# arangesh/Ground-Plane-Polling

Hardware: AMD Instinct MI355X
Metric: images/sec end-to-end (resnet50, 1k planes, 1242x375) (higher is better)
Workload: dtype f16x3

## Files before the change

### ground-plane-polling_amd/csrc/conv_igemm.hip

```cpp

#include <hip/hip_runtime.h>
#include <stdint.h>
#include <stdlib.h>

#include "conv_igemm_types.h"
#include "conv_tiles.h"
#include "gpp.h"

namespace {

inline bool is_x3(int dtype) { return dtype == GPP_BF16X3 || dtype == GPP_F16X3; }
inline bool f32_storage(int dtype) { return dtype == GPP_F32 || is_x3(dtype); }
inline int elem_size(int dtype) { return f32_storage(dtype) ? 4 : 2; }

int validate(const gpp_conv_desc& d)
{
    if (!d.in || !d.weight || !d.out) return GPP_ERR_BAD_ARG;
    if (d.dtype != GPP_BF16 && d.dtype != GPP_F16 && d.dtype != GPP_F32 && !is_x3(d.dtype)) return GPP_ERR_UNSUPPORTED;
    const int esz = elem_size(d.dtype), ck = 128 / esz, va = 16 / esz;
    if (d.batch <= 0 || d.C_in <= 0 || d.C_out <= 0 || d.KH <= 0 || d.KW <= 0) return GPP_ERR_BAD_ARG;
    constexpr int kMaxDim = 1 << 20;
    if (d.batch > kMaxDim || d.C_in > kMaxDim || d.C_out > kMaxDim || d.in_pitch > kMaxDim || d.out_pitch > kMaxDim || d.res_pitch > kMaxDim ||
        d.weight_rows > kMaxDim || d.weight_rows < 0 || d.in_pitch < 0 || d.out_pitch < 0 || d.res_pitch < 0 || d.partial_bytes < 0)
        return GPP_ERR_UNSUPPORTED;
    if (d.KH > 8 || d.KW > 8) return GPP_ERR_UNSUPPORTED;
    if (d.C_in % ck != 0 || d.C_out % 4 != 0) return GPP_ERR_UNSUPPORTED;
    if (d.stride != 1 && d.stride != 2) return GPP_ERR_UNSUPPORTED;
    if (d.n_groups < 1 || d.n_groups > GPP_MAX_GROUPS) return GPP_ERR_BAD_ARG;
    if (d.split_k < 0) return GPP_ERR_BAD_ARG;
#ifndef GPP_STAMPS
    if (d.reserved != 0) return GPP_ERR_BAD_ARG;
#endif
    if (d.reserved2 != 0 || (d.x3_split & ~(GPP_X3_IN | GPP_X3_OUT | GPP_X3_RES))) return GPP_ERR_BAD_ARG;
    if (d.reserved3 != 0 || (d.gather_rows != nullptr) != (d.gather_counts != nullptr)) return GPP_ERR_BAD_ARG;
    if (((uintptr_t)d.gather_rows | (uintptr_t)d.gather_counts | (uintptr_t)d.guard) & 3) return GPP_ERR_ALIGN;
    if (d.gather_rows && (d.stride != 1 || d.residual || !d.out_f32 || d.split_k > 1)) return GPP_ERR_UNSUPPORTED;
    if (d.x3_split && !is_x3(d.dtype)) return GPP_ERR_BAD_ARG;
    if (d.out_scale && d.dtype != GPP_F16X3) return GPP_ERR_BAD_ARG;
    if ((d.x3_split & GPP_X3_OUT) && (d.out_f32 || d.C_out % 32 != 0 || d.out_pitch % 32 != 0)) return GPP_ERR_UNSUPPORTED;
    if ((d.x3_split & GPP_X3_IN) && d.in_pitch % 32 != 0) return GPP_ERR_UNSUPPORTED;
    if ((d.x3_split & GPP_X3_RES) && (!d.residual || d.res_pitch % 32 != 0)) return GPP_ERR_UNSUPPORTED;
    const int oa = (d.out_f32 || f32_storage(d.dtype)) ? 4 : 8;
    if (d.in_pitch < d.C_in || d.in_pitch % va != 0) return GPP_ERR_ALIGN;
    if (d.out_pitch < d.C_out || d.out_pitch % oa != 0) return GPP_ERR_ALIGN;
    if (d.residual && (d.res_pitch < d.C_out || d.res_pitch % va != 0)) return GPP_ERR_ALIGN;
    if (((uintptr_t)d.in | (uintptr_t)d.weight | (uintptr_t)d.out | (uintptr_t)d.zero_page | (uintptr_t)d.residual |
         (uintptr_t)d.bias | (uintptr_t)d.partial) & 15)
        return GPP_ERR_ALIGN;
    for (int g = 0; g < d.n_groups; ++g) {
        const gpp_conv_group& G = d.groups[g];
        if (G.H_in <= 0 || G.W_in <= 0 || G.H_out <= 0 || G.W_out <= 0) return GPP_ERR_BAD_ARG;
        if (G.H_in > kMaxDim || G.W_in > kMaxDim || G.H_out > kMaxDim || G.W_out > kMaxDim || G.H_res > kMaxDim || G.W_res > kMaxDim) return GPP_ERR_UNSUPPORTED;
        constexpr int64_t kMaxOff = (int64_t)1 << 40;
        if (G.in_off < 0 || G.out_off < 0 || G.res_off < 0 || G.in_bstride < 0 || G.out_bstride < 0 || G.res_bstride < 0 || G.in_off > kMaxOff ||
            G.out_off > kMaxOff || G.res_off > kMaxOff || G.in_bstride > kMaxOff || G.out_bstride > kMaxOff || G.res_bstride > kMaxOff)
            return GPP_ERR_BAD_ARG;
        if ((G.out_off | G.out_bstride) % oa != 0) return GPP_ERR_ALIGN;
        if ((G.in_off | G.in_bstride) % va != 0) return GPP_ERR_ALIGN;
        if (d.residual && ((G.res_off | G.res_bstride) % va != 0 || G.H_res <= 0 || G.W_res <= 0)) return GPP_ERR_ALIGN;
        if ((int64_t)d.batch * G.H_out * G.W_out >= (1LL << 31)) return GPP_ERR_UNSUPPORTED;
        if ((d.x3_split & GPP_X3_OUT) && ((G.out_off | G.out_bstride) % 32 != 0)) return GPP_ERR_ALIGN;
        if ((d.x3_split & GPP_X3_IN) && ((G.in_off | G.in_bstride) % 32 != 0)) return GPP_ERR_ALIGN;
        if ((d.x3_split & GPP_X3_RES) && ((G.res_off | G.res_bstride) % 32 != 0)) return GPP_ERR_ALIGN;
    }
    return GPP_OK;
}

int split_rule(const gpp_conv_desc& d)
{
    if (!d.partial) return 1;
    int64_t pix = 0;
    for (int g = 0; g < d.n_groups; ++g) pix += (int64_t)d.groups[g].H_out * d.groups[g].W_out;
    const int64_t tiles_per_image = ((pix + 127) / 128) * ((d.C_out + 127) / 128);
    const int64_t kdepth = (int64_t)d.KH * d.KW * d.C_in;
    if (tiles_per_image > 24 || kdepth < 3072) return 1;
    int split = (int)((kdepth + 768) / 1536);
    return split < 1 ? 1 : (split > 8 ? 8 : split);
}

int fill_range_counter(gpp_conv_desc& d)
{
    if (d.dtype != GPP_F16X3) return d.range_counter ? GPP_ERR_BAD_ARG : GPP_OK;
    if (!d.range_counter) d.range_counter = (uint64_t*)gpp_x3_range_counter_f16x3();
    if (!d.range_counter) return GPP_ERR_UNSUPPORTED;
    return ((uintptr_t)d.range_counter & 7) ? GPP_ERR_ALIGN : GPP_OK;
}

int dispatch_any(gpp_conv_desc& d, hipStream_t st)
{
    const int rc = fill_range_counter(d);
    if (rc != GPP_OK) return rc;
    if (d.split_k == 0) d.split_k = split_rule(d);
    if (d.gather_rows) {
        if (d.split_k > 1) return GPP_ERR_UNSUPPORTED;
        return gpp_conv_gather_dispatch(d, st);
    }
    switch (d.dtype) {
        case GPP_BF16: return gpp_conv_dispatch_bf16(d, st);
        case GPP_F16: return gpp_conv_dispatch_f16(d, st);
        case GPP_BF16X3: return gpp_conv_dispatch_bf16x3(d, st);
        case GPP_F16X3: return gpp_conv_dispatch_f16x3(d, st);
        default: return gpp_conv_dispatch_f32(d, st);
    }
}

int tail_entry(const gpp_conv_desc* conv3x3, const gpp_conv_desc* conv1x1, int tile_rows, void* stream)
{
    if (!conv3x3 || !conv1x1) return GPP_ERR_BAD_ARG;
    gpp_conv_desc d1 = *conv3x3, d2 = *conv1x1;
    int rc = validate(d1);
    if (rc == GPP_OK) rc = validate(d2);
    if (rc != GPP_OK) return rc;
    if (d1.gather_rows || d2.gather_rows || d1.guard || d2.guard) return GPP_ERR_UNSUPPORTED;
    const gpp_conv_group &G1 = d1.groups[0], &G2 = d2.groups[0];
    if (d1.dtype == GPP_F32) return GPP_ERR_UNSUPPORTED;
    if (is_x3(d1.dtype) && (!(d1.x3_split & GPP_X3_IN) || (d2.x3_split & (GPP_X3_OUT | GPP_X3_RES)) != (GPP_X3_OUT | GPP_X3_RES) || !d2.residual))
        return GPP_ERR_UNSUPPORTED;
    if (d1.dtype != d2.dtype || d1.n_groups != 1 || d2.n_groups != 1 || d1.batch != d2.batch) return GPP_ERR_UNSUPPORTED;
    if (d1.KH != 3 || d1.KW != 3 || d1.stride != 1 || d1.pad_top != 1 || d1.pad_left != 1 || d1.residual || d1.out_f32) return GPP_ERR_UNSUPPORTED;
    if (d1.C_in != d1.C_out || (d1.C_in != 64 && d1.C_in != 128) || d1.weight_rows < d1.C_out) return GPP_ERR_UNSUPPORTED;
    if (d2.KH != 1 || d2.KW != 1 || d2.stride != 1 || d2.pad_top != 0 || d2.pad_left != 0 || d2.C_in != d1.C_out) return GPP_ERR_UNSUPPORTED;
    if (d2.C_out % 128 != 0 || d2.weight_rows < d2.C_out) return GPP_ERR_UNSUPPORTED;
    if (G1.H_in != G1.H_out || G1.W_in != G1.W_out || G2.H_out != G1.H_out || G2.W_out != G1.W_out || G2.H_in != G1.H_out || G2.W_in != G1.W_out)
        return GPP_ERR_BAD_ARG;
    rc = fill_range_counter(d1);
    if (rc == GPP_OK) rc = fill_range_counter(d2);
    if (rc != GPP_OK) return rc;
    hipStream_t st = (hipStream_t)stream;
    switch (d1.dtype) {
        case GPP_BF16: return gpp_tail_dispatch_bf16(d1, d2, tile_rows, st);
        case GPP_F16: return gpp_tail_dispatch_f16(d1, d2, tile_rows, st);
        case GPP_BF16X3: return gpp_tail_dispatch_bf16x3(d1, d2, tile_rows, st);
        default: return gpp_tail_dispatch_f16x3(d1, d2, tile_rows, st);
    }
}

int block_entry(const gpp_conv_desc* conv_a, const gpp_conv_desc* conv_b, const gpp_conv_desc* conv_c, int tile, void* stream)
{
    if (!conv_a || !conv_b || !conv_c) return GPP_ERR_BAD_ARG;
    gpp_conv_desc d1 = *conv_a, d2 = *conv_b, d3 = *conv_c;
    int rc = validate(d1);
    if (rc == GPP_OK) rc = validate(d2);
    if (rc == GPP_OK) rc = validate(d3);
    if (rc != GPP_OK) return rc;
    if (d1.gather_rows || d2.gather_rows || d3.gather_rows || d1.guard || d2.guard || d3.guard) return GPP_ERR_UNSUPPORTED;
    const gpp_conv_group &G1 = d1.groups[0], &G2 = d2.groups[0], &G3 = d3.groups[0];
    if (!is_x3(d1.dtype) || d1.dtype != d2.dtype || d1.dtype != d3.dtype) return GPP_ERR_UNSUPPORTED;
    if (d1.n_groups != 1 || d2.n_groups != 1 || d3.n_groups != 1 || d1.batch != d2.batch || d1.batch != d3.batch) return GPP_ERR_UNSUPPORTED;
    if (d1.x3_split != (GPP_X3_IN | GPP_X3_OUT) || d2.x3_split != (GPP_X3_IN | GPP_X3_OUT) || d3.x3_split != (GPP_X3_IN | GPP_X3_OUT | GPP_X3_RES))
        return GPP_ERR_UNSUPPORTED;
    if (d1.KH != 1 || d1.KW != 1 || d1.pad_top != 0 || d1.pad_left != 0 || d1.residual || d1.out_f32 || d1.split_k > 1) return GPP_ERR_UNSUPPORTED;
    if (d2.KH != 3 || d2.KW != 3 || d2.stride != 1 || d2.pad_top != 1 || d2.pad_left != 1 || d2.residual || d2.out_f32 || d2.split_k > 1) return GPP_ERR_UNSUPPORTED;
    if (d3.KH != 1 || d3.KW != 1 || d3.stride != 1 || d3.pad_top != 0 || d3.pad_left != 0 || !d3.residual || d3.out_f32 || d3.split_k > 1) return GPP_ERR_UNSUPPORTED;
    const int C = d2.C_in;
    if ((C != 64 && C != 128) || d2.C_out != C || d1.C_out != C || d3.C_in != C || d3.C_out % 128 != 0) return GPP_ERR_UNSUPPORTED;
    if (d1.weight_rows < C || d2.weight_rows < C || d3.weight_rows < d3.C_out) return GPP_ERR_UNSUPPORTED;
    if (G1.H_out != (G1.H_in - 1) / d1.stride + 1 || G1.W_out != (G1.W_in - 1) / d1.stride + 1) return GPP_ERR_BAD_ARG;
    if (G2.H_in != G1.H_out || G2.W_in != G1.W_out || G2.H_out != G1.H_out || G2.W_out != G1.W_out || G3.H_in != G1.H_out || G3.W_in != G1.W_out ||
        G3.H_out != G1.H_out || G3.W_out != G1.W_out || G3.H_res != G1.H_out || G3.W_res != G1.W_out)
        return GPP_ERR_BAD_ARG;
    rc = fill_range_counter(d1);
    if (rc == GPP_OK) rc = fill_range_counter(d2);
    if (rc == GPP_OK) rc = fill_range_counter(d3);
    if (rc != GPP_OK) return rc;
    if (d1.range_counter != d3.range_counter || d2.range_counter != d3.range_counter) return GPP_ERR_BAD_ARG;
    hipStream_t st = (hipStream_t)stream;
    return d1.dtype == GPP_F16X3 ? gpp_block_dispatch_f16x3(d1, d2, d3, tile, st) : gpp_block_dispatch_bf16x3(d1, d2, d3, tile, st);
}

}

extern "C" int gpp_bottleneck_block(const gpp_conv_desc* conv1x1_a, const gpp_conv_desc* conv3x3_b, const gpp_conv_desc* conv1x1_c, int tile, void* stream)
{
    return block_entry(conv1x1_a, conv3x3_b, conv1x1_c, tile, stream);
}

extern "C" int gpp_bottleneck_tail(const gpp_conv_desc* conv3x3, const gpp_conv_desc* conv1x1, int tile_rows, void* stream)
{
    return tail_entry(conv3x3, conv1x1, tile_rows, stream);
}

extern "C" int gpp_x3_range_events(uint64_t* host_count, int reset)
{
    unsigned long long v = 0;
    const int rc = gpp_x3_range_events_f16x3(&v, reset);
    if (rc == GPP_OK && host_count) *host_count = (uint64_t)v;
    return rc;
}

extern "C" int gpp_x3_range_snapshot(uint64_t* device_count, void* stream)
{
    return gpp_x3_range_snapshot_of(nullptr, device_count, stream);
}

extern "C" int gpp_x3_range_snapshot_of(const uint64_t* counter, uint64_t* device_count, void* stream)
{
    if (!device_count) return GPP_ERR_BAD_ARG;
    if (((uintptr_t)counter | (uintptr_t)device_count) & 7) return GPP_ERR_ALIGN;
    return gpp_x3_range_snapshot_f16x3((const unsigned long long*)counter, (unsigned long long*)device_count, (hipStream_t)stream);
}

extern "C" int gpp_conv2d_flops(const gpp_conv_desc* host_desc, double* flops)
{
    if (!host_desc || !flops) return GPP_ERR_BAD_ARG;
    if (host_desc->n_groups < 1 || host_desc->n_groups > GPP_MAX_GROUPS) return GPP_ERR_BAD_ARG;
    double f = 0.0;
    for (int g = 0; g < host_desc->n_groups; ++g)
        f += 2.0 * host_desc->batch * (double)host_desc->groups[g].H_out * host_desc->groups[g].W_out *
             host_desc->KH * host_desc->KW * (double)host_desc->C_in * host_desc->C_out;
    *flops = f;
    return GPP_OK;
}

extern "C" int gpp_conv2d_split_rule(const gpp_conv_desc* host_desc, int* split_k)
{
    if (!host_desc || !split_k) return GPP_ERR_BAD_ARG;
    gpp_conv_desc d = *host_desc;
    int rc = validate(d);
    if (rc != GPP_OK) return rc;
    *split_k = d.split_k > 0 ? d.split_k : split_rule(d);
    return GPP_OK;
}

extern "C" int gpp_conv2d_workspace_bytes(const gpp_conv_desc* host_desc, size_t* bytes)
{
    if (!host_desc || !bytes) return GPP_ERR_BAD_ARG;
    gpp_conv_desc d = *host_desc;
    char probe[16] __attribute__((aligned(16)));
    if (!d.partial) { d.partial = probe; d.partial_bytes = 0; }
    int rc = validate(d);
    if (rc != GPP_OK) return rc;
    const int split = d.split_k > 0 ? d.split_k : split_rule(d);
    *bytes = 0;
    if (split <= 1) return GPP_OK;
    int64_t rows = 0;
    for (int g = 0; g < d.n_groups; ++g) rows += (int64_t)d.batch * d.groups[g].H_out * d.groups[g].W_out + 256;
    const int64_t npad = (d.C_out + 255) / 256 * 256;
    *bytes = (size_t)(split * rows * npad * 4);
    return GPP_OK;
}

extern "C" int gpp_conv2d_igemm(const gpp_conv_desc* host_desc, void* stream)
{
    if (!host_desc) return GPP_ERR_BAD_ARG;
    gpp_conv_desc d = *host_desc;
    for (int g = 0; g < GPP_MAX_GROUPS; ++g) d.groups[g].row_begin = 0;
    int rc = validate(d);
    if (rc != GPP_OK) return rc;
    return dispatch_any(d, (hipStream_t)stream);
}

static const gpp_tiles::Entry kTiles[] = {{0, gpp_tiles::PLAIN, gpp_tiles::ALL, 0, 128, 0, 0, 0}, GPP_CONV_TILES(GPP_TILE_ENTRY, GPP_TILE_NONE, GPP_TILE_NONE)};

static bool env_is_1(const char* name) { const char* e = getenv(name); return e && e[0] == '1'; }

static bool tile_is_candidate(const gpp_conv_desc* desc, const gpp_tiles::Entry& t)
{
    using namespace gpp_tiles;
    const gpp_conv_desc& d = *desc;
    if ((d.gather_rows != nullptr) != (t.form == GATHER)) return t.code == 0;
    const bool x3_in = is_x3(d.dtype) && (d.x3_split & GPP_X3_IN);
    if (!owner_has(t.owner, f32_storage(d.dtype), is_x3(d.dtype))) return false;
    if (is_x3(d.dtype) && x3_wants_split_input(t.form, t.owner) && !x3_in && t.owner != ALL_X3IN) return false;
    const int nk = d.KH * d.KW * (d.C_in / (128 / elem_size(d.dtype)));
    if (t.form == DUAL && !dual_can_run(d, nk)) return false;
    if (t.form == MIX && !mix_can_run(d, nk)) return false;
    if (t.form == WS && !ws_can_run(d, t.bm, t.bn)) return false;
    static const bool no_deep = env_is_1("GPP_NO_DEEP_TILES"), no_ws = env_is_1("GPP_NO_WS_TILES"), no_mix = env_is_1("GPP_NO_MIX_TILES");
    int64_t rows = 0;
    for (int g = 0; g < d.n_groups; ++g) rows += (int64_t)d.batch * d.groups[g].H_out * d.groups[g].W_out;
    const int bn = t.bn;
    const auto pads_less_than = [&](int other) { return (d.C_out + bn - 1) / bn * bn < (d.C_out + other - 1) / other * other; };
    switch (t.form) {
        case GATHER: return bn != 160 || pads_less_than(64);
        case DEEP: {
            int64_t tiles_m = 0;
            for (int g = 0; g < d.n_groups; ++g) tiles_m += ((int64_t)d.batch * d.groups[g].H_out * d.groups[g].W_out + t.bm - 1) / t.bm;
            const int64_t wgs = tiles_m * ((d.C_out + bn - 1) / bn) * (d.split_k > 1 ? d.split_k : 1);
            return !(bn == 64 && d.C_out > 256) && !no_deep && nk >= 12 && wgs <= 320;
        }
        case WS: return !no_ws && rows >= 256 * 16;
        case MIX: return !no_mix && nk >= 4 && rows * (d.C_out / 256) >= 256 * 256;
        default: break;
    }
    if (t.code == 0) return true;
    if (bn == 64 && d.C_out > 256 && !(d.KH == 1 && d.KW == 1 && d.C_in <= 256)) return false;
    if (bn == 256 && (d.C_out < 192 || rows < 256 * 16)) return false;
    if ((t.form == PIPE || t.form == DUAL) && nk < 4) return false;
    if ((bn == 160 || bn == 96) && !pads_less_than(128)) return false;
    return true;
}

extern "C" int gpp_conv2d_tile_candidates(const gpp_conv_desc* desc, int* tiles, int capacity, int* count)
{
    if (!desc || !count || capacity < 0 || (capacity > 0 && !tiles)) return GPP_ERR_BAD_ARG;
    {
        gpp_conv_desc d = *desc;
        for (int g = 0; g < GPP_MAX_GROUPS; ++g) d.groups[g].row_begin = 0;
        const int rc = validate(d);
        if (rc != GPP_OK) return rc;
    }
    int n = 0;
    for (const gpp_tiles::Entry& t : kTiles) {
        if (!tile_is_candidate(desc, t)) continue;
        if (n < capacity) tiles[n] = t.code;
        ++n;
    }
    *count = n;
    return GPP_OK;
}

extern "C" int gpp_conv2d_autotune(gpp_conv_desc* desc, int iters, void* stream, float* best_us)
{
    if (!desc || iters < 1) return GPP_ERR_BAD_ARG;
    {
        gpp_conv_desc d = *desc;
        for (int g = 0; g < GPP_MAX_GROUPS; ++g) d.groups[g].row_begin = 0;
        const int rc = validate(d);
        if (rc != GPP_OK) return rc;
    }
    hipStream_t st = (hipStream_t)stream;
    hipEvent_t e0, e1;
    hipError_t e = hipEventCreate(&e0);
    if (e != hipSuccess) return (int)e;
    e = hipEventCreate(&e1);
    if (e != hipSuccess) { (void)hipEventDestroy(e0); return (int)e; }
    const int tile_in = desc->tile_hint;
    float best = 1e30f;
    int best_tile = tile_in, rc = GPP_OK;
    auto time_one = [&](int tile, float* us, int reps = 2) -> int {
        desc->tile_hint = tile;
        int r = gpp_conv2d_igemm(desc, stream);
        if (r != GPP_OK) return r;
        float t_best = 1e30f;
        for (int rep = 0; rep < reps; ++rep) {
            (void)hipEventRecord(e0, st);
            for (int i = 0; i < iters; ++i) (void)gpp_conv2d_igemm(desc, stream);
            (void)hipEventRecord(e1, st);
            hipError_t s = hipEventSynchronize(e1);
            if (s != hipSuccess) return (int)s;
            float ms = 0.0f;
            (void)hipEventElapsedTime(&ms, e0, e1);
            t_best = ms < t_best ? ms : t_best;
        }
        *us = t_best * 1000.0f / iters;
        return GPP_OK;
    };
    float second = 1e30f;
    int second_tile = -1;
    for (const gpp_tiles::Entry& t : kTiles) {
        if (!tile_is_candidate(desc, t)) continue;
        const int tile = t.code;
        float us = 0.0f;
        int r = time_one(tile, &us);
        if (r != GPP_OK) { if (tile == 0) { rc = r; break; } continue; }
        if (us < best) { second = best; second_tile = best_tile; best = us; best_tile = tile; }
        else if (us < second) { second = us; second_tile = tile; }
    }
    if (rc == GPP_OK && second_tile >= 0 && second_tile != best_tile && second <= best * 1.05f) {
        float sum_a = 0.0f, sum_b = 0.0f;
        bool ok = true;
        for (int round = 0; round < 3 && ok; ++round) {
            float a = 0.0f, b = 0.0f;
            ok = time_one(best_tile, &a, 1) == GPP_OK && time_one(second_tile, &b, 1) == GPP_OK;
            sum_a += a;
            sum_b += b;
        }
        if (ok && sum_b < sum_a) { best_tile = second_tile; best = sum_b / 3.0f; }
        else if (ok) best = sum_a / 3.0f;
    }
    (void)hipEventDestroy(e0);
    (void)hipEventDestroy(e1);
    desc->tile_hint = rc == GPP_OK ? best_tile : tile_in;
    if (best_us) *best_us = best;
    return rc;
}

namespace {

#define GPP_TILE_CODE(code, ...) code,
static const int kPreactTiles[] = {0, GPP_CONV_TILES(GPP_TILE_NONE, GPP_TILE_NONE, GPP_TILE_CODE)};
#undef GPP_TILE_CODE

int preact_validate(gpp_conv_desc& d, const float* in_scale, const float* in_shift)
{
    for (int g = 0; g < GPP_MAX_GROUPS; ++g) d.groups[g].row_begin = 0;
    int rc = validate(d);
    if (rc != GPP_OK) return rc;
    if (d.dtype != GPP_F32 && !is_x3(d.dtype)) return GPP_ERR_UNSUPPORTED;
    if (!in_scale || !in_shift) return GPP_ERR_BAD_ARG;
    if (((uintptr_t)in_scale | (uintptr_t)in_shift) & 15) return GPP_ERR_ALIGN;
    if (d.KH != 1 || d.KW != 1 || d.stride != 1 || d.pad_top != 0 || d.pad_left != 0) return GPP_ERR_UNSUPPORTED;
    if (d.x3_split & GPP_X3_IN) return GPP_ERR_UNSUPPORTED;
    if (d.gather_rows || d.guard) return GPP_ERR_UNSUPPORTED;
    if (d.C_in > 4096) return GPP_ERR_UNSUPPORTED;
    return GPP_OK;
}

int preact_run(gpp_conv_desc& d, const float* in_scale, const float* in_shift, hipStream_t st)
{
    int rc = fill_range_counter(d);
    if (rc != GPP_OK) return rc;
    if (d.split_k == 0) d.split_k = split_rule(d);
    switch (d.dtype) {
        case GPP_BF16X3: return gpp_preact_dispatch_bf16x3(d, in_scale, in_shift, st);
        case GPP_F16X3: return gpp_preact_dispatch_f16x3(d, in_scale, in_shift, st);
        default: return gpp_preact_dispatch_f32(d, in_scale, in_shift, st);
    }
}

}

extern "C" int gpp_conv2d_preact(const gpp_conv_desc* host_desc, const float* in_scale, const float* in_shift, void* stream)
{
    if (!host_desc) return GPP_ERR_BAD_ARG;
    gpp_conv_desc d = *host_desc;
    const int rc = preact_validate(d, in_scale, in_shift);
    if (rc != GPP_OK) return rc;
    return preact_run(d, in_scale, in_shift, (hipStream_t)stream);
}

extern "C" int gpp_conv2d_preact_tile_candidates(const gpp_conv_desc* desc, int* tiles, int capacity, int* count)
{
    if (!desc || !count || capacity < 0 || (capacity > 0 && !tiles)) return GPP_ERR_BAD_ARG;
    gpp_conv_desc d = *desc;
    static const float probe[4] __attribute__((aligned(16))) = {0.f, 0.f, 0.f, 0.f};
    const int rc = preact_validate(d, probe, probe);
    if (rc != GPP_OK) return rc;
    int n = 0;
    for (int tile : kPreactTiles) {
        if (n < capacity) tiles[n] = tile;
        ++n;
    }
    *count = n;
    return GPP_OK;
}

extern "C" int gpp_conv2d_preact_autotune(gpp_conv_desc* desc, const float* in_scale, const float* in_shift, int iters, void* stream,
                                          float* best_us)
{
    if (!desc || iters < 1) return GPP_ERR_BAD_ARG;
    {
        gpp_conv_desc d = *desc;
        const int rc = preact_validate(d, in_scale, in_shift);
        if (rc != GPP_OK) return rc;
    }
    hipStream_t st = (hipStream_t)stream;
    hipEvent_t e0, e1;
    hipError_t e = hipEventCreate(&e0);
    if (e != hipSuccess) return (int)e;
    e = hipEventCreate(&e1);
    if (e != hipSuccess) { (void)hipEventDestroy(e0); return (int)e; }
    const int tile_in = desc->tile_hint;
    float best = 1e30f;
    int best_tile = tile_in, rc = GPP_OK;
    for (int tile : kPreactTiles) {
        desc->tile_hint = tile;
        int r = gpp_conv2d_preact(desc, in_scale, in_shift, stream);
        if (r != GPP_OK) { if (tile == 0) { rc = r; break; } continue; }
        float t_best = 1e30f;
        for (int rep = 0; rep < 2 && r == GPP_OK; ++rep) {
            (void)hipEventRecord(e0, st);
            for (int i = 0; i < iters; ++i) (void)gpp_conv2d_preact(desc, in_scale, in_shift, stream);
            (void)hipEventRecord(e1, st);
            const hipError_t s = hipEventSynchronize(e1);
            if (s != hipSuccess) { r = (int)s; break; }
            float ms = 0.0f;
            (void)hipEventElapsedTime(&ms, e0, e1);
            t_best = ms < t_best ? ms : t_best;
        }
        if (r != GPP_OK) { rc = r; break; }
        const float us = t_best * 1000.0f / iters;
        if (us < best) { best = us; best_tile = tile; }
    }
    (void)hipEventDestroy(e0);
    (void)hipEventDestroy(e1);
    desc->tile_hint = rc == GPP_OK ? best_tile : tile_in;
// ... 4 lines not shown
```

### ground-plane-polling_amd/csrc/conv_igemm_impl.h

```cpp
#ifndef GPP_CONV_IGEMM_IMPL_H_
#define GPP_CONV_IGEMM_IMPL_H_

#include <hip/hip_runtime.h>
#include <stdint.h>

#include <atomic>
#include <type_traits>

#include "conv_tiles.h"
#include "gpp.h"

namespace {

typedef __attribute__((ext_vector_type(8))) __bf16 bf16x8;
typedef __attribute__((ext_vector_type(8))) _Float16 f16x8;
typedef __attribute__((ext_vector_type(4))) float f32x4;

struct f32x8 {
    f32x4 lo, hi;
    __device__ __forceinline__ float operator[](int e) const { return e < 4 ? lo[e] : hi[e - 4]; }
};

template <int DT> struct Elem;
template <> struct Elem<GPP_BF16> {
// ... 269 lines not shown
        *(vec8*)dst = Elem<DT>::pack(v);
    }
}

struct RowAddr { int64_t obase; int64_t rbase; };
__device__ __forceinline__ RowAddr row_addr(const gpp_conv_desc& d, int m, int HoWo, int W_out, int H_out, int H_res, int W_res,
                                            int64_t out_off, int64_t out_bs, int64_t res_off, int64_t res_bs)
{
    const int b = m / HoWo, p = m - b * HoWo;
    int64_t rp = p;
    if (d.residual && (H_res != H_out || W_res != W_out)) {
        const float sy = (float)H_res / (float)H_out, sx = (float)W_res / (float)W_out;
        const int oy = p / W_out, ox = p - oy * W_out;
        const int ry = min((int)floorf((float)oy * sy), H_res - 1);
        const int rx = min((int)floorf((float)ox * sx), W_res - 1);
        rp = (int64_t)ry * W_res + rx;
    }
    RowAddr a;
    a.obase = out_off + (int64_t)b * out_bs + (int64_t)p * d.out_pitch;
    a.rbase = res_off + (int64_t)b * res_bs + rp * d.res_pitch;
    return a;
}

struct PixWalk {
    int b, oy, ox;
    __device__ __forceinline__ void init(int m, int HoWo, int W_out)
    {
        b = m / HoWo;
        const int p = m - b * HoWo;
        oy = p / W_out;
        ox = p - oy * W_out;
    }
    __device__ __forceinline__ void advance(int n, int H_out, int W_out)
    {
        ox += n;
        while (ox >= W_out) { ox -= W_out; ++oy; }
        while (oy >= H_out) { oy -= H_out; ++b; }
    }
};

__device__ __forceinline__ RowAddr row_addr_at(const gpp_conv_desc& d, const PixWalk& w, int W_out, int H_out, int H_res, int W_res,
                                               int64_t out_off, int64_t out_bs, int64_t res_off, int64_t res_bs)
{
    const int p = w.oy * W_out + w.ox;
    int64_t rp = p;
    if (d.residual && (H_res != H_out || W_res != W_out)) {
        const float sy = (float)H_res / (float)H_out, sx = (float)W_res / (float)W_out;
        const int ry = min((int)floorf((float)w.oy * sy), H_res - 1);
        const int rx = min((int)floorf((float)w.ox * sx), W_res - 1);
        rp = (int64_t)ry * W_res + rx;
    }
    RowAddr a;
    a.obase = out_off + (int64_t)w.b * out_bs + (int64_t)p * d.out_pitch;
    a.rbase = res_off + (int64_t)w.b * res_bs + rp * d.res_pitch;
    return a;
}

template <int DT> struct ElemX3 {
    using scalar = float;
    using vec8 = f32x8;
    using frag = f32x4;
    static constexpr int ESZ = 4;
    static __device__ __forceinline__ vec8 pack(const float (&v)[8]) { return Elem<GPP_F32>::pack(v); }
    static __device__ __forceinline__ f32x4 mfma(frag, frag, f32x4 c) { return c; }
    static __device__ __forceinline__ void split(const f32x4 x0, const f32x4 x1, typename X3Half<DT>::vec& hi, typename X3Half<DT>::vec& lo)
    {
        using half = typename X3Half<DT>::half;
#pragma unroll
        for (int e = 0; e < 8; ++e) {
            const float x = X3Half<DT>::clamp(e < 4 ? x0[e] : x1[e - 4]);
            const half h = (half)x;
            hi[e] = h;
            lo[e] = (half)(x - (float)h);
        }
    }
};
template <> struct Elem<GPP_BF16X3> : ElemX3<GPP_BF16X3> {};
template <> struct Elem<GPP_F16X3> : ElemX3<GPP_F16X3> {};

template <int DT> constexpr bool kF32Storage = (DT == GPP_F32 || DT == GPP_BF16X3 || DT == GPP_F16X3);

constexpr int stage_rows(int BM, int NW) { return (BM + 8 * NW - 1) / (8 * NW) * (8 * NW); }

template <int DT, int BM, int BN, int WM, int WN, int STAGES, bool PIPE, bool XIN = false, bool PRE = false, bool GATHER = false>
__device__ __forceinline__ void conv_igemm_body(const gpp_conv_desc& d, const int block_x, const int grid_x, const float* pre_s = nullptr,
                                                const float* pre_t = nullptr)
{
    static_assert(!XIN || kX3<DT>, "pre-split input maps: GPP_BF16X3 / GPP_F16X3");
    static_assert(!PRE || (!PIPE && !XIN && kF32Storage<DT>), "pre-activation: float32-sized input maps, plain loop");
    static_assert(!GATHER || (!PIPE && !PRE), "gathered rows: plain loop");
    if (d.guard != nullptr && *(const volatile int32_t*)d.guard != d.guard_value) return;
    using E = Elem<DT>;
    using vec8 = typename E::vec8;
    using frag = typename E::frag;
    using scalar = typename E::scalar;
    using xh8 = typename X3Half<DT>::vec;
    constexpr int ESZ = E::ESZ, CK = kRowBytes / ESZ;
    constexpr int NW = WM * WN;
    constexpr int MF = BM / WM / 16, NF = BN / WN / 16;
    constexpr int BMS = stage_rows(BM, NW);
    constexpr int A_BYTES = BMS * kRowBytes, B_BYTES = BN * kRowBytes, STAGE = A_BYTES + B_BYTES;
    constexpr int A_IT = BMS / 8 / NW, B_IT = BN / 8 / NW;
    constexpr int PER_STAGE = A_IT + B_IT;
    constexpr int PF = STAGES - 1;
    static_assert(MF >= 1 && NF >= 1 && A_IT >= 1 && B_IT >= 1 && BMS % (8 * NW) == 0 && BN % (8 * NW) == 0 && BM % (16 * WM) == 0, "tile / wave shape");

    extern __shared__ __attribute__((aligned(16))) unsigned char smem[];

    const int tid = threadIdx.x, lane = tid & 63;
    const int wave = __builtin_amdgcn_readfirstlane(tid >> 6);
    const int wm = wave / WN, wn = wave % WN;
    GPP_STAMP(0);

    const int bid = GATHER ? block_x : xcd_remap(block_x, grid_x);
    const int n_tiles = (d.C_out + BN - 1) / BN;
    const int nt = bid % n_tiles, mt = bid / n_tiles;
    int tile_start = 0, row_begin = 0, H_in = 0, W_in = 0, H_out = 0, W_out = 0, H_res = 0, W_res = 0;
    int64_t in_off = 0, in_bs = 0, out_off = 0, out_bs = 0, res_off = 0, res_bs = 0;
    int list_begin = 0, list_next = 0, group = 0;
#pragma unroll
    for (int q = 0; q < GPP_MAX_GROUPS; ++q) {
        if constexpr (GATHER) {
            if (q < d.n_groups && mt >= d.groups[q].tile_start) { list_begin = list_next; group = q; }
            if (q < d.n_groups) list_next += d.batch * d.groups[q].H_out * d.groups[q].W_out;
        }
        if (q < d.n_groups && mt >= d.groups[q].tile_start) {
            tile_start = d.groups[q].tile_start;
            row_begin = d.groups[q].row_begin;
            H_in = d.groups[q].H_in; W_in = d.groups[q].W_in;
            H_out = d.groups[q].H_out; W_out = d.groups[q].W_out;
            H_res = d.groups[q].H_res; W_res = d.groups[q].W_res;
            in_off = d.groups[q].in_off; in_bs = d.groups[q].in_bstride;
            out_off = d.groups[q].out_off; out_bs = d.groups[q].out_bstride;
            res_off = d.groups[q].res_off; res_bs = d.groups[q].res_bstride;
        }
    }
    const int HoWo = H_out * W_out;
    const int Mpix = d.batch * HoWo;
    const int32_t* const glist = GATHER ? d.gather_rows + list_begin : nullptr;
    const int Mg = GATHER ? min(max(d.gather_counts[group], 0), Mpix) : Mpix;
    const int m0 = row_begin + (mt - tile_start) * BM, n0 = nt * BN;
    if constexpr (GATHER) {
        if (m0 >= Mg) return;
    }
    auto pixel_of = [&](int m) { return min(max(glist[m], 0), Mpix - 1); };
    const int Ktot = d.KH * d.KW * d.C_in;
    const int cpt = d.C_in / CK;
    const int nk_total = d.KH * d.KW * cpt;
    const int nsplit = gridDim.y, split = blockIdx.y;
    int ks0 = 0, nk = nk_total;
    if (nsplit > 1) {
        ks0 = (int)((unsigned)(nk_total * split) / (unsigned)nsplit);
        nk = (int)((unsigned)(nk_total * (split + 1)) / (unsigned)nsplit) - ks0;
    }

    const int srow = lane >> 3;
    const int gchunk = (lane & 7) ^ srow;
    const __amdgpu_buffer_rsrc_t in_rsrc = __builtin_amdgcn_make_buffer_rsrc((void*)d.in, 0, d.in_bytes, 0x00020000);
    const __amdgpu_buffer_rsrc_t w_rsrc = __builtin_amdgcn_make_buffer_rsrc((void*)d.weight, 0, d.weight_bytes, 0x00020000);
    constexpr bool VOFF_INLINE = PIPE && A_IT >= 8;
    int a_base[A_IT], a_mask[A_IT], a_voff[VOFF_INLINE ? 1 : A_IT];
    int tap_delta = 0, tap_need = 0;
    const int pitch2 = d.in_pitch * ESZ;
    {
        PixWalk pw;
        if constexpr (!GATHER) pw.init(m0 + wave * A_IT * 8 + srow, HoWo, W_out);
#pragma unroll
        for (int i = 0; i < A_IT; ++i) {
            const int m = m0 + (wave * A_IT + i) * 8 + srow;
            a_mask[i] = 0;
            a_base[i] = 0;
            if (m < Mg) {
                if constexpr (GATHER) pw.init(pixel_of(m), HoWo, W_out);
                const int iy0 = pw.oy * d.stride - d.pad_top, ix0 = pw.ox * d.stride - d.pad_left;
                const int rlo = max(0, -iy0), rhi = min(d.KH, max(0, H_in - iy0));
                const int clo = max(0, -ix0), chi = min(d.KW, max(0, W_in - ix0));
                const int rmask = rhi > rlo ? ((1 << rhi) - 1) & ~((1 << rlo) - 1) : 0;
                const int cmask = chi > clo ? ((1 << chi) - 1) & ~((1 << clo) - 1) : 0;
                a_mask[i] = rmask | (cmask << 8);
                a_base[i] = (int)((in_off + (int64_t)pw.b * in_bs) * ESZ) + gchunk * 16 + (iy0 * W_in + ix0) * pitch2;
            }
            if (!GATHER && i + 1 < A_IT) pw.advance(8, H_out, W_out);
        }
    }
    int w_voff[B_IT];
#pragma unroll
    for (int i = 0; i < B_IT; ++i) w_voff[i] = (n0 + (wave * B_IT + i) * 8 + srow) * Ktot * ESZ + gchunk * 16;

    auto set_tap = [&](int kh, int kw) {
        const int delta = (kh * W_in + kw) * pitch2;
        const int need = (1 << kh) | (1 << (8 + kw));
        if constexpr (VOFF_INLINE) {
            tap_delta = delta; tap_need = need;
        } else {
#pragma unroll
            for (int i = 0; i < A_IT; ++i) a_voff[i] = ((a_mask[i] & need) == need) ? a_base[i] + delta : kOutOfRange;
        }
    };
    auto voff_of = [&](int i) {
        if constexpr (VOFF_INLINE) return ((a_mask[i] & tap_need) == tap_need) ? a_base[i] + tap_delta : kOutOfRange;
        else return a_voff[i];
    };
    auto stage = [&](int buf, int cc, int ks) {
        unsigned char* sa = smem + buf * STAGE + wave * A_IT * 8 * kRowBytes;
        unsigned char* sb = smem + buf * STAGE + A_BYTES + wave * B_IT * 8 * kRowBytes;
#pragma unroll
        for (int i = 0; i < A_IT; ++i) glds16(in_rsrc, voff_of(i), cc * kRowBytes, sa + i * 8 * kRowBytes);
#pragma unroll
        for (int i = 0; i < B_IT; ++i) glds16(w_rsrc, w_voff[i], ks * kRowBytes, sb + i * 8 * kRowBytes);
    };
// ... 456 lines not shown
        }
        if (use_pre) {
#pragma unroll
            for (int i = 0; i < MF; ++i) {
                const int m = m0 + wm * (BM / WM) + i * 16 + frow;
                if (m >= Mg) continue;
#pragma unroll
                for (int jj = 0; jj < NF / 2; ++jj) {
                    const int n = n0 + wn * COLS + jj * 32 + fq * 8;
                    if (n >= d.C_out) continue;
                    float v[8];
#pragma unroll
                    for (int e = 0; e < 4; ++e) {
                        v[e] = comb(acc[i][2 * jj][e], jj, e);
                        v[4 + e] = comb(acc[i][2 * jj + 1][e], jj, 4 + e);
                    }
                    finish8_pre<DT>(d, v, n, ra_pre[i].obase, true, rpre[i][jj]);
                }
            }
            GPP_STAMP_END();
            return;
        }
    }
    if (interior && !res) {
        const int mfirst = m0 + wm * (BM / WM) + frow;
        int b = mfirst / HoWo, p = mfirst - b * HoWo;
#pragma unroll
        for (int i = 0; i < MF; ++i) {
            const int64_t obase = out_off + (int64_t)b * out_bs + (int64_t)p * d.out_pitch;
#pragma unroll
            for (int jj = 0; jj < NF / 2; ++jj) {
                float v[8];
#pragma unroll
                for (int e = 0; e < 4; ++e) {
                    v[e] = comb(acc[i][2 * jj][e], jj, e);
                    v[4 + e] = comb(acc[i][2 * jj + 1][e], jj, 4 + e);
                }
                finish8_pre<DT>(d, v, n0 + wn * COLS + jj * 32 + fq * 8, obase, false, typename E::vec8());
            }
            p += 16;
            while (p >= HoWo) { p -= HoWo; ++b; }
        }
        GPP_STAMP_END();
        return;
    }
    PixWalk pwe;
    if constexpr (!GATHER) pwe.init(m0 + wm * (BM / WM) + frow, HoWo, W_out);
#pragma unroll
    for (int i = 0; i < MF; ++i) {
        const int m = m0 + wm * (BM / WM) + i * 16 + frow;
        if (m >= Mg) break;
        if constexpr (GATHER) pwe.init(pixel_of(m), HoWo, W_out);
        const RowAddr ra = row_addr_at(d, pwe, W_out, H_out, H_res, W_res, out_off, out_bs, res_off, res_bs);
        if constexpr (!GATHER) pwe.advance(16, H_out, W_out);
        const scalar* rrow = res ? res + ra.rbase : nullptr;
#pragma unroll
        for (int jj = 0; jj < NF / 2; ++jj) {
            const int n = n0 + wn * COLS + jj * 32 + fq * 8;
            if (n >= d.C_out) continue;
            float v[8];
#pragma unroll
            for (int e = 0; e < 4; ++e) {
                v[e] = comb(acc[i][2 * jj][e], jj, e);
                v[4 + e] = comb(acc[i][2 * jj + 1][e], jj, 4 + e);
            }
            finish8<DT>(d, v, n, ra.obase, rrow);
        }
    }
    GPP_STAMP_END();
}

template <int DT, int BM, int BN, int WM, int WN, int STAGES, bool PIPE, bool XIN = false>
__global__ __launch_bounds__(64 * WM * WN, 2) void conv_igemm_kernel(const gpp_conv_desc d)
{
    conv_igemm_body<DT, BM, BN, WM, WN, STAGES, PIPE, XIN>(d, blockIdx.x, gridDim.x);
}

template <int DT, int BM, int BN, int WM, int WN, int STAGES, bool XIN>
__global__ __launch_bounds__(64 * WM * WN, 2) void conv_gather_kernel(const gpp_conv_desc d)
{
    conv_igemm_body<DT, BM, BN, WM, WN, STAGES, false, XIN, false, true>(d, blockIdx.x, gridDim.x);
}

template <int DT, int BM, int BN, int WM, int WN>
__global__ __launch_bounds__(64 * WM * WN, 2) void conv_preact_kernel(const gpp_conv_desc d, const float* in_scale, const float* in_shift)
{
    conv_igemm_body<DT, BM, BN, WM, WN, 2, false, false, true>(d, blockIdx.x, gridDim.x, in_scale, in_shift);
}

template <int DT, bool XIN = false>
__global__ __launch_bounds__(512, 2) void conv_igemm_dual_kernel(const gpp_conv_desc d0, const gpp_conv_desc d1, const int n0,
                                                                 const int split0, const int n1)
{
    if ((int)blockIdx.x < split0) {
        if ((int)blockIdx.x < n0) conv_igemm_body<DT, 256, 256, 2, 4, 2, true, XIN>(d0, blockIdx.x, n0);
    } else {
        conv_igemm_body<DT, 512, 128, 4, 2, 2, true, XIN>(d1, (int)blockIdx.x - split0, n1);
    }
}

template <int DT, int BMA, int BMB, int BN, bool XIN>
__global__ __launch_bounds__(512, 2) void conv_igemm_mix_kernel(const gpp_conv_desc da, const gpp_conv_desc db, const int na,
                                                                const int splita, const int nb)
{
    if ((int)blockIdx.x < splita) {
        if ((int)blockIdx.x < na) conv_igemm_body<DT, BMA, BN, 2, 4, 2, true, XIN>(da, blockIdx.x, na);
    } else {
        conv_igemm_body<DT, BMB, BN, 2, 4, 2, true, XIN>(db, (int)blockIdx.x - splita, nb);
    }
}

template <int DT>
__global__ __launch_bounds__(256) void splitk_reduce_kernel(const gpp_conv_desc d, int BM, int npad, int nsplit)
{
    if (d.guard != nullptr && *(const volatile int32_t*)d.guard != d.guard_value) return;
    using scalar = typename Elem<DT>::scalar;
    const int n8 = (d.C_out + 7) / 8;
    const int64_t total = (int64_t)d.partial_rows * n8;
    const int64_t e = (int64_t)blockIdx.x * 256 + threadIdx.x;
    if (e >= total) return;
    const int r = (int)(e / n8), n = (int)(e - (int64_t)r * n8) * 8;
    const int mt = r / BM;
    int tile_start = 0, H_out = 0, W_out = 0, H_res = 0, W_res = 0;
    int64_t out_off = 0, out_bs = 0, res_off = 0, res_bs = 0;
#pragma unroll
    for (int q = 0; q < GPP_MAX_GROUPS; ++q) {
        if (q < d.n_groups && mt >= d.groups[q].tile_start) {
            tile_start = d.groups[q].tile_start;
            H_out = d.groups[q].H_out; W_out = d.groups[q].W_out;
            H_res = d.groups[q].H_res; W_res = d.groups[q].W_res;
            out_off = d.groups[q].out_off; out_bs = d.groups[q].out_bstride;
            res_off = d.groups[q].res_off; res_bs = d.groups[q].res_bstride;
        }
    }
    const int HoWo = H_out * W_out;
    const int m = r - tile_start * BM;
    if (m >= d.batch * HoWo) return;
    float v[8];
#pragma unroll
    for (int k = 0; k < 8; ++k) v[k] = 0.0f;
    const float* src = (const float*)d.partial + (int64_t)r * npad + n;
    for (int s = 0; s < nsplit; ++s) {
        const f32x4 a = *(const f32x4*)(src + (int64_t)s * d.partial_rows * npad);
        const f32x4 b = *(const f32x4*)(src + (int64_t)s * d.partial_rows * npad + 4);
#pragma unroll
        for (int k = 0; k < 4; ++k) { v[k] += a[k]; v[4 + k] += b[k]; }
    }
    if constexpr (DT == GPP_F16X3) {
        if (d.out_scale) {
#pragma unroll
            for (int k = 0; k < 8; ++k) if (n + k < d.C_out) v[k] *= d.out_scale[n + k];
        }
    }
    if (d.bias) {
#pragma unroll
        for (int k = 0; k < 8; ++k) if (n + k < d.C_out) v[k] += d.bias[n + k];
    }
    const RowAddr ra = row_addr(d, m, HoWo, W_out, H_out, H_res, W_res, out_off, out_bs, res_off, res_bs);
    finish8<DT>(d, v, n, ra.obase, d.residual ? (const scalar*)d.residual + ra.rbase : nullptr);
}

template <int DT, int BM, int CMID>
__global__ __launch_bounds__(256, 2) void bottleneck_tail_kernel(const gpp_conv_desc d1, const gpp_conv_desc d2)
{
    using E = Elem<DT>;
    using vec8 = typename E::vec8;
// ... 911 lines not shown

template <int DT, int BMA, int BMB>
int launch_mix(const gpp_conv_desc& d, hipStream_t st)
{
    constexpr int BN = 256, CUS = 256;
    constexpr int ESZ = Elem<DT>::ESZ, CK = kRowBytes / ESZ;
    static_assert(kX3<DT>, "mixed grids exist for the x3 types");
    if (!gpp_tiles::mix_can_run(d, d.KH * d.KW * (d.C_in / CK))) return GPP_ERR_UNSUPPORTED;
    const int n_tiles = d.C_out / BN;
    const int64_t rows0 = (int64_t)d.batch * d.groups[0].H_out * d.groups[0].W_out;
    auto tiles_b = [&](int64_t begin, int bm) {
        int64_t t = (rows0 - begin + bm - 1) / bm;
        for (int g = 1; g < d.n_groups; ++g) t += ((int64_t)d.batch * d.groups[g].H_out * d.groups[g].W_out + bm - 1) / bm;
        return t * n_tiles;
    };
    int64_t best_cost = (tiles_b(0, BMA) + CUS - 1) / CUS * BMA;
    int best_ra = 0;
    for (int ra = 1; ra <= 64; ++ra) {
        if ((ra * CUS) % n_tiles != 0) continue;
        const int64_t ma = (int64_t)ra * CUS / n_tiles;
        if (ma * BMA > rows0) break;
        const int64_t cost = (int64_t)ra * BMA + (tiles_b(ma * BMA, BMB) + CUS - 1) / CUS * BMB;
        if (cost < best_cost) { best_cost = cost; best_ra = ra; }
    }
    if (best_ra == 0) return GPP_ERR_UNSUPPORTED;
    constexpr int lds = 2 * (stage_rows(BMA > BMB ? BMA : BMB, 8) + BN) * kRowBytes;
    constexpr auto kernel = conv_igemm_mix_kernel<DT, BMA, BMB, BN, true>;
    const int rc = allow_lds<kernel>(lds);
    if (rc != GPP_OK) return rc;
    const int ma = best_ra * CUS / n_tiles;
    gpp_conv_desc da = d, db = d;
    da.n_groups = 1;
    const int ta = prepare<BMA, BN>(da);
    if (ta < 0) return ta;
    db.groups[0].row_begin = ma * BMA;
    const int tb = prepare<BMB, BN>(db);
    if (tb < 0) return tb;
    da.in_bytes = db.in_bytes;
    const int na = ma * n_tiles, nb = tb * n_tiles;
    const int splita = (na + 7) / 8 * 8;
    kernel<<<dim3((unsigned)(splita + nb)), dim3(512), lds, st>>>(da, db, na, splita, nb);
    return last_launch_rc();
}

template <int DT, int BM, int BN>
int launch_ws(gpp_conv_desc& d, hipStream_t st)
{
    constexpr int R = 4;
    static_assert(kX3<DT>, "weight-stationary 1 x 1: x3 types");
    if (!gpp_tiles::ws_can_run(d, BM, BN)) return GPP_ERR_UNSUPPORTED;
    const gpp_conv_group& G = d.groups[0];
    const int lds = (d.C_in / 32) * BN * kRowBytes + R * BM * kRowBytes;
    const int tiles = prepare<BM, BN>(d);
    if (tiles < 0) return tiles;
    const int n_mtiles = (int)(((int64_t)d.batch * G.H_out * G.W_out + BM - 1) / BM);
    const auto go = [&](auto has_res) {
        constexpr auto kernel = conv1x1_ws_kernel<DT, BM, BN, decltype(has_res)::value>;
        const int rc = allow_lds<kernel>(160 * 1024);
        if (rc != GPP_OK) return rc;
        kernel<<<dim3(256), dim3(512), lds, st>>>(d, n_mtiles);
        return last_launch_rc();
    };
    return d.residual ? go(std::true_type()) : go(std::false_type());
}

template <int DT, int BM, int BN, int WM, int WN, int STAGES, bool XIN = false>
int launch_gather(gpp_conv_desc& d, hipStream_t st)
{
    if constexpr (kX3<DT> && !XIN) {
        if (d.x3_split & GPP_X3_IN) return launch_gather<DT, BM, BN, WM, WN, STAGES, true>(d, st);
    }
    constexpr int BMS = stage_rows(BM, WM * WN);
    constexpr int lds = STAGES * (BMS + BN) * kRowBytes;
    constexpr auto kernel = conv_gather_kernel<DT, BM, BN, WM, WN, STAGES, XIN>;
    const int rc = allow_lds<kernel>(lds);
    if (rc != GPP_OK) return rc;
    const int tiles = prepare<BM, BN>(d);
    if (tiles < 0) return tiles;
    const int n_tiles = (d.C_out + BN - 1) / BN;
    kernel<<<dim3((unsigned)(tiles * n_tiles)), dim3(64 * WM * WN), lds, st>>>(d);
    return last_launch_rc();
}

template <int DT, int FORM, int OWNER, int BM, int BN, int WM, int WN, int STAGES>
int run_tile(gpp_conv_desc& d, hipStream_t st)
{
    if constexpr (FORM == gpp_tiles::GATHER) {
        return GPP_ERR_BAD_ARG;
    } else if constexpr (!gpp_tiles::owner_has(OWNER, kF32Storage<DT>, kX3<DT>)) {
        return kF32Storage<DT> ? GPP_ERR_UNSUPPORTED : GPP_ERR_BAD_ARG;
    } else {
        constexpr bool XIN = kX3<DT> && gpp_tiles::x3_wants_split_input(FORM, OWNER);
        if (XIN && !(d.x3_split & GPP_X3_IN)) return GPP_ERR_UNSUPPORTED;
        if constexpr (FORM == gpp_tiles::DUAL) return launch_dual<DT>(d, st);
        else if constexpr (FORM == gpp_tiles::MIX) return launch_mix<DT, BM, BN>(d, st);
        else if constexpr (FORM == gpp_tiles::WS) return d.guard ? GPP_ERR_UNSUPPORTED : launch_ws<DT, BM, BN>(d, st);
        else return launch<DT, BM, BN, WM, WN, STAGES, gpp_tiles::tile_pipelined(FORM, BM, BN, kF32Storage<DT>), XIN>(d, st);
    }
}

#define GPP_RUN_TILE(code, form, owner, bm, bn, wm, wn, stages) \
    case code: return run_tile<DT, gpp_tiles::form, gpp_tiles::owner, bm, bn, wm, wn, stages>(d, st);
#define GPP_RUN_GATHER(code, form, owner, bm, bn, wm, wn, stages) \
    case code: if constexpr (gpp_tiles::form == gpp_tiles::GATHER) return launch_gather<DT, bm, bn, wm, wn, stages>(d, st); else break;
#define GPP_RUN_PREACT(code, form, owner, bm, bn, wm, wn, stages) \
    case code: return launch_preact<DT, bm, bn, wm, wn>(d, in_scale, in_shift, st);

template <int DT>
int dispatch_preact(gpp_conv_desc& d, const float* in_scale, const float* in_shift, hipStream_t st)
{
    switch (d.tile_hint) {
        case 0: return d.C_out <= 64 ? launch_preact<DT, 128, 64, 2, 2>(d, in_scale, in_shift, st)
                                     : launch_preact<DT, 128, 128, 2, 2>(d, in_scale, in_shift, st);
        GPP_CONV_TILES(GPP_TILE_NONE, GPP_TILE_NONE, GPP_RUN_PREACT)
        default: return GPP_ERR_BAD_ARG;
    }
}

template <int DT>
int dispatch_gather(gpp_conv_desc& d, hipStream_t st)
{
    switch (d.tile_hint) {
        case 0: return launch_gather<DT, 64, 64, 2, 2, 2>(d, st);
        GPP_CONV_TILES(GPP_RUN_GATHER, GPP_RUN_GATHER, GPP_TILE_NONE)
        default: break;
    }
    return GPP_ERR_BAD_ARG;
}

template <int DT>
int dispatch(gpp_conv_desc& d, hipStream_t st)
{
#ifdef GPP_STAMPS
    if constexpr (!kF32Storage<DT>) {
        if ((d.reserved & 4) && (d.tile_hint == 128 || d.tile_hint == 128128)) return launch<DT, 128, 128, 2, 2, 2, true>(d, st);
        if ((d.reserved & 8) && (d.tile_hint == 512 || d.tile_hint == 256256)) return launch<DT, 256, 256, 2, 4, 2, false>(d, st);
    }
#endif
    switch (d.tile_hint) {
        GPP_CONV_TILES(GPP_RUN_TILE, GPP_RUN_TILE, GPP_TILE_NONE)
        case 0: break;
        default: return GPP_ERR_BAD_ARG;
    }
    if (d.C_out <= 64 || (d.C_out % 128 != 0 && d.C_out % 128 <= 64)) return launch<DT, 128, 64, 2, 2, 2, false>(d, st);
    if constexpr (!kF32Storage<DT>) {
        int64_t rows = 0;
        for (int g = 0; g < d.n_groups; ++g) rows += (int64_t)d.batch * d.groups[g].H_out * d.groups[g].W_out;
        const int nk = d.KH * d.KW * (d.C_in / 64);
        const int n256 = (d.C_out + 255) / 256;
        const int64_t big_blocks = ((rows + 255) / 256) * n256;
        const bool n_fits = d.C_out >= 256 && n256 * 256 * 7 <= d.C_out * 8;
        if (n_fits && big_blocks >= 512 && nk >= 8 && d.split_k <= 1) return launch<DT, 256, 256, 2, 4, 2, true>(d, st);
    }
    return launch<DT, 128, 128, 2, 2, 2, false>(d, st);
}

template <auto KERNEL, int BM, int CMID, int ESZ, int LDS>
int launch_tail_as(gpp_conv_desc& d1, gpp_conv_desc& d2, hipStream_t st)
{
    int rc = allow_lds<KERNEL>(LDS);
    if (rc == GPP_OK) rc = set_input_extent(d1, ESZ);
    if (rc == GPP_OK) rc = set_weight_extent(d1, 9 * CMID, ESZ);
    if (rc == GPP_OK) rc = set_weight_extent(d2, CMID, ESZ);
    if (rc != GPP_OK) return rc;
    const gpp_conv_group& G = d1.groups[0];
    const int64_t rows = (int64_t)d1.batch * G.H_out * G.W_out;
    KERNEL<<<dim3((unsigned)((rows + BM - 1) / BM)), dim3(256), LDS, st>>>(d1, d2);
    return last_launch_rc();
}

template <int DT, int BM, int CMID>
int launch_tail(gpp_conv_desc& d1, gpp_conv_desc& d2, hipStream_t st)
{
    return launch_tail_as<bottleneck_tail_kernel<DT, BM, CMID>, BM, CMID, 2, 2 * (BM + CMID) * kRowBytes>(d1, d2, st);
}

template <int DT, int BM, int CMID>
int launch_tail_x3(gpp_conv_desc& d1, gpp_conv_desc& d2, hipStream_t st)
{
    constexpr int KC = CMID / 32;
    constexpr int ring = 2 * (BM + CMID) * kRowBytes, phase2 = KC * BM * kRowBytes + KC * 128 * kRowBytes;
    return launch_tail_as<bottleneck_tail_x3_kernel<DT, BM, CMID>, BM, CMID, 4, (ring > phase2 ? ring : phase2)>(d1, d2, st);
}

template <int DT>
int dispatch_tail_x3(gpp_conv_desc& d1, gpp_conv_desc& d2, int tile_rows, hipStream_t st)
{
    if (d1.C_in != 64) return GPP_ERR_UNSUPPORTED;
    switch (tile_rows) {
        case 64: return launch_tail_x3<DT, 64, 64>(d1, d2, st);
        case 96: return launch_tail_x3<DT, 96, 64>(d1, d2, st);
        case 0:
        case 128: return launch_tail_x3<DT, 128, 64>(d1, d2, st);
        case 160: return launch_tail_x3<DT, 160, 64>(d1, d2, st);
        default: return GPP_ERR_BAD_ARG;
    }
}

template <int DT>
int dispatch_tail(gpp_conv_desc& d1, gpp_conv_desc& d2, int tile_rows, hipStream_t st)
{
    const bool c64 = d1.C_in == 64;
    switch (tile_rows) {
        case 96: return c64 ? launch_tail<DT, 96, 64>(d1, d2, st) : launch_tail<DT, 96, 128>(d1, d2, st);
        case 0:
        case 128: return c64 ? launch_tail<DT, 128, 64>(d1, d2, st) : launch_tail<DT, 128, 128>(d1, d2, st);
// ... 9 lines not shown
```

### ground-plane-polling_amd/csrc/conv_tiles.h

```cpp
#ifndef GPP_CONV_TILES_H_
#define GPP_CONV_TILES_H_

#include <stdint.h>

#include "gpp.h"

namespace gpp_tiles {

enum Form {
    PLAIN,
    PIPE,
    DUAL,
    MIX,
    WS,
    DEEP,
    GATHER,
    PREACT,
};

enum Owner {
    ALL,
    ALL_X3IN,
    B16,
    NOT_F32,
    X3,
    X3IN,
};

struct Entry {
    int code, form, owner;
    int bm, bn;
    int wm, wn, stages;
};

#define GPP_CONV_TILES(T, X, P)                                                                                                          \
    T(64064, PLAIN, ALL, 64, 64, 2, 2, 2)                                                                                                \
    T(96064, PLAIN, ALL, 96, 64, 2, 2, 2)                                                                                                \
    T(128064, PLAIN, ALL, 128, 64, 2, 2, 2)                                                                                              \
    T(160064, PLAIN, ALL, 160, 64, 2, 2, 2)                                                                                              \
    T(192064, PLAIN, ALL, 192, 64, 2, 2, 2)                                                                                              \
    T(64128, PLAIN, ALL, 64, 128, 2, 2, 2)                                                                                               \
    T(96128, PLAIN, ALL, 96, 128, 2, 2, 2)                                                                                               \
    T(128128, PLAIN, ALL, 128, 128, 2, 2, 2)                                                                                             \
    T(160128, PLAIN, ALL, 160, 128, 2, 2, 2)                                                                                             \
    T(192128, PLAIN, ALL, 192, 128, 2, 2, 2)                                                                                             \
    T(224128, PLAIN, ALL, 224, 128, 2, 2, 2)                                                                                             \
    T(1128128, PIPE, NOT_F32, 128, 128, 2, 2, 2)                                                                                         \
    T(1192128, PIPE, NOT_F32, 192, 128, 2, 2, 2)                                                                                         \
    T(1128256, PIPE, NOT_F32, 128, 256, 2, 4, 2)                                                                                         \
    T(1160256, PIPE, X3IN, 160, 256, 2, 4, 2)                                 \
    T(1192256, PIPE, NOT_F32, 192, 256, 2, 4, 2)                                                                                         \
    T(1224256, PIPE, X3IN, 224, 256, 2, 4, 2)                                                                                            \
                                \
    T(256256, PLAIN, NOT_F32, 256, 256, 2, 4, 2)                                                                                         \
    T(1256256, PIPE, X3IN, 256, 256, 2, 4, 2)                                                                                            \
                     \
    T(128160, PLAIN, ALL, 128, 160, 4, 1, 2)                                                                                             \
    T(192160, PLAIN, ALL_X3IN, 192, 160, 4, 1, 2)                  \
    T(1192160, PIPE, B16, 192, 160, 4, 1, 2)                                                                                             \
    T(1128160, PIPE, NOT_F32, 128, 160, 4, 1, 2)                                                                                         \
    T(2256256, DUAL, NOT_F32, 256, 256, 2, 4, 2)                                                                                         \
    T(1192096, PIPE, NOT_F32, 192, 96, 4, 1, 2)                                                                                          \
    T(3256224, MIX, X3IN, 256, 224, 2, 4, 2)                                                                                             \
    T(3192160, MIX, X3IN, 192, 160, 2, 4, 2)                                                                                             \
    T(4128064, WS, X3IN, 128, 64, 2, 4, 4)                                                                                               \
    T(4064064, WS, X3IN, 64, 64, 2, 4, 4)                                                                                                \
    T(4128128, WS, X3IN, 128, 128, 2, 4, 4)                                                                                              \
    T(4064128, WS, X3IN, 64, 128, 2, 4, 4)                                                                                               \
              \
    T(5064064, DEEP, X3IN, 64, 64, 2, 2, 4)                                                                                              \
    T(5096064, DEEP, X3IN, 96, 64, 2, 2, 4)                                                                                              \
    T(5064128, DEEP, X3IN, 64, 128, 2, 2, 4)                                                                                             \
    T(5096128, DEEP, X3IN, 96, 128, 2, 2, 4)                                                                                             \
    T(5128128, DEEP, X3IN, 128, 128, 2, 2, 4)                                                                                            \
                                                 \
    T(128256, PLAIN, X3, 128, 256, 2, 4, 2)                                                                                              \
    T(192256, PLAIN, X3, 192, 256, 2, 4, 2)                                                                                              \
           \
    T(6064064, GATHER, ALL, 64, 64, 2, 2, 2)                                                                                             \
    T(6032064, GATHER, ALL, 32, 64, 2, 2, 2)                                                                                             \
    T(6064160, GATHER, ALL, 64, 160, 4, 1, 2)                                                                                            \
    T(7064064, GATHER, ALL, 64, 64, 2, 2, 4)                                                                                             \
    T(7032064, GATHER, ALL, 32, 64, 2, 2, 4)                                                                                             \
    T(7064160, GATHER, ALL, 64, 160, 4, 1, 4)                                                                                            \
    X(64, PLAIN, ALL, 128, 64, 2, 2, 2)                                                                                                  \
    X(128, PLAIN, ALL, 128, 128, 2, 2, 2)                                                                                                \
    X(256, PLAIN, B16, 256, 128, 4, 2, 3)                                                             \
    X(512, PLAIN, B16, 256, 256, 2, 4, 2)                                                                                                \
    P(64064, PREACT, ALL, 64, 64, 2, 2, 2)                                                                                               \
    P(128064, PREACT, ALL, 128, 64, 2, 2, 2)                                                                                             \
    P(64128, PREACT, ALL, 64, 128, 2, 2, 2)                                                                                              \
    P(128128, PREACT, ALL, 128, 128, 2, 2, 2)                                                                                            \
    P(192128, PREACT, ALL, 192, 128, 2, 2, 2)

#define GPP_TILE_ENTRY(code, form, owner, bm, bn, wm, wn, stages) {code, gpp_tiles::form, gpp_tiles::owner, bm, bn, wm, wn, stages},
#define GPP_TILE_NONE(...)

constexpr bool owner_has(int owner, bool f32_storage, bool x3)
{
    return owner == ALL || owner == ALL_X3IN || (owner == B16 && !f32_storage) || (owner == NOT_F32 && (!f32_storage || x3)) ||
           ((owner == X3 || owner == X3IN) && x3);
}

constexpr bool x3_wants_split_input(int form, int owner)
{
    return owner == X3IN || owner == ALL_X3IN || (form != PLAIN && form != GATHER && form != PREACT);
}

constexpr bool tile_pipelined(int form, int bm, int bn, bool f32_storage) { return form == PIPE || (!f32_storage && form == PLAIN && bm == 256 && bn == 256); }


inline bool dual_can_run(const gpp_conv_desc& d, int nk) { return d.C_out >= 384 && d.C_out % 256 == 128 && nk >= 2 && d.split_k <= 1; }

inline bool mix_can_run(const gpp_conv_desc& d, int nk) { return d.C_out % 256 == 0 && nk >= 2 && d.split_k <= 1; }

inline bool ws_can_run(const gpp_conv_desc& d, int bm, int bn)
{
    const gpp_conv_group& G = d.groups[0];
    return (d.x3_split & GPP_X3_IN) && d.KH == 1 && d.KW == 1 && d.stride == 1 && d.pad_top == 0 && d.pad_left == 0 && d.n_groups == 1 && d.split_k <= 1 &&
           d.C_out % bn == 0 && 32 % (d.C_out / bn) == 0 && d.C_in % 32 == 0 && G.H_in == G.H_out && G.W_in == G.W_out &&
           (!d.residual || ((d.x3_split & GPP_X3_RES) && G.H_res == G.H_out && G.W_res == G.W_out)) &&
           (d.C_in / 32) * bn * 128 + 4 * bm * 128 <= 160 * 1024;
}

}

#endif
```

### ground-plane-polling_amd/csrc/decode.hip

```cpp

#include <hip/hip_runtime.h>
#include <stdint.h>
#include <limits.h>

#include <atomic>

#include "gpp.h"

namespace {

constexpr int kCounterStride = 4096;
constexpr int kHeaderBytes = 64 * kCounterStride;
constexpr int kKeptCountWord = 1;
constexpr int kKeptKeysOffset = 1024;

__device__ __forceinline__ float cephes_expf(float x)
{
    x = fminf(fmaxf(x, -88.3762626647949f), 88.3762626647949f);
    float fx = floorf(x * 1.44269504088896341f + 0.5f);
    x = (x - fx * 0.693359375f) - fx * -2.12194440e-4f;
    const float z = x * x;
    float y = 1.9875691500e-4f;
    y = y * x + 1.3981999507e-3f;
    y = y * x + 8.3334519073e-3f;
// ... 567 lines not shown
    if (stages & GPP_DETECT_CANDIDATES) {
        clear_counters_kernel<<<1, 64, 0, st>>>(cnt, lists);
        const dim3 grid((unsigned)((n_anchors + 255) / 256), (unsigned)B);
        if (osf) candidates_osf_kernel<<<grid, 256, 0, st>>>(cls_logits, n_anchors, kstride, score_thr, keys, cnt);
        else candidates_kernel<<<grid, 256, 0, st>>>(cls_logits, n_anchors, kstride, score_thr, keys, cnt);
    }
    if (stages & GPP_DETECT_SELECT) {
        static std::atomic<uint64_t> configured{0};
        int dev = 0;
        e = hipGetDevice(&dev);
        if (e != hipSuccess) return (int)e;
        if (!(configured.load(std::memory_order_acquire) & (1ull << (dev & 63)))) {
            e = hipFuncSetAttribute((const void*)nms_kernel, hipFuncAttributeMaxDynamicSharedMemorySize, kLdsKeys * 16 + kHistBins * 4);
            if (e != hipSuccess) return (int)e;
            configured.fetch_or(1ull << (dev & 63), std::memory_order_release);
        }
        nms_kernel<<<dim3((unsigned)lists), kNmsThreads, kLdsKeys * 16 + kHistBins * 4, st>>>(
            keys, cnt, kstride, cls_logits, regression, regression_dim, (const float4*)anchors, n_anchors, L, iou_thr, max_det,
            counts, wboxes, alive, ws, lists_per_image);
    }
    if (stages & GPP_DETECT_EMIT) {
        if (osf)
            emit_osf_kernel<<<dim3((unsigned)B), 512, 0, st>>>(ws, cls_logits, regression, regression_dim, (const float4*)anchors,
                                                               n_anchors, L, max_det, boxes, dims, scores, labels, orientations,
                                                               anchor_index, counts);
        else
            emit_kernel<<<dim3((unsigned)B), 128, 0, st>>>(ws, cls_logits, regression, regression_dim, (const float4*)anchors,
                                                           n_anchors, L, max_det, boxes, dims, scores, labels, orientations, anchor_index);
    }
    e = hipGetLastError();
    return e == hipSuccess ? GPP_OK : (int)e;
}

}

namespace {

__global__ __launch_bounds__(256) void pack_kernel(const float* __restrict__ boxes, const float* __restrict__ dims,
                                                   const float* __restrict__ scores, const int32_t* __restrict__ labels,
                                                   const int32_t* __restrict__ orient, const float* __restrict__ keypoints,
                                                   const float* __restrict__ keyplanes, const float* __restrict__ residuals,
                                                   float* __restrict__ out, int64_t rows)
{
    const int64_t e = (int64_t)blockIdx.x * 256 + threadIdx.x;
    if (e >= rows * 35) return;
    const int64_t r = e / 35;
    const int c = (int)(e - r * 35);
    float v;
    if (c < 12) v = boxes[r * 12 + c];
    else if (c < 15) v = dims[r * 3 + (c - 12)];
    else if (c == 15) v = scores[r];
    else if (c == 16) v = (float)labels[r];
    else if (c == 17) v = (float)orient[r];
    else if (c < 30) v = keypoints[r * 12 + (c - 18)];
    else if (c < 34) v = keyplanes[r * 4 + (c - 30)];
    else v = residuals[r];
    out[e] = v;
}

}

extern "C" int gpp_pack_detections(const float* boxes, const float* dims, const float* scores, const int32_t* labels,
                                   const int32_t* orientations, const float* keypoints, const float* keyplanes,
                                   const float* residuals, int B, int D, float* packed, void* stream)
{
    if (B < 0 || D < 0) return GPP_ERR_BAD_ARG;
    if (B == 0 || D == 0) return GPP_OK;
    if (!boxes || !dims || !scores || !labels || !orientations || !keypoints || !keyplanes || !residuals || !packed) return GPP_ERR_BAD_ARG;
    const int64_t rows = (int64_t)B * D;
    pack_kernel<<<dim3((unsigned)((rows * 35 + 255) / 256)), 256, 0, (hipStream_t)stream>>>(
        boxes, dims, scores, labels, orientations, keypoints, keyplanes, residuals, packed, rows);
    hipError_t e = hipGetLastError();
    return e == hipSuccess ? GPP_OK : (int)e;
}

namespace {

struct LevelTable {
    int n_levels;
    int pix[GPP_MAX_GROUPS];
    int pix_begin[GPP_MAX_GROUPS];
    int word_begin[GPP_MAX_GROUPS];
    int list_begin[GPP_MAX_GROUPS];
};

__global__ __launch_bounds__(256) void mark_pixels_kernel(const unsigned long long* __restrict__ keys, const int32_t* __restrict__ cnt,
                                                          int64_t key_stride, int64_t n_anchors, int nba, int lists_per_image,
                                                          const LevelTable T, uint32_t* __restrict__ bitmap)
{
    const int list = blockIdx.y, b = list / lists_per_image;
    const int64_t n = min((int64_t)max(cnt[list * (kCounterStride / 4)], 0), n_anchors);
    for (int64_t i = (int64_t)blockIdx.x * 256 + threadIdx.x; i < n; i += (int64_t)gridDim.x * 256) {
        const uint32_t a = 0xFFFFFFFFu - (uint32_t)keys[(int64_t)list * key_stride + i];
        if ((int64_t)a >= n_anchors) continue;
        const int pixel = (int)(a / (uint32_t)nba);
        int l = 0;
        for (int q = 1; q < T.n_levels; ++q) l = pixel >= T.pix_begin[q] ? q : l;
        const int bit = b * T.pix[l] + (pixel - T.pix_begin[l]);
        atomicOr(&bitmap[T.word_begin[l] + (bit >> 5)], 1u << (bit & 31));
    }
}

constexpr int kCompactThreads = 1024;
__global__ __launch_bounds__(kCompactThreads) void compact_pixels_kernel(uint32_t* __restrict__ bitmap, const LevelTable T, int B, int max_rows,
                                                                         int32_t* __restrict__ rows, int32_t* __restrict__ counts,
                                                                         int32_t* __restrict__ flag)
{
    __shared__ int wave_sum[kCompactThreads / 64];
    const int tid = threadIdx.x, lane = tid & 63, wave = tid >> 6;
    int total = 0;
    for (int l = 0; l < GPP_MAX_GROUPS; ++l) {
        int running = 0;
        if (l < T.n_levels) {
            const int n_words = (B * T.pix[l] + 31) >> 5;
            for (int w0 = 0; w0 < n_words; w0 += kCompactThreads) {
                const int w = w0 + tid;
                uint32_t word = 0;
                if (w < n_words) {
                    word = bitmap[T.word_begin[l] + w];
                    if (word) bitmap[T.word_begin[l] + w] = 0;
                }
                const int c = __popc(word);
                int incl = c;
#pragma unroll
                for (int s = 1; s < 64; s <<= 1) {
                    const int up = __shfl_up(incl, s, 64);
                    if (lane >= s) incl += up;
                }
                if (lane == 63) wave_sum[wave] = incl;
                __syncthreads();
                int before = 0, all = 0;
#pragma unroll
                for (int q = 0; q < kCompactThreads / 64; ++q) {
                    const int v = wave_sum[q];
                    before += q < wave ? v : 0;
                    all += v;
                }
                __syncthreads();
                int pos = running + before + incl - c;
                while (word) {
                    const int bit = __ffs((int)word) - 1;
                    word &= word - 1;
                    rows[T.list_begin[l] + pos++] = w * 32 + bit;
                }
                running += all;
            }
        }
        if (tid == 0) counts[l] = running;
        total += running;
    }
    if (tid == 0) {
        counts[GPP_MAX_GROUPS] = total;
        flag[0] = total > max_rows ? 1 : 0;
    }
}

}

extern "C" int gpp_detect_pixel_lists(const gpp_pixel_list_desc* host_desc, void* stream)
{
    if (!host_desc) return GPP_ERR_BAD_ARG;
    const gpp_pixel_list_desc& d = *host_desc;
    if (d.B < 0 || d.B > kMaxBatch || d.n_anchors <= 0 || d.n_anchors > kMaxAnchors || d.num_base_anchors <= 0 || d.max_rows < 0 ||
        d.n_levels < 1 || d.n_levels > GPP_MAX_GROUPS || (d.lists_per_image != 1 && d.lists_per_image != 4) || d.reserved != 0 || d.reserved2 != 0)
        return GPP_ERR_BAD_ARG;
    if (d.B == 0) return GPP_OK;
    if (!d.workspace || !d.bitmap || !d.rows || !d.counts || !d.flag) return GPP_ERR_BAD_ARG;
    if (((uintptr_t)d.workspace & 15) || (((uintptr_t)d.bitmap | (uintptr_t)d.rows | (uintptr_t)d.counts | (uintptr_t)d.flag) & 3)) return GPP_ERR_ALIGN;
    const int lists = d.B * d.lists_per_image;
    if (lists > 64) return GPP_ERR_UNSUPPORTED;
    LevelTable T;
    T.n_levels = d.n_levels;
    int64_t pixels = 0, words = 0;
    for (int l = 0; l < GPP_MAX_GROUPS; ++l) {
        const int pix = l < d.n_levels ? d.level_pixels[l] : 0;
        if (l < d.n_levels && pix <= 0) return GPP_ERR_BAD_ARG;
        if ((int64_t)d.B * (pixels + pix) >= (1LL << 31)) return GPP_ERR_UNSUPPORTED;
        T.pix[l] = pix;
        T.pix_begin[l] = (int)pixels;
        T.word_begin[l] = (int)words;
        T.list_begin[l] = (int)((int64_t)d.B * pixels);
        pixels += pix;
        words += ((int64_t)d.B * pix + 31) / 32;
    }
    if (pixels * d.num_base_anchors != d.n_anchors) return GPP_ERR_BAD_ARG;
    hipStream_t st = (hipStream_t)stream;
    const unsigned char* ws = (const unsigned char*)d.workspace;
    const int32_t* cnt = (const int32_t*)ws;
    const unsigned long long* keys = (const unsigned long long*)(ws + kHeaderBytes);
    mark_pixels_kernel<<<dim3(16, (unsigned)lists), 256, 0, st>>>(keys, cnt, pow2_ceil(d.n_anchors), d.n_anchors, d.num_base_anchors,
                                                                   d.lists_per_image, T, d.bitmap);
    compact_pixels_kernel<<<1, kCompactThreads, 0, st>>>(d.bitmap, T, d.B, d.max_rows, d.rows, d.counts, d.flag);
    const hipError_t e = hipGetLastError();
    return e == hipSuccess ? GPP_OK : (int)e;
}

extern "C" int gpp_detect_workspace_bytes(int B, int64_t n_anchors, size_t* bytes)
{
    if (!bytes || B < 0 || B > kMaxBatch || n_anchors <= 0 || n_anchors > kMaxAnchors) return GPP_ERR_BAD_ARG;
    *bytes = detect_bytes(B, n_anchors, 1);
    return GPP_OK;
}

extern "C" int gpp_detect_osf_workspace_bytes(int B, int64_t n_anchors, size_t* bytes)
{
    if (!bytes || B < 0 || B > kMaxBatch || n_anchors <= 0 || n_anchors > kMaxAnchors) return GPP_ERR_BAD_ARG;
    *bytes = detect_bytes(B, n_anchors, 4);
    return GPP_OK;
}

extern "C" int gpp_detect_stages_f32(int stages, const float* cls_logits, const float* regression,
                                     const float* regression_dim, const float* anchors, int B, int64_t n_anchors,
                                     int num_base_anchors, int fused_layout, float score_thr, float iou_thr, int max_det,
                                     float* boxes, float* dims, float* scores, int32_t* labels, int32_t* orientations,
                                     int32_t* anchor_index, int32_t* counts,
                                     void* workspace, size_t workspace_bytes, void* stream)
{
    return detect_impl(stages, 1, cls_logits, regression, regression_dim, anchors, B, n_anchors, num_base_anchors, fused_layout, score_thr,
                       iou_thr, max_det, boxes, dims, scores, labels, orientations, anchor_index, counts, workspace, workspace_bytes, stream);
}

extern "C" int gpp_detect_osf_f32(const float* cls_logits, const float* regression, const float* regression_dim,
                                  const float* anchors, int B, int64_t n_anchors, int num_base_anchors, int fused_layout,
                                  float score_thr, float iou_thr, int max_det,
                                  float* boxes, float* dims, float* scores, int32_t* labels, int32_t* orientations,
                                  int32_t* anchor_index, int32_t* counts,
                                  void* workspace, size_t workspace_bytes, void* stream)
{
    return detect_impl(GPP_DETECT_CANDIDATES | GPP_DETECT_SELECT | GPP_DETECT_EMIT, 4, cls_logits, regression, regression_dim, anchors, B,
                       n_anchors, num_base_anchors, fused_layout, score_thr, iou_thr, max_det, boxes, dims, scores, labels, orientations,
                       anchor_index, counts, workspace, workspace_bytes, stream);
}

extern "C" int gpp_detect_f32(const float* cls_logits, const float* regression, const float* regression_dim,
                              const float* anchors, int B, int64_t n_anchors, int num_base_anchors, int fused_layout,
                              float score_thr, float iou_thr, int max_det,
                              float* boxes, float* dims, float* scores, int32_t* labels, int32_t* orientations,
                              int32_t* anchor_index, int32_t* counts,
                              void* workspace, size_t workspace_bytes, void* stream)
{
    return gpp_detect_stages_f32(GPP_DETECT_CANDIDATES | GPP_DETECT_SELECT | GPP_DETECT_EMIT, cls_logits, regression, regression_dim,
                                 anchors, B, n_anchors, num_base_anchors, fused_layout, score_thr, iou_thr, max_det, boxes, dims,
                                 scores, labels, orientations, anchor_index, counts, workspace, workspace_bytes, stream);
}
```

### ground-plane-polling_amd/keras_retinanet_3D/backend/hip.py

```python

import ctypes
import os

_LIB = None
_HERE = os.path.dirname(os.path.abspath(__file__))
LIB_PATH = os.environ.get('GPP_LIB') or os.path.normpath(os.path.join(_HERE, '..', '..', 'lib', 'libgpp_hip.so'))
CSRC_DIR = os.path.normpath(os.path.join(_HERE, '..', '..', 'csrc'))

GPP_OK = 0
_ERRORS = {
    -1: 'GPP_ERR_BAD_ARG',
    -2: 'GPP_ERR_WORKSPACE',
    -3: 'GPP_ERR_ALIGN',
    -4: 'GPP_ERR_UNSUPPORTED',
}

c_void_p = ctypes.c_void_p
c_int = ctypes.c_int
c_float = ctypes.c_float
c_size_t = ctypes.c_size_t
c_int64 = ctypes.c_int64


GPP_BF16 = 1
GPP_F16 = 2
GPP_F32 = 3
GPP_BF16X3 = 4
GPP_F16X3 = 5
GPP_MAX_GROUPS = 5
GPP_DRAW_PRIM_WORDS = 16
GPP_DRAW_PRIMS_PER_DET = 26
GPP_DRAW_COUNT_WORDS = 4
GPP_POSE_COLS = 36
GPP_EVAL_MAX_DETECTIONS, GPP_EVAL_MAX_ANNOTATIONS = 1024, 1024
GPP_EVAL_ANN_COLS, GPP_EVAL_ERR_COLS = 17, 11
GPP_KITTI_MAX_DETECTIONS, GPP_KITTI_MAX_LABELS = 128, 128
GPP_KITTI_MAX_THRESHOLDS, GPP_KITTI_LABEL_COLS = 41, 16
GPP_LABEL_MOD_COLS = 20
GPP_ABSMAX_F32, GPP_ABSMAX_SPLIT_F16, GPP_ABSMAX_SPLIT_BF16 = 1, 2, 3


class GppError(RuntimeError):
    pass


class ConvGroup(ctypes.Structure):
    _fields_ = [('in_off', c_int64), ('in_bstride', c_int64), ('out_off', c_int64), ('out_bstride', c_int64),
                ('res_off', c_int64), ('res_bstride', c_int64),
                ('H_in', ctypes.c_int32), ('W_in', ctypes.c_int32), ('H_out', ctypes.c_int32), ('W_out', ctypes.c_int32),
                ('H_res', ctypes.c_int32), ('W_res', ctypes.c_int32), ('tile_start', ctypes.c_int32),
                ('row_begin', ctypes.c_int32)]


class ConvDesc(ctypes.Structure):
    _fields_ = [('inp', c_void_p), ('weight', c_void_p), ('bias', c_void_p), ('residual', c_void_p),
                ('out', c_void_p), ('zero_page', c_void_p),
                ('dtype', ctypes.c_int32), ('out_f32', ctypes.c_int32),
                ('batch', ctypes.c_int32), ('C_in', ctypes.c_int32), ('C_out', ctypes.c_int32),
                ('KH', ctypes.c_int32), ('KW', ctypes.c_int32), ('stride', ctypes.c_int32),
                ('pad_top', ctypes.c_int32), ('pad_left', ctypes.c_int32),
                ('in_pitch', ctypes.c_int32), ('out_pitch', ctypes.c_int32), ('res_pitch', ctypes.c_int32),
                ('weight_rows', ctypes.c_int32), ('relu', ctypes.c_int32), ('n_groups', ctypes.c_int32),
                ('tile_hint', ctypes.c_int32), ('reserved', ctypes.c_int32),
                ('in_bytes', ctypes.c_int32), ('weight_bytes', ctypes.c_int32),
                ('partial', c_void_p), ('partial_bytes', c_int64), ('split_k', ctypes.c_int32), ('partial_rows', ctypes.c_int32),
                ('groups', ConvGroup * GPP_MAX_GROUPS),
                ('x3_split', ctypes.c_int32), ('reserved2', ctypes.c_int32), ('out_scale', c_void_p), ('range_counter', c_void_p),
                ('gather_rows', c_void_p), ('gather_counts', c_void_p), ('guard', c_void_p),
                ('guard_value', ctypes.c_int32), ('reserved3', ctypes.c_int32)]


class PixelListDesc(ctypes.Structure):
    _fields_ = [('workspace', c_void_p), ('bitmap', c_void_p), ('rows', c_void_p), ('counts', c_void_p), ('flag', c_void_p),
                ('n_anchors', c_int64)] + \
               [(n, ctypes.c_int32) for n in ('B', 'num_base_anchors', 'lists_per_image', 'n_levels', 'max_rows', 'reserved')] + \
               [('level_pixels', ctypes.c_int32 * GPP_MAX_GROUPS), ('reserved2', ctypes.c_int32)]


class MobileNetBlockDesc(ctypes.Structure):
    _fields_ = [('inp', c_void_p), ('dw_weight', c_void_p), ('dw_bias', c_void_p), ('pw_weight', c_void_p), ('pw_bias', c_void_p),
                ('out_scale', c_void_p), ('out', c_void_p)] + \
               [(n, ctypes.c_int32) for n in ('dtype', 'B', 'H', 'W', 'C_in', 'C_out', 'stride', 'in_pitch', 'out_pitch', 'weight_rows',
                                              'tile_hint', 'reserved')]


class MobileNetStemDesc(ctypes.Structure):
    _fields_ = [('inp', c_void_p), ('weight', c_void_p), ('bias', c_void_p), ('out', c_void_p)] + \
               [(n, ctypes.c_int32) for n in ('B', 'H', 'W', 'C_out', 'out_pitch', 'reserved')]


class AbsmaxDesc(ctypes.Structure):
    _fields_ = [('inp', c_void_p), ('out', c_void_p), ('M', c_int64), ('pitch', c_int64)] + \
               [(n, ctypes.c_int32) for n in ('C', 'c_off', 'layout', 'reserved')]


class AbsmaxClearDesc(ctypes.Structure):
    _fields_ = [('table', c_void_p), ('n', c_int64)]


def _declare(lib):
    lib.gpp_version.restype = ctypes.c_char_p
    lib.gpp_version.argtypes = []
    lib.gpp_poll_workspace_bytes.restype = c_int
    lib.gpp_poll_workspace_bytes.argtypes = [c_int, c_int, c_int, ctypes.POINTER(c_size_t)]
    lib.gpp_poll_f32.restype = c_int
    lib.gpp_poll_f32.argtypes = [c_void_p] * 5 + [c_int, c_int, c_int, c_int, c_float] + [c_void_p] * 4 + \
        [c_void_p, c_size_t, c_void_p]
    lib.gpp_pose_f32.restype = c_int
    lib.gpp_pose_f32.argtypes = [c_void_p] * 8 + [c_int, c_int, c_float] + [c_void_p] * 3
    if hasattr(lib, 'gpp_draw_build'):
        lib.gpp_draw_workspace_bytes.restype = c_int
        lib.gpp_draw_workspace_bytes.argtypes = [c_int, c_int, ctypes.POINTER(c_size_t), ctypes.POINTER(c_size_t)]
        lib.gpp_draw_build.restype = c_int
        lib.gpp_draw_build.argtypes = [c_void_p, c_void_p, c_int, c_int, c_float, c_void_p, c_void_p, c_void_p]
        lib.gpp_draw_raster.restype = c_int
        lib.gpp_draw_raster.argtypes = [c_void_p, c_void_p, c_int, c_int, c_void_p, c_void_p, c_int, c_void_p, c_void_p, c_void_p]
    if hasattr(lib, 'gpp_eval_match_f32'):
        lib.gpp_eval_match_f32.restype = c_int
        lib.gpp_eval_match_f32.argtypes = [c_void_p] * 8 + [c_int] * 4 + [c_float, c_int, ctypes.c_double] + [c_void_p] * 4
    if hasattr(lib, 'gpp_kitti_overlaps_f64'):
        lib.gpp_kitti_overlaps_f64.restype = c_int
        lib.gpp_kitti_overlaps_f64.argtypes = [c_void_p] * 3 + [c_int] * 3 + [c_void_p] * 2
        lib.gpp_kitti_stats_f64.restype = c_int
        lib.gpp_kitti_stats_f64.argtypes = [c_void_p] * 4 + [ctypes.POINTER(ctypes.c_double)] + [c_void_p] * 2 + [c_int] * 4 + [c_void_p] * 5
    if hasattr(lib, 'gpp_label_prep_f64'):
        lib.gpp_label_prep_f64.restype = c_int
        lib.gpp_label_prep_f64.argtypes = [c_void_p] * 4 + [c_int, c_int, ctypes.c_uint, c_int] + [c_void_p] * 7
    if hasattr(lib, 'gpp_detect_pixel_lists'):
        lib.gpp_detect_pixel_lists.restype = c_int
        lib.gpp_detect_pixel_lists.argtypes = [ctypes.POINTER(PixelListDesc), c_void_p]
    lib.gpp_conv2d_igemm.restype = c_int
    lib.gpp_conv2d_igemm.argtypes = [ctypes.POINTER(ConvDesc), c_void_p]
    lib.gpp_stem_conv7x7_bn_relu.restype = c_int
    lib.gpp_stem_conv7x7_bn_relu.argtypes = [c_void_p, c_void_p, c_void_p, c_void_p, c_int, c_int, c_int, c_int, c_void_p]
    lib.gpp_stem_conv7x7_bn_relu_mfma.restype = c_int
    lib.gpp_stem_conv7x7_bn_relu_mfma.argtypes = [c_void_p, c_void_p, c_void_p, c_void_p, c_int, c_int, c_int, c_int, c_void_p]
    lib.gpp_stem_pack_weights_f16.restype = c_int
    lib.gpp_stem_pack_weights_f16.argtypes = [c_void_p, c_void_p, c_size_t]
    lib.gpp_stem_pack_weights_f16x3.restype = c_int
    lib.gpp_stem_pack_weights_f16x3.argtypes = [c_void_p, c_void_p, c_size_t]
    lib.gpp_stem_conv7x7_bn_relu_x3.restype = c_int
    lib.gpp_stem_conv7x7_bn_relu_x3.argtypes = [c_void_p, c_void_p, c_void_p, c_void_p, c_int, c_int, c_int, c_void_p]
    lib.gpp_stem_pool_fused_mfma.restype = c_int
    lib.gpp_stem_pool_fused_mfma.argtypes = [c_void_p, c_void_p, c_void_p, c_void_p, c_int, c_int, c_int, c_int, c_void_p]
    lib.gpp_maxpool3x3s2_same.restype = c_int
    lib.gpp_maxpool3x3s2_same.argtypes = [c_void_p, c_void_p, c_int, c_int, c_int, c_int, c_int, c_void_p]
    lib.gpp_conv2d_preact.restype = c_int
    lib.gpp_conv2d_preact.argtypes = [ctypes.POINTER(ConvDesc), c_void_p, c_void_p, c_void_p]
    lib.gpp_conv2d_preact_tile_candidates.restype = c_int
    lib.gpp_conv2d_preact_tile_candidates.argtypes = [ctypes.POINTER(ConvDesc), ctypes.POINTER(c_int), c_int, ctypes.POINTER(c_int)]
    lib.gpp_conv2d_preact_autotune.restype = c_int
    lib.gpp_conv2d_preact_autotune.argtypes = [ctypes.POINTER(ConvDesc), c_void_p, c_void_p, c_int, c_void_p, ctypes.POINTER(c_float)]
    lib.gpp_maxpool3x3s2_pad_f32.restype = c_int
    lib.gpp_maxpool3x3s2_pad_f32.argtypes = [c_void_p, c_void_p, c_int, c_int, c_int, c_int, c_int, c_int, c_void_p]
    lib.gpp_avgpool2x2_f32.restype = c_int
    lib.gpp_avgpool2x2_f32.argtypes = [c_void_p, c_void_p, c_int, c_int, c_int, c_int, c_int, c_void_p]
    lib.gpp_mobilenet_block.restype = c_int
    lib.gpp_mobilenet_block.argtypes = [ctypes.POINTER(MobileNetBlockDesc), c_void_p]
    lib.gpp_mobilenet_block_tile_candidates.restype = c_int
# ... 261 lines not shown
```

### ground-plane-polling_amd/keras_retinanet_3D/models/plan.py

```python

import collections
import ctypes

import numpy as np

from ..backend import hip
from ..layers import conv as C


class StemDesc(ctypes.Structure):
    _fields_ = [('inp', ctypes.c_void_p), ('weight', ctypes.c_void_p), ('bias', ctypes.c_void_p), ('out', ctypes.c_void_p),
                ('dtype', ctypes.c_int32), ('B', ctypes.c_int32), ('H', ctypes.c_int32), ('W', ctypes.c_int32), ('range_counter', ctypes.c_void_p)]


class PoolDesc(ctypes.Structure):
    _fields_ = [('inp', ctypes.c_void_p), ('out', ctypes.c_void_p), ('dtype', ctypes.c_int32), ('B', ctypes.c_int32),
                ('H', ctypes.c_int32), ('W', ctypes.c_int32), ('C', ctypes.c_int32), ('reserved', ctypes.c_int32)]


class RaggedStemDesc(ctypes.Structure):
    _fields_ = [('stem', StemDesc), ('heights', ctypes.c_void_p), ('Hp', ctypes.c_int32), ('reserved', ctypes.c_int32)]


class RaggedPoolDesc(ctypes.Structure):
    _fields_ = [('pool', PoolDesc), ('heights', ctypes.c_void_p), ('Hp', ctypes.c_int32), ('reserved', ctypes.c_int32)]


class ReluDesc(ctypes.Structure):
    _fields_ = [('inp', ctypes.c_void_p), ('out', ctypes.c_void_p), ('in_bstride', ctypes.c_int64),
                ('out_bstride', ctypes.c_int64), ('count', ctypes.c_int64), ('dtype', ctypes.c_int32), ('B', ctypes.c_int32)]


class DetectDesc(ctypes.Structure):
    _fields_ = [(n, ctypes.c_void_p) for n in ('cls_logits', 'regression', 'regression_dim', 'anchors', 'boxes', 'dims',
                                               'scores', 'labels', 'orientations', 'anchor_index', 'counts', 'workspace')] + \
               [('workspace_bytes', ctypes.c_size_t), ('n_anchors', ctypes.c_int64),
                ('B', ctypes.c_int32), ('num_base_anchors', ctypes.c_int32), ('fused_layout', ctypes.c_int32),
                ('max_det', ctypes.c_int32), ('score_thr', ctypes.c_float), ('iou_thr', ctypes.c_float)]


class CandidatePixelsDesc(ctypes.Structure):
    _fields_ = [('detect', ctypes.c_void_p), ('lists', hip.PixelListDesc)]


class PollDesc(ctypes.Structure):
    _fields_ = [(n, ctypes.c_void_p) for n in ('boxes', 'dims', 'orient', 'P_inv', 'planes', 'keypoints', 'keyplanes',
                                               'residuals', 'best_idx', 'workspace')] + \
               [('workspace_bytes', ctypes.c_size_t), ('B', ctypes.c_int32), ('D', ctypes.c_int32), ('N', ctypes.c_int32),
                ('planes_batched', ctypes.c_int32), ('thr', ctypes.c_float), ('reserved', ctypes.c_int32)]


class PoseDesc(ctypes.Structure):
    _fields_ = [(n, ctypes.c_void_p) for n in ('boxes', 'dims', 'scores', 'labels', 'orientations', 'keypoints', 'residuals',
                                               'frame_info', 'rows', 'counts')] + \
               [('B', ctypes.c_int32), ('D', ctypes.c_int32), ('score_thr', ctypes.c_float), ('reserved', ctypes.c_int32)]


class PreactDesc(ctypes.Structure):
    _fields_ = [('conv', ctypes.c_void_p), ('in_scale', ctypes.c_void_p), ('in_shift', ctypes.c_void_p)]


class DensePoolDesc(ctypes.Structure):
    _fields_ = [('inp', ctypes.c_void_p), ('out', ctypes.c_void_p), ('B', ctypes.c_int32), ('H', ctypes.c_int32), ('W', ctypes.c_int32),
                ('C', ctypes.c_int32), ('pad', ctypes.c_int32), ('out_pitch', ctypes.c_int32)]


class PlanOp(ctypes.Structure):
    _fields_ = [('kind', ctypes.c_int32), ('tag', ctypes.c_int32), ('desc', ctypes.c_void_p)]


class TailDesc(ctypes.Structure):
    _fields_ = [('conv3x3', ctypes.c_void_p), ('conv1x1', ctypes.c_void_p), ('tile_rows', ctypes.c_int32), ('reserved', ctypes.c_int32)]


class BlockDesc(ctypes.Structure):
    _fields_ = [('conv1x1_a', ctypes.c_void_p), ('conv3x3_b', ctypes.c_void_p), ('conv1x1_c', ctypes.c_void_p), ('tile', ctypes.c_int32), ('reserved', ctypes.c_int32)]


OP_STEM, OP_MAXPOOL, OP_CONV, OP_RELU, OP_DETECT, OP_POLL, OP_TAIL = 1, 2, 3, 4, 5, 6, 7
OP_BLOCK = 16
OP_DETECT_CANDIDATES, OP_DETECT_SELECT, OP_DETECT_EMIT = 8, 9, 10
OP_DETECT_OSF = 12
OP_STEM_POOL = 13
OP_MAXPOOL_PAD, OP_AVGPOOL, OP_CONV_PREACT = 17, 18, 32
OP_MOBILENET_STEM, OP_MOBILENET_BLOCK = 33, 34
OP_POSE = 19
OP_ABSMAX, OP_ABSMAX_CLEAR = 35, 36
OP_STEM_RAGGED, OP_STEM_POOL_RAGGED, OP_MAXPOOL_RAGGED = 37, 38, 39
OP_DETECT_CANDIDATE_PIXELS = 40
DETECT_OPS = (OP_DETECT, OP_DETECT_CANDIDATES, OP_DETECT_SELECT, OP_DETECT_EMIT, 12, OP_DETECT_CANDIDATE_PIXELS)
OP_JOIN, OP_SYNC = 0x10000, 0x20000


PlanOptions = collections.namedtuple('PlanOptions', 'x3_level fuse_stem_pool stage_chunks half_stages fuse_tail fuse_block fuse_block_proj '
                                                    'br1_lane fpn_lanes p4_lane head_lanes decode_overlap cls_lane autotune tune_key sparse_heads')


def block_form(opts, width, projection, split_input, halves, join):
    if width in opts.fuse_block and (not projection or opts.fuse_block_proj) and split_input:
        launch = 'block'
    else:
        launch = 'tail' if width in opts.fuse_tail else 'convs'
    if not projection:
        return launch, 'identity'
    return launch, 'side' if opts.br1_lane and not halves and not join else 'inline'


def part_of(fm, c0, nb):
    return C.FMap(fm.buf, nb, fm.H, fm.W, fm.C, off=fm.off + c0 * fm.bstride, bstride=fm.bstride, pitch=fm.pitch, split=fm.split, half=fm.half)


TOWER_SLICES = {('pyramid_towers_0', 0): 'pyramid_regression_0', ('pyramid_towers_0', 512): 'pyramid_classification_0',
                ('pyramid_towers_0', 768): 'pyramid_regression_dim_0'}
RANGE_AUDIT_THRESHOLD = 2.0 ** -9
X3_QUANTUM = 2.0 ** -24
SPARSE_HEADS_MAX_SHARE = '0.5'


def audit_report(maps, table, threshold=RANGE_AUDIT_THRESHOLD):
    table = np.ascontiguousarray(table).view(np.uint32).reshape(-1)
    out = []
    for m in maps:
        first, n = m['row']
        bits = table[first:first + n]
        vals = bits.view(np.float32).astype(np.float64)
        live = vals[bits != 0]
        finite = live[~np.isnan(live)]
        absmax = float('nan') if len(finite) < len(live) else float(finite.max()) if len(finite) else 0.0
        rec = {k: m[k] for k in ('name', 'consumers', 'channels') if k in m}
        rec.update({'live': int(len(live)), 'absmax': absmax,
                    'absmax_min_live': float(finite.min()) if len(finite) else None,
                    'absmax_median_live': float(np.median(finite)) if len(finite) else None,
                    'small_channels': int((finite < threshold).sum()),
                    'bits': None if not absmax > 0 else int(min(22, max(0, np.floor(np.log2(absmax / X3_QUANTUM))))) if np.isfinite(absmax) else 22,
                    'flagged': bool(0 < absmax < threshold)})
        out.append(rec)
    return out


class SparseHeads(object):

    def __init__(self, torch, device, B, level_pixels, max_share):
        i32 = torch.int32
        self.B, self.level_pixels = B, [int(p) for p in level_pixels]
        total = B * sum(self.level_pixels)
        self.max_rows = max(0, min(total, int(max_share * total)))
        self.bitmap = torch.zeros((sum((B * p + 31) // 32 for p in self.level_pixels),), dtype=i32, device=device)
        self.rows = torch.zeros((total,), dtype=i32, device=device)
        self.counts = torch.zeros((hip.GPP_MAX_GROUPS + 1,), dtype=i32, device=device)
        self.flag = torch.ones((1,), dtype=i32, device=device)
        self.dense, self.gathered = [], []
        self.lists_joined = False

    def tensors(self):
        return [self.bitmap, self.rows, self.counts, self.flag]

    def put_every_nth(self, torch, n=8):
        begin, counts = 0, []
        for p in self.level_pixels:
            idx = torch.arange(0, self.B * p, n, dtype=torch.int32, device=self.rows.device)
            self.rows[begin:begin + idx.numel()] = idx
            counts.append(int(idx.numel()))
            begin += self.B * p
        counts += [0] * (hip.GPP_MAX_GROUPS - len(counts)) + [sum(counts)]
        self.counts.copy_(torch.as_tensor(counts, dtype=torch.int32))

    def reset(self, torch):
        self.counts.zero_()
        self.flag.fill_(1)


class Plan(object):

    def __init__(self):
        self.keep = []
        self.io = {}
        self.io_parts = {}
        self.tuning_parts = {}
        self.ops = []
        self.oracle_names = {}
        self.lanes = []
        self.access = []
        self.atomic = []
        self.wrote = []
        self.op_io = []
        self.audit_table = None
        self.audit_maps = []
        self.audit_unobserved = []
        self.inner = {}
        self.open_lanes = set()
        self.conv_descs = []
        self.ws_need = {}
        self.array = None
        self.flops = 0.0
        self.ragged = False
        self.heights = None
        self.sparse = None
        self.heads_stale = False

    @property
    def regression(self):
        self.complete_heads()
        return self._regression

    @regression.setter
    def regression(self, tensor):
        self._regression = tensor

    @property
    def regression_dim(self):
        self.complete_heads()
        return self._regression_dim

    @regression_dim.setter
    def regression_dim(self, tensor):
        self._regression_dim = tensor

    def complete_heads(self):
        if self.sparse is None or not self.heads_stale:
            return
        self.heads_stale = False
        for guarded in self.sparse.dense:
            d = type(guarded).from_buffer_copy(guarded)
            d.guard, d.guard_value = None, 0
            hip.check(hip.lib().gpp_conv2d_igemm(ctypes.byref(d), hip.stream_ptr()), 'gpp_conv2d_igemm (head tensors completed)')

    def emit(self, kind, desc, name, reads=(), writes=(), tag=0, flops=0.0, lane=0, join=False, sync=False, io=None, inner=(), atomic=()):
        self.keep += list(inner) + [desc]
        if inner:
            self.inner[id(desc)] = tuple(inner)
        self.ops.append((kind, tag, desc, name, flops))
        self.lanes.append((int(lane) << 8) | (OP_JOIN if join else 0) | (OP_SYNC if sync else 0))
        self.access.append((self.spans(reads), self.spans(writes)))
        self.atomic.append(self.spans(atomic))
        self.wrote.append([x for x in writes if isinstance(x, C.FMap)])
        self.op_io.append(io)
        self.flops += flops
        if lane:
            self.open_lanes.add(lane)
        elif join:
            self.open_lanes.clear()
        if io is not None:
            self.io[name] = io
            self.io_parts.setdefault(name, []).append(io)

    @staticmethod
    def span(fm):
        e = fm.buf.element_size()
        base = fm.buf.data_ptr() + fm.off * e
        size = ((fm.H * fm.W - 1) * fm.pitch + fm.C) * e
        return [(base + b * fm.bstride * e, base + b * fm.bstride * e + size) for b in range(fm.B)]

    @staticmethod
    def span_of(tensor):
        return [(tensor.data_ptr(), tensor.data_ptr() + tensor.numel() * tensor.element_size())]

    @staticmethod
    def spans(items):
        return [iv for x in items for iv in (Plan.span(x) if isinstance(x, C.FMap) else Plan.span_of(x))]

    def insert_behind(self, extra):
        old = (self.ops, self.lanes, self.access, self.atomic, self.wrote, self.op_io)
        self.ops, self.lanes, self.access, self.atomic, self.wrote, self.op_io = [], [], [], [], [], []
        for pos, row in enumerate(zip(*old)):
            for dst, item in zip((self.ops, self.lanes, self.access, self.atomic, self.wrote, self.op_io), row):
                dst.append(item)
            for kind, desc, name, reads, atomic in extra.get(pos, ()):
                self.keep.append(desc)
                self.ops.append((kind, 0, desc, name, 0.0))
                self.lanes.append(row[1] & 0xff00)
                self.access.append((self.spans(reads), []))
                self.atomic.append(self.spans(atomic))
                self.wrote.append([])
                self.op_io.append(None)

    def check_stream_ordering(self):
        def overlap(a, b):
            return any(x0 < y1 and y0 < x1 for x0, x1 in a for y0, y1 in b)
        bad, seen = [], []
        active = {}
        forks, joins = {}, []
        for pos, (kind, _, desc, name, _) in enumerate(self.ops):
            flags = self.lanes[pos]
            lane, join, sync = (flags >> 8) & 0xff, bool(flags & OP_JOIN), bool(flags & OP_SYNC)
            if lane > 0:
                if not active.get(lane) or sync:
                    forks.setdefault(lane, []).append(pos)
                    active[lane] = True
            elif join:
                joins.append(pos)
                active = {}
            reads, writes = self.access[pos]
            atomic = self.atomic[pos]
            for p0, l0, n0, r0, w0, a0 in seen:
                if l0 == lane or not (overlap(w0, reads) or overlap(w0, writes) or overlap(r0, writes) or overlap(a0, reads) or
                                      overlap(a0, writes) or overlap(w0, atomic) or overlap(r0, atomic)):
                    continue
                j = [q for q in joins if p0 < q <= pos]
                if l0 == 0:
                    ok = any(p0 < f <= pos for f in forks.get(lane, []))
                elif lane == 0:
                    ok = bool(j)
                else:
                    ok = bool(j) and any(min(j) <= f <= pos for f in forks.get(lane, []))
# ... 29 lines not shown
```

### ground-plane-polling_amd/keras_retinanet_3D/models/retinanet.py

```python

import ctypes
import json
import os

import numpy as np

from ..backend import hip
from ..layers import conv as C
from ..layers import mobilenet as M
from ..layers.filter_detections import MAX_DETECTIONS, NMS_THRESHOLD, SCORE_THRESHOLD
from ..utils import anchors as anchor_utils
from ..utils.gpp_utils import POLL_THRESHOLD, POSE_SCORE_THRESHOLD
from . import weights as W
from .plan import (BlockDesc, CandidatePixelsDesc, DensePoolDesc, DetectDesc, PlanOp, PollDesc, PoolDesc, PoseDesc,
                   PreactDesc, RaggedPoolDesc, RaggedStemDesc, ReluDesc, StemDesc, TailDesc,
                   OP_STEM, OP_MAXPOOL, OP_CONV, OP_RELU, OP_DETECT, OP_POLL, OP_TAIL, OP_BLOCK,
                   OP_DETECT_CANDIDATES, OP_DETECT_SELECT, OP_DETECT_EMIT, OP_DETECT_OSF, OP_STEM_POOL,
                   OP_MAXPOOL_PAD, OP_AVGPOOL, OP_CONV_PREACT, OP_MOBILENET_STEM, OP_MOBILENET_BLOCK, OP_POSE,
                   OP_ABSMAX, OP_ABSMAX_CLEAR, OP_STEM_RAGGED, OP_STEM_POOL_RAGGED, OP_MAXPOOL_RAGGED,
                   OP_DETECT_CANDIDATE_PIXELS, DETECT_OPS, OP_JOIN, OP_SYNC,
                   PlanOptions, block_form, part_of, TOWER_SLICES, RANGE_AUDIT_THRESHOLD, X3_QUANTUM,
                   SPARSE_HEADS_MAX_SHARE, audit_report, SparseHeads, Plan)


class RetinaNet3D(object):

    def __init__(self, weights, backbone_name='resnet50', dtype='f16x3', nms=True, class_specific_filter=True,
                 orientation_specific_filter=False, name='retinanet-bbox', on_range_event=None, plan=None, pose=False, range_audit=False):
        import torch
        self.audit = bool(range_audit)
        if self.audit and dtype != 'f16x3':
            raise ValueError("range_audit=True watches the lower range of dtype='f16x3', got dtype={!r}: the IEEE-half pair is a fixed-point "
                             "number with a quantum of 2^-24 below 2^-14; bf16 halves keep float32's exponent and have no such regime, "
                             "and the other types store no split halves".format(dtype))
        self.small_magnitude_events = 0
        self.last_range_audit = None
        self._last_plan = None
        self.pose = bool(pose)
        self.plan_mode = plan or os.environ.get('GPP_PLAN', 'throughput')
        if self.plan_mode not in ('throughput', 'latency'):
            raise ValueError("plan must be 'throughput' or 'latency', got {!r}".format(self.plan_mode))
        self.on_range_event = on_range_event or os.environ.get('GPP_ON_RANGE_EVENT', 'f32')
        if self.on_range_event not in ('f32', 'raise', 'ignore'):
            raise ValueError("on_range_event must be 'f32', 'raise' or 'ignore', got {!r}".format(self.on_range_event))
        self.range_fallbacks = 0
        self._twin = None
        self._weights = weights if (dtype == 'f16x3' and self.on_range_event == 'f32') else None
        self.class_specific_filter = class_specific_filter
        self.osf = bool(orientation_specific_filter)
        self.nms = bool(nms)
        self.name = name
        self.mobilenet = W.is_mobilenet(backbone_name)
        self.backbone_name = backbone_name if self.mobilenet else backbone_name.split('_')[0]
        self.densenet = W.is_densenet(self.backbone_name)
        if self.backbone_name not in W.BLOCKS and not self.densenet and not self.mobilenet:
            raise ValueError('Backbone (\'{}\') not in allowed backbones ({}).'.format(
                backbone_name, sorted(W.BLOCKS) + sorted(W.DENSENET_BLOCKS) + ['{}_<{}>'.format(r, '|'.join(str(a) for a in W.MOBILENET_ALPHAS))
                                                                              for r in W.MOBILENET_ROWS]))
        if dtype not in ('bf16', 'f16', 'f32', 'bf16x3', 'f16x3'):
            raise ValueError("dtype must be 'bf16', 'f16', 'f32', 'bf16x3' or 'f16x3', got {!r}".format(dtype))
        if self.densenet and dtype not in ('f32', 'f16x3', 'bf16x3'):
            raise ValueError("a DenseNet backbone runs with dtype 'f32', 'f16x3' or 'bf16x3', got {!r}".format(dtype))
        if self.mobilenet and dtype not in ('f32', 'f16x3', 'bf16x3'):
            raise ValueError("a MobileNet backbone runs with dtype 'f32', 'f16x3' or 'bf16x3', got {!r}".format(dtype))
        self.dtype = dtype
        self.esz = C.elem_size(dtype)
        self.tdtype = C.torch_dtype(dtype)
        self.device = hip.require_device()
        hip.lib()
        self.torch = torch
        self._plans = {}
        self._anchors = {}
        self._taps, self._ragged_taps = {}, {}
        self._tuned = {}
        self.stem_x3 = False
        self._load_tune_cache()
        self._upload(weights)
        self.tag_names = []

    def _upload(self, weights):
        torch, dev = self.torch, self.device
        W.validate_weights(weights, self.backbone_name)
        self.conv_w = {}
        self.conv_scale = {}

        def put(name, kernel, bias):
            self.conv_w[name] = (C.pack_weight(kernel, self.dtype, dev), torch.as_tensor(bias).to(dev).contiguous(),
                                 kernel.shape)
            if self.dtype == 'f16x3':
                self.conv_scale[name] = C.out_scale_of(kernel, dev)

        if self.densenet:
            self._upload_densenet(weights, put)
        if self.mobilenet:
            self._upload_mobilenet(weights)
        for conv, bn, kh, kw, cin, cout, _ in (() if self.densenet or self.mobilenet else W.backbone_layers(self.backbone_name)):
            k, b = W.folded_conv(weights, conv, bn)
            if k.shape != (kh, kw, cin, cout):
                raise ValueError('weight {} has shape {}, expected {}'.format(conv, k.shape, (kh, kw, cin, cout)))
            if conv == 'conv1':
                if self.dtype in C.X3_TYPES and os.environ.get('GPP_X3_STEM', 'mfma') != 'valu':
                    self.stem_w = hip.pack_stem_weights_x3(k.reshape(147, 64), dev)
                    self.stem_x3 = True
                elif self.esz == 4:
                    self.stem_w = torch.as_tensor(np.ascontiguousarray(k.reshape(147, 64), dtype=np.float32)).to(dev).contiguous()
# ... 227 lines not shown
            d = M.block_desc(x, y, dw_w, dw_b, pw_w, pw_b, scale, stride, self.dtype)
            plan.emit(OP_MOBILENET_BLOCK, d, 'conv_pw_{}'.format(i), [x], [y], flops=M.block_flops(d), io=([x], [y], None))
            x = y
            if i in W.MOBILENET_TAPS:
                feats.append(x)
        return feats

    def _pyramid(self, plan, opts, B, H, Wd, C3, C4, C5):
        got = [(C3.H, C3.W), (C4.H, C4.W), (C5.H, C5.W)]
        shapes = anchor_utils.pyramid_shapes_of_features(got) if self.densenet else anchor_utils.pyramid_shapes((H, Wd))
        if got != [tuple(s) for s in shapes[:3]]:
            raise RuntimeError('backbone / pyramid shape mismatch: {} vs {}'.format(got, shapes))
        pix = [h * w for h, w in shapes]
        total = sum(pix)
        plan.n_anchors = total * anchor_utils.NUM_BASE_ANCHORS
        x3s = opts.x3_level >= 1

        def pyramid(c, dtype=None):
            buf = self.torch.empty((B, total, c), dtype=dtype or self.tdtype, device=self.device)
            plan.keep.append(buf)
            sp = x3s and dtype is None
            return buf, [C.FMap(buf, B, h, w, c, off=sum(pix[:i]) * c, bstride=total * c, split=sp, half=self.dtype if sp else 'bf16x3')
                         for i, (h, w) in enumerate(shapes)]
        return shapes, pyramid

    def _fpn(self, plan, opts, C3, C4, C5, pyramid, smap):
        _, P = pyramid(512)
        l_p5, l_p6 = (1, 2) if opts.fpn_lanes else (0, 0)
        T5 = smap(C5.H, C5.W, 512)
        self._conv(plan, 'C5_reduced', [C5], [T5], 1, join=bool(plan.open_lanes))
        self._conv(plan, 'P5', [T5], [P[2]], 3, pad=(1, 1), lane=l_p5)
        self._conv(plan, 'P6', [C5], [P[3]], 3, stride=2, pad=(C.same_pad(C5.H, 3, 2)[1], C.same_pad(C5.W, 3, 2)[1]), lane=l_p6)
        R6 = smap(P[3].H, P[3].W, 512)
        relu_d = ReluDesc(P[3].buf.data_ptr() + P[3].off * self.esz, R6.buf.data_ptr(), P[3].bstride, R6.bstride, P[3].H * P[3].W * 512,
                          C.gpp_dtype(self.dtype) if opts.x3_level >= 1 else C.gpp_storage_dtype(self.dtype), P[3].B)
        plan.emit(OP_RELU, relu_d, 'C6_relu', [P[3]], [R6], lane=l_p6)
        plan.relu_io = (P[3], R6)
        self._conv(plan, 'P7', [R6], [P[4]], 3, stride=2, pad=(C.same_pad(P[3].H, 3, 2)[1], C.same_pad(P[3].W, 3, 2)[1]), lane=l_p6)
        T4 = smap(C4.H, C4.W, 512)
        self._conv(plan, 'C4_reduced', [C4], [T4], 1, residuals=[T5])
        self._conv(plan, 'P4', [T4], [P[1]], 3, pad=(1, 1), lane=opts.p4_lane, sync=bool(opts.p4_lane))
        T3 = smap(C3.H, C3.W, 512)
        self._conv(plan, 'C3_reduced', [C3], [T3], 1, residuals=[T4])
        self._conv(plan, 'P3', [T3], [P[0]], 3, pad=(1, 1))
        return P

    def _detect(self, plan, B, anchors, pyramid):
        torch, dev, D = self.torch, self.device, MAX_DETECTIONS
        f32, i32 = torch.float32, torch.int32
        plan.cls_logits, cls_o = pyramid(96, f32)
        plan.regression, reg_o = pyramid(144, f32)
        plan.regression_dim, dim_o = pyramid(36, f32)
        plan.boxes = torch.empty((B, D, 12), dtype=f32, device=dev)
        plan.dimensions = torch.empty((B, D, 3), dtype=f32, device=dev)
        plan.scores = torch.empty((B, D), dtype=f32, device=dev)
        plan.labels = torch.empty((B, D), dtype=i32, device=dev)
        plan.orientations = torch.empty((B, D), dtype=i32, device=dev)
        plan.anchor_index = torch.empty((B, D), dtype=i32, device=dev)
        plan.counts = torch.zeros((B,), dtype=i32, device=dev)
        need = hip.c_size_t(0)
        if self.osf and B > 16:
            raise ValueError('orientation_specific_filter=True handles at most 16 images per batch')
        size_fn = hip.lib().gpp_detect_osf_workspace_bytes if self.osf else hip.lib().gpp_detect_workspace_bytes
        hip.check(size_fn(B, plan.n_anchors, need), 'gpp_detect_workspace_bytes')
        plan.detect_ws = ws = torch.empty((int(need.value),), dtype=torch.uint8, device=dev)
        plan.anchors = anchors
        dd = DetectDesc(plan.cls_logits.data_ptr(), plan.regression.data_ptr(), plan.regression_dim.data_ptr(),
                        anchors.data_ptr(), plan.boxes.data_ptr(), plan.dimensions.data_ptr(), plan.scores.data_ptr(),
                        plan.labels.data_ptr(), plan.orientations.data_ptr(), plan.anchor_index.data_ptr(),
                        plan.counts.data_ptr(), ws.data_ptr(), ws.numel(), plan.n_anchors,
                        B, anchor_utils.NUM_BASE_ANCHORS, 1, D, SCORE_THRESHOLD, NMS_THRESHOLD if self.nms else 2.0)
        heads = [plan.cls_logits, plan.regression, plan.regression_dim]
        dets = [plan.boxes, plan.dimensions, plan.scores, plan.labels, plan.orientations, plan.anchor_index]
        access = {OP_DETECT_CANDIDATES: ([plan.cls_logits], [ws, plan.counts]), OP_DETECT_SELECT: ([ws, plan.regression], [ws]),
                  OP_DETECT_EMIT: (heads + [ws], dets)}

        def decode(kind, name='filtered_detections', **flags):
            reads, writes = access.get(kind, (heads, dets + [ws, plan.counts]))
            if kind == OP_DETECT_CANDIDATE_PIXELS:
                sp = plan.sparse
                lists = hip.PixelListDesc(ws.data_ptr(), sp.bitmap.data_ptr(), sp.rows.data_ptr(), sp.counts.data_ptr(), sp.flag.data_ptr(),
                                          plan.n_anchors, B, anchor_utils.NUM_BASE_ANCHORS, 4 if self.osf else 1, len(sp.level_pixels),
                                          sp.max_rows, 0, (ctypes.c_int32 * hip.GPP_MAX_GROUPS)(*sp.level_pixels), 0)
                reads, writes = access[OP_DETECT_CANDIDATES]
                plan.emit(kind, CandidatePixelsDesc(ctypes.addressof(dd), lists), name, reads, writes + sp.tensors(), inner=(dd,), **flags)
                return
            plan.emit(kind, dd, name, reads, writes, **flags)
        return (cls_o, reg_o, dim_o), decode

    def _heads(self, plan, opts, P, pyramid, outs, decode):
        cls_o, reg_o, dim_o = outs
        _, wide = pyramid(896)
        self._conv(plan, 'pyramid_towers_0', P, wide, 3, pad=(1, 1), relu=True, join=True)

        def tower(prefix, width, c0, out_name, out, tag=0, lane=0, join=False):
            src = [C.FMap(m.buf, m.B, m.H, m.W, width, off=m.off + c0, bstride=m.bstride, pitch=m.pitch, split=m.split, half=m.half)
                   for m in wide]
            for i in range(1, 4):
                _, dst = pyramid(width)
                self._conv(plan, '{}_{}'.format(prefix, i), src, dst, 3, pad=(1, 1), relu=True, tag=tag, lane=lane)
                src = dst
            out_layer(out_name, src, out, lane, join)

        def out_layer(name, src, out, lane, join):
            sp = plan.sparse
            kh, kw, cin, cout = self.conv_w[name][2]
            pixels = sum(f.H * f.W for f in out)
            split = (C.latency_split if self.plan_mode == 'latency' else C.default_split)(kh, kw, cin, cout, pixels)
            if sp is None or name == 'pyramid_classification' or lane or split > 1:
                self._conv(plan, name, src, out, 3, pad=(1, 1), out_f32=True, lane=lane, join=join)
                if sp is not None and join and not lane:
                    sp.lists_joined = True
                return
            dense = self._desc(plan, name, src, out, 3, pad=(1, 1), out_f32=True, lane=lane)
            dense.guard, dense.guard_value = sp.flag.data_ptr(), 1
            plan.emit(OP_CONV, dense, name, list(src) + [sp.flag], out, flops=C.conv_flops(dense), lane=lane, join=join or not sp.lists_joined,
                      io=(src, out, None))
            sp.lists_joined = True
            rows = self._desc(plan, name, src, out, 3, pad=(1, 1), out_f32=True, lane=lane)
            rows.gather_rows, rows.gather_counts, rows.split_k = sp.rows.data_ptr(), sp.counts.data_ptr(), 1
            rows.guard, rows.guard_value = sp.flag.data_ptr(), 0
            plan.emit(OP_CONV, rows, name, list(src) + [sp.rows, sp.counts, sp.flag], out, lane=lane, io=(src, out, None))
            sp.dense.append(dense)
            sp.gathered.append(rows)

        l_dim, l_cls = (1, 2) if opts.head_lanes else (0, 0)
        towers = {'cls': ('pyramid_classification', 256, 512, 'pyramid_classification', cls_o, 0, l_cls or opts.cls_lane),
                  'reg': ('pyramid_regression', 512, 0, 'pyramid_regression_ops', reg_o, 1, 0, bool(opts.cls_lane)),
                  'dim': ('pyramid_regression_dim', 128, 768, 'pyramid_regression_dim', dim_o, 0, l_dim)}
        if opts.sparse_heads:
            plan.sparse = SparseHeads(self.torch, self.device, P[0].B, [m.H * m.W for m in P], opts.sparse_heads)
            plan.keep += plan.sparse.tensors()
        if opts.decode_overlap:
            tower(*towers['cls'])
            decode(OP_DETECT_CANDIDATE_PIXELS if plan.sparse else OP_DETECT_CANDIDATES, 'filtered_detections/candidates',
                   lane=opts.cls_lane or 1)
            tower(*towers['reg'])
            decode(OP_DETECT_SELECT, 'filtered_detections/select', lane=1, sync=True)
            tower(*towers['dim'])
            decode(OP_DETECT_EMIT, join=True)
        else:
            for t in ('dim', 'cls', 'reg'):
                tower(*towers[t])
            decode(OP_DETECT_OSF if self.osf else OP_DETECT, join=True)

    def _poll(self, plan, B, n_planes, planes_batched):
        torch, dev, D = self.torch, self.device, MAX_DETECTIONS
        plan.keypoints = torch.empty((B, D, 4, 3), dtype=torch.float32, device=dev)
        plan.keyplanes = torch.empty((B, D, 1, 4), dtype=torch.float32, device=dev)
        plan.residuals = torch.empty((B, D), dtype=torch.float32, device=dev)
        plan.best_index = torch.empty((B, D), dtype=torch.int32, device=dev)
        need = hip.c_size_t(0)
        hip.check(hip.lib().gpp_poll_workspace_bytes(B, n_planes, int(planes_batched), need), 'gpp_poll_workspace_bytes')
        plan.poll_ws = torch.empty((max(int(need.value), 16),), dtype=torch.uint8, device=dev)
        pd = PollDesc(plan.boxes.data_ptr(), plan.dimensions.data_ptr(), plan.orientations.data_ptr(), plan.P_inv.data_ptr(),
                      plan.planes.data_ptr(), plan.keypoints.data_ptr(), plan.keyplanes.data_ptr(), plan.residuals.data_ptr(),
                      plan.best_index.data_ptr(), plan.poll_ws.data_ptr(), plan.poll_ws.numel(), B, D, n_planes,
                      int(planes_batched), POLL_THRESHOLD, 0)
        plan.emit(OP_POLL, pd, 'fit_road_planes', [plan.boxes, plan.dimensions, plan.orientations, plan.P_inv, plan.planes],
                  [plan.keypoints, plan.keyplanes, plan.residuals, plan.best_index, plan.poll_ws], tag=2,
                  flops=162.0 * B * D * n_planes)

    def _pose(self, plan, B):
        torch, dev, D = self.torch, self.device, MAX_DETECTIONS
        n = B * D * hip.GPP_POSE_COLS
        plan.pose_out = torch.zeros((n + 2 + B,), dtype=torch.float32, device=dev)
        plan.pose_rows = plan.pose_out[:n].view(B, D, hip.GPP_POSE_COLS)
        plan.pose_counts = plan.pose_out[n + 2:].view(torch.int32)
        plan.frame_info = torch.tensor([[1.0, plan.shape[1], plan.shape[2]]] * B, dtype=torch.float32, device=dev)
        pd = PoseDesc(plan.boxes.data_ptr(), plan.dimensions.data_ptr(), plan.scores.data_ptr(), plan.labels.data_ptr(),
                      plan.orientations.data_ptr(), plan.keypoints.data_ptr(), plan.residuals.data_ptr(), plan.frame_info.data_ptr(),
                      plan.pose_rows.data_ptr(), plan.pose_counts.data_ptr(), B, D, POSE_SCORE_THRESHOLD, 0)
        plan.emit(OP_POSE, pd, 'recover_pose', [plan.boxes, plan.dimensions, plan.scores, plan.labels, plan.orientations, plan.keypoints,
                                                plan.residuals, plan.frame_info], [plan.pose_rows, plan.pose_counts])

    def _audit(self, plan):
        torch, esz = self.torch, self.esz
        views, order = {}, []

        def key_of(f):
            return (f.buf.data_ptr(), f.pitch, f.off % f.pitch, f.C)

        for pos, (kind, _, desc, name, _) in enumerate(plan.ops):
            io = plan.op_io[pos]
            if kind == OP_CONV_PREACT:
                lo, hi = min(a for a, _ in Plan.spans(io[0])), max(b for _, b in Plan.spans(io[0]))
                plan.audit_unobserved.append({'name': name + '/operand', 'consumers': [name], 'extent': (lo, hi),
                                              'reason': 'max(x * scale + shift, 0) is formed after the load (gpp_conv2d_preact)'})
            elif kind == OP_MOBILENET_BLOCK:
                plan.audit_unobserved.append({'name': name.replace('conv_pw_', 'conv_dw_'), 'consumers': [name], 'extent': None,
                                              'reason': 'the depthwise result lives in LDS (gpp_mobilenet_block); bounded by ReLU6'})
            elif kind == OP_CONV:
                for f in list(io[0]) + list(io[2] or []):
                    k = key_of(f)
                    if k not in views:
                        views[k] = {'consumers': [], 'producers': [], 'channels': f.C, 'spans': [], 'fmaps': [], 'split': f.split,
                                    'layout': 'split_f16' if f.split else 'f32'}
                        order.append(k)
                    if name not in views[k]['consumers']:
                        views[k]['consumers'].append(name)
                    views[k]['spans'] += Plan.span(f)
                    if not any((g.off, g.B, g.H, g.W) == (f.off, f.B, f.H, f.W) for g in views[k]['fmaps']):
                        views[k]['fmaps'].append(f)
        offset = 0
        for k in order:
            views[k]['row'] = (offset, k[3])
            offset += k[3]
        plan.audit_table = table = torch.zeros((max(offset, 1),), dtype=torch.int32, device=self.device)
        extra = {}
        for pos, (kind, _, desc, name, _) in enumerate(plan.ops):
            for k in order:
                ptr, pitch, c0, c = k
                outs = [o for o in plan.wrote[pos] if o.buf.data_ptr() == ptr and o.pitch == pitch]
                if not outs:
                    continue
                oc0, oc = outs[0].off % pitch, outs[0].C
                lo, hi = max(c0, oc0), min(c0 + c, oc0 + oc)
                if lo >= hi:
                    continue
                v = views[k]
                if name not in v['producers']:
                    v['producers'].append(name)
                runs = []
                for start, n in sorted(((o.off - oc0 + b * o.bstride) // pitch, o.H * o.W) for o in outs for b in range(o.B)):
                    if runs and runs[-1][0] + runs[-1][1] == start:
                        runs[-1][1] += n
                    else:
                        runs.append([start, n])
                row = table[v['row'][0] + lo - c0:v['row'][0] + hi - c0]
                for start, n in runs:
                    d = hip.AbsmaxDesc(ptr + start * pitch * esz, row.data_ptr(), n, pitch, hi - lo, lo,
                                       hip.GPP_ABSMAX_SPLIT_F16 if v['split'] else hip.GPP_ABSMAX_F32, 0)
                    extra.setdefault(pos, []).append((OP_ABSMAX, d, 'absmax:' + name, outs, [row]))
        plan.insert_behind(extra)
        plan.keep.append(table)
        clear = hip.AbsmaxClearDesc(table.data_ptr(), table.numel())
        plan.emit(OP_ABSMAX_CLEAR, clear, 'absmax:clear', [], [table])
        for lst in (plan.ops, plan.lanes, plan.access, plan.atomic, plan.wrote, plan.op_io):
            lst.insert(0, lst.pop())
        for k in order:
            v = views[k]
            names = v['producers']
            if not names:
                raise RuntimeError('range audit: no launch of the plan writes the operand of {}'.format(v['consumers']))
            name = TOWER_SLICES.get((names[0], k[2]), names[0]) if len(names) == 1 else \
                '+'.join(sorted(names)) if len(names) <= 5 else '{}..{}'.format(names[0], names[-1])
            plan.audit_maps.append({'name': name, 'producers': names, 'consumers': v['consumers'], 'channels': v['channels'],
                                    'layout': v['layout'], 'row': v['row'], 'fmaps': v['fmaps'],
                                    'extent': (min(a for a, _ in v['spans']), max(b for _, b in v['spans']))})

    def _bind_workspaces(self, plan):
        plan.workspaces = {lane: self.torch.empty((max(need, 16),), dtype=self.torch.uint8, device=self.device)
                           for lane, need in plan.ws_need.items()}
        for d, lane in plan.conv_descs:
            d.partial = plan.workspaces[lane].data_ptr()
            d.partial_bytes = plan.workspaces[lane].numel()

    def _plan_options(self, B):
        env = os.environ.get
        x3 = self.dtype in C.X3_TYPES
        x3_level = int(env('GPP_X3_SPLIT', '2')) if x3 else 0
        chunks = env('GPP_STAGE_CHUNKS')
        fuse_tail = [int(v) for v in env('GPP_FUSE_TAIL', '64,128').split(',') if v.strip() and int(v) > 0]
        if x3:
            fuse_tail = [v for v in fuse_tail if v == 64] if x3_level >= 2 else []
        elif self.esz == 4:
            fuse_tail = []
        fuse_block = [int(v) for v in env('GPP_FUSE_BLOCK', '64,128').split(',') if v.strip()] if (x3 and x3_level >= 2) else []
        if self.audit:
            fuse_tail, fuse_block = [], []
        head_lanes = env('GPP_HEAD_LANES', '0') != '0'
        fpn_lanes = head_lanes or env('GPP_FPN_LANES', '1') != '0'
        overlap = env('GPP_DECODE_OVERLAP', '1') != '0' and not head_lanes and not self.osf
        return PlanOptions(
            x3_level=x3_level,
            fuse_stem_pool=not self.densenet and not self.mobilenet and (self.esz == 2 or self.stem_x3) and env('GPP_FUSE_STEM_POOL', '1') != '0',
            stage_chunks=tuple(max(1, min(B, int(v))) for v in chunks.split(',')) if chunks else (B,) * 4,
            half_stages=frozenset(int(v) for v in env('GPP_HALF_LANES', '0,1,2,3').split(',') if v.strip()) if B >= 2 else frozenset(),
            fuse_tail=tuple(v for v in fuse_tail if v in (64, 128)),
            fuse_block=tuple(v for v in fuse_block if v in (64, 128)),
            fuse_block_proj=env('GPP_FUSE_BLOCK_PROJ', '0') != '0',
            br1_lane=env('GPP_BR1_LANE', '1') != '0',
            fpn_lanes=fpn_lanes,
            p4_lane=1 if (fpn_lanes and env('GPP_P4_LANE', '1') != '0') else 0,
            head_lanes=head_lanes,
            decode_overlap=overlap,
            cls_lane=2 if (overlap and env('GPP_CLS_LANE', '1' if B <= 2 else '0') != '0') else 0,
            autotune=env('GPP_AUTOTUNE', '1') != '0',
            sparse_heads=(max(1e-9, float(env('GPP_SPARSE_HEADS_MAX_SHARE', SPARSE_HEADS_MAX_SHARE)))
                          if (overlap and not self.audit and env('GPP_SPARSE_HEADS', '1') != '0') else 0.0),
            tune_key='x3split={};fuse={}/{};plan={}{}'.format(env('GPP_X3_SPLIT', '2'), env('GPP_FUSE_TAIL', '64,128'), env('GPP_FUSE_BLOCK', '64,128'),
                                                              self.plan_mode, C.latency_split_config() if self.plan_mode == 'latency' else '') +
                     (';audit' if self.audit else ''))

    def _build(self, B, H, Wd, n_planes, planes_batched, ragged=False):
        torch, dev = self.torch, self.device
        if ragged:
            if self.mobilenet or self.densenet:
                raise ValueError('{} has no ragged form: {}; run its images grouped by shape'.format(
                    self.backbone_name, 'its first block runs at conv1\'s resolution, which differs inside a height class' if self.mobilenet
                    else 'its zero-padded pool1 (gpp_maxpool3x3s2_pad_f32) has no per-image form'))
            if self.audit:
                raise ValueError('range_audit=True has no ragged form: the audit of the conv1 map reads rows that a shorter image does not have')
            if H % 4:
                raise ValueError('the canvas of a ragged plan has 4 Hp rows, got {}'.format(H))
        opts = self._plan_options(B)
        plan = Plan()
        plan.shape = (B, H, Wd, n_planes, planes_batched)
        plan.ragged = bool(ragged)
        if ragged:
            plan.heights = torch.full((B,), H, dtype=torch.int32, device=dev)
            plan.heights_host = [H] * B
        plan.side_lanes = {'fpn': opts.fpn_lanes, 'branch1': opts.br1_lane, 'p4': bool(opts.p4_lane),
                           'half_batch_stages': sorted(opts.half_stages), 'cls_tower': bool(opts.cls_lane)}
        plan.decode_overlap = opts.decode_overlap
        plan.range_slot = torch.zeros((1,), dtype=torch.int64, device=dev)
        plan.range_seen = 0
        plan.images = torch.empty((B, H, Wd, 3), dtype=torch.float32, device=dev)
        plan.P_inv = torch.empty((B, 4, 3), dtype=torch.float32, device=dev)
        plan.planes = torch.empty((B, n_planes, 4) if planes_batched else (n_planes, 4), dtype=torch.float32, device=dev)

        def fmap(h, w, c, split=False):
            f = C.FMap.empty(B, h, w, c, self.tdtype, dev, half=self.dtype if self.dtype in C.X3_TYPES else 'bf16x3')
            plan.keep.append(f.buf)
            return f.mark_split() if split else f

        backbone = self._densenet_backbone if self.densenet else self._mobilenet_backbone if self.mobilenet else self._resnet_backbone
        C2, C3, C4, C5 = backbone(plan, opts, B, H, Wd, fmap, lambda h, w, c: fmap(h, w, c, opts.x3_level >= 2))
        plan.features = {'stem': plan.stem_out, 'C2': C2, 'C3': C3, 'C4': C4, 'C5': C5}
        shapes, pyramid = self._pyramid(plan, opts, B, H, Wd, C3, C4, C5)
        P = self._fpn(plan, opts, C3, C4, C5, pyramid, lambda h, w, c: fmap(h, w, c, opts.x3_level >= 1))
        plan.features.update({'P{}'.format(i + 3): P[i] for i in range(5)})
        outs, decode = self._detect(plan, B, self._anchor_table((H, Wd), shapes if self.densenet else None), pyramid)
        self._heads(plan, opts, P, pyramid, outs, decode)
        self._poll(plan, B, n_planes, planes_batched)
        if self.pose:
            self._pose(plan, B)
        if self.audit:
            self._audit(plan)
        self._bind_workspaces(plan)
        plan.finalize()
        plan.tagged = [name for _, tag, _, name, _ in plan.ops if tag]
        if opts.autotune:
            self._autotune(plan)
        return plan

    def _tune_cache_path(self):
        return os.environ.get('GPP_TUNE_CACHE')

    def _tune_config(self):
        ver = hip.lib().gpp_version().decode().split('src:')[-1]
        return 'v2;{};{}'.format(ver, self._plan_options(1).tune_key)

    def _load_tune_cache(self):
        path = self._tune_cache_path()
        if path and os.path.exists(path):
            with open(path) as f:
                for key, val in json.load(f).items():
                    parts = key.split('|')
                    if len(parts) != 7:
                        continue
                    cfg, bb, dt, name, b, h, w = parts
                    if cfg == self._tune_config() and bb == self.backbone_name and dt == self.dtype:
                        self._tuned[(name, int(b), int(h), int(w))] = (int(val[0]), float(val[-1]))

    def _save_tune_cache(self):
        path = self._tune_cache_path()
        if not path or int(os.environ.get('RANK', '0')) != 0:
            return
        data = {}
        if os.path.exists(path):
            try:
                with open(path) as f:
                    data = json.load(f)
            except ValueError:
                data = {}
        for (name, b, h, w), val in self._tuned.items():
            data['|'.join([self._tune_config(), self.backbone_name, self.dtype, name, str(b), str(h), str(w)])] = list(val)
        tmp = '{}.tmp.{}'.format(path, os.getpid())
        with open(tmp, 'w') as f:
            json.dump(data, f, indent=0, sort_keys=True)
        os.replace(tmp, path)

    def _autotune(self, plan):
        self._require_hip()
        H, Wd = plan.shape[1:3]
        plan.images.uniform_(-120.0, 130.0)
        fresh = False
        plan.tuning = {}
        rnd = None
        if os.environ.get('GPP_TUNE_RANDOM'):
            import random
            rnd = random.Random(int(os.environ['GPP_TUNE_RANDOM']) * 1000003 + int(os.environ.get('RANK', '0')))
        for index, (kind, _, desc, name, flops) in enumerate(plan.ops):
            if kind in DETECT_OPS or kind == OP_POLL:
                continue
            gathered = kind == OP_CONV and bool(desc.gather_rows)
            if kind == OP_CONV and desc.guard:
                plan.sparse.flag.fill_(0 if gathered else 1)
                if gathered:
                    plan.sparse.put_every_nth(self.torch)
                    name = name + '@rows'
            self.run_op(plan, index)
            if kind not in (OP_CONV, OP_TAIL, OP_CONV_PREACT, OP_MOBILENET_BLOCK):
                continue
            target = plan.inner[id(desc)][0] if kind == OP_CONV_PREACT else desc
            field = 'tile_rows' if kind == OP_TAIL else 'tile_hint'
            if rnd is not None:
                setattr(target, field, rnd.choice(self._tile_choices(plan, index, kind, target)))
                plan.tuning[name] = (int(getattr(target, field)), 0.0)
                self.run_op(plan, index)
                continue
            key = (name, target.B if kind == OP_MOBILENET_BLOCK else (plan.inner[id(desc)][0] if kind == OP_TAIL else target).batch, H, Wd)
            if kind == OP_CONV and key in self._tuned and not self._tile_is_listed(desc, self._tuned[key][0]):
                del self._tuned[key]
            if key not in self._tuned:
                self._tuned[key] = self._time_tiles(plan, index, kind, desc, target, flops)
                fresh = True
            setattr(target, field, self._tuned[key][0])
            plan.tuning[name] = self._tuned[key]
            plan.tuning_parts.setdefault(name, []).append(self._tuned[key])
        if plan.sparse is not None:
            plan.sparse.reset(self.torch)
        self.torch.cuda.synchronize()
        if fresh:
            self._save_tune_cache()

    def _tile_choices(self, plan, index, kind, target):
        if kind == OP_TAIL:
            return (64, 96, 128, 160) if self.dtype in C.X3_TYPES else (96, 128, 160)
        lib, tiles, count = hip.lib(), (ctypes.c_int * 32)(), ctypes.c_int(0)
        if kind == OP_MOBILENET_BLOCK:
            hip.check(lib.gpp_mobilenet_block_tile_candidates(ctypes.byref(target), tiles, 16, ctypes.byref(count)),
                      'gpp_mobilenet_block_tile_candidates')
            return list(tiles[:min(count.value, 16)])
        if kind == OP_CONV_PREACT:
            hip.check(lib.gpp_conv2d_preact_tile_candidates(ctypes.byref(target), tiles, 16, ctypes.byref(count)),
                      'gpp_conv2d_preact_tile_candidates')
            return list(tiles[:min(count.value, 16)])
        hip.check(lib.gpp_conv2d_tile_candidates(ctypes.byref(target), tiles, 32, ctypes.byref(count)), 'gpp_conv2d_tile_candidates')
        ok = []
        for tile in tiles[:count.value]:
            target.tile_hint = tile
            if lib.gpp_plan_run(ctypes.byref(plan.array, index * ctypes.sizeof(PlanOp)), 1, hip.stream_ptr(), None, 0) == 0:
                ok.append(tile)
        return ok

    def _time_tiles(self, plan, index, kind, desc, target, flops):
        if kind == OP_TAIL:
            times = {}
            for rows in self._tile_choices(plan, index, kind, target):
                if rows == 64 and os.environ.get('GPP_TAIL64', '1') == '0':
                    continue
                desc.tile_rows = rows
                e0, e1 = self.torch.cuda.Event(enable_timing=True), self.torch.cuda.Event(enable_timing=True)
                self.run_op(plan, index)
                e0.record()
                for _ in range(16):
                    self.run_op(plan, index)
                e1.record()
                e1.synchronize()
                times[rows] = e0.elapsed_time(e1) * 1000.0 / 16
            rows = min(times, key=times.get)
            return rows, round(times[rows], 2)
        slow = self.dtype == 'f32'
        iters = (2 if slow else 6) if flops > 5e10 else (4 if slow else 16)
        best = ctypes.c_float(0.0)
        if kind == OP_MOBILENET_BLOCK:
            hip.check(hip.lib().gpp_mobilenet_block_autotune(ctypes.byref(target), iters, hip.stream_ptr(), ctypes.byref(best)),
                      'gpp_mobilenet_block_autotune')
        elif kind == OP_CONV_PREACT:
            hip.check(hip.lib().gpp_conv2d_preact_autotune(ctypes.byref(target), desc.in_scale, desc.in_shift, iters, hip.stream_ptr(),
                                                           ctypes.byref(best)), 'gpp_conv2d_preact_autotune')
        else:
            hip.check(hip.lib().gpp_conv2d_autotune(ctypes.byref(target), iters, hip.stream_ptr(), ctypes.byref(best)), 'gpp_conv2d_autotune')
        return int(target.tile_hint), round(float(best.value), 2)

    @staticmethod
    def _tile_is_listed(desc, tile):
        tiles, count = (ctypes.c_int * 64)(), ctypes.c_int(0)
        hip.check(hip.lib().gpp_conv2d_tile_candidates(ctypes.byref(desc), tiles, 64, ctypes.byref(count)), 'gpp_conv2d_tile_candidates')
        return int(tile) in list(tiles[:min(count.value, 64)])

    def x3_range_events(self, reset=False):
        if self.dtype != 'f16x3':
            return 0
        self.torch.cuda.synchronize()
        total = 0
        for plan in self._plans.values():
            total += int(plan.range_slot.item())
            if reset:
                plan.range_slot.zero_()
                plan.range_seen = 0
        if reset:
            self.torch.cuda.synchronize()
        return total

    def note_range(self, plan, count):
        if count == plan.range_seen:
            return False
        plan.range_seen = count
        return True

    def plan_for(self, B, H, Wd, n_planes, planes_batched, ragged=False):
        key = (int(B), int(H), int(Wd), int(n_planes), bool(planes_batched))
        if ragged:
            key = (key[0], ('class', key[1] // 4), key[2], key[3], key[4])
        if key not in self._plans:
            self._plans[key] = self._build(int(B), int(H), *key[2:], **({'ragged': True} if ragged else {}))
        self._last_plan = self._plans[key]
        return self._plans[key]

    def put_heights(self, plan, heights):
        from ..utils import image as image_utils
        if not getattr(plan, 'ragged', False):
            raise ValueError('put_heights: not a ragged plan')
        B, rows = plan.shape[0], plan.shape[1]
        lo, hi = image_utils.class_height_range(rows // 4)
        h = [int(v) for v in np.asarray(heights).reshape(-1)]
        if len(h) != B or any(v < lo or v > hi for v in h):
            raise ValueError('heights {} do not fit the plan: {} images of height {}..{} (class Hp = {})'.format(h, B, lo, hi, rows // 4))
        plan.heights_host = h
        plan.heights.copy_(self.torch.as_tensor(np.asarray(h, dtype=np.int32)), non_blocking=True)

    def _require_hip(self):
        if self.device.type != 'cuda':
            raise hip.GppError('the model was built on {}: its plans do not run'.format(self.device))

    def run_op(self, plan, index):
        self._require_hip()
        hip.check(hip.lib().gpp_plan_run(ctypes.byref(plan.array, index * ctypes.sizeof(PlanOp)), 1, hip.stream_ptr(), None, 0), 'gpp_plan_run')

    def run_plan(self, plan, events=None):
        self._require_hip()
        plan.heads_stale = plan.sparse is not None
        if events is None and getattr(plan, 'graph', None) is not None:
            plan.graph.replay()
            return
        if events is not None:
            arr = (ctypes.c_void_p * len(events))(*events)
            rc = hip.lib().gpp_plan_run(plan.array, len(plan.ops), hip.stream_ptr(), arr, len(events))
        else:
            rc = hip.lib().gpp_plan_run(plan.array, len(plan.ops), hip.stream_ptr(), None, 0)
        hip.check(rc, 'gpp_plan_run')

    def capture(self, plan):
        self._require_hip()
        torch = self.torch
        self.run_plan(plan)
        torch.cuda.synchronize()
        graph = torch.cuda.CUDAGraph()
        plan.heads_stale = plan.sparse is not None
        with torch.cuda.graph(graph):
            rc = hip.lib().gpp_plan_run(plan.array, len(plan.ops), hip.stream_ptr(), None, 0)
        hip.check(rc, 'gpp_plan_run (capture)')
        plan.graph = graph
        return graph

    def outputs(self, plan):
# ... 392 lines not shown
```

### include/gpp.h

```cpp
#ifndef GPP_H_
#define GPP_H_

#include <stddef.h>
#include <stdint.h>

#ifdef __cplusplus
extern "C" {
#endif

#define GPP_OK 0
#define GPP_ERR_BAD_ARG (-1)
#define GPP_ERR_WORKSPACE (-2)
#define GPP_ERR_ALIGN (-3)
#define GPP_ERR_UNSUPPORTED (-4)

const char* gpp_version(void);

int gpp_poll_workspace_bytes(int B, int N, int planes_batched, size_t* bytes);

int gpp_poll_f32(const float* boxes, const float* dims, const int32_t* orient, const float* P_inv,
                 const float* planes, int B, int D, int N, int planes_batched, float thr,
                 float* keypoints, float* keyplanes, float* residuals, int32_t* best_idx,
                 void* workspace, size_t workspace_bytes, void* stream);


#define GPP_BF16 1
#define GPP_F16 2
#define GPP_F32 3
#define GPP_BF16X3 4
#define GPP_F16X3 5

#define GPP_MAX_GROUPS 5

typedef struct gpp_conv_group {
    int64_t in_off, in_bstride;
    int64_t out_off, out_bstride;
    int64_t res_off, res_bstride;
    int32_t H_in, W_in, H_out, W_out;
    int32_t H_res, W_res;
    int32_t tile_start;
    int32_t row_begin;
} gpp_conv_group;

typedef struct gpp_conv_desc {
    const void* in;
    const void* weight;
    const float* bias;
    const void* residual;
    void* out;
    const void* zero_page;
    int32_t dtype;
    int32_t out_f32;
    int32_t batch, C_in, C_out, KH, KW, stride, pad_top, pad_left;
    int32_t in_pitch, out_pitch, res_pitch;
    int32_t weight_rows;
    int32_t relu;
    int32_t n_groups;
    int32_t tile_hint;
    int32_t reserved;
    int32_t in_bytes, weight_bytes;
    void* partial;
    int64_t partial_bytes;
    int32_t split_k;
    int32_t partial_rows;
    gpp_conv_group groups[GPP_MAX_GROUPS];
    int32_t x3_split;
    int32_t reserved2;
    const float* out_scale;
    uint64_t* range_counter;
    const int32_t* gather_rows;
    const int32_t* gather_counts;
    const int32_t* guard;
    int32_t guard_value;
    int32_t reserved3;
} gpp_conv_desc;
#define GPP_X3_IN 1
#define GPP_X3_OUT 2
#define GPP_X3_RES 4

int gpp_conv2d_igemm(const gpp_conv_desc* host_desc, void* stream);

int gpp_conv2d_split_rule(const gpp_conv_desc* host_desc, int* split_k);
int gpp_conv2d_workspace_bytes(const gpp_conv_desc* host_desc, size_t* bytes);

int gpp_conv2d_autotune(gpp_conv_desc* desc, int iters, void* stream, float* best_us);

int gpp_conv2d_tile_candidates(const gpp_conv_desc* host_desc, int* tiles, int capacity, int* count);

int gpp_bottleneck_tail(const gpp_conv_desc* conv3x3, const gpp_conv_desc* conv1x1, int tile_rows, void* stream);

int gpp_bottleneck_block(const gpp_conv_desc* conv1x1_a, const gpp_conv_desc* conv3x3_b, const gpp_conv_desc* conv1x1_c, int tile, void* stream);

int gpp_x3_range_events(uint64_t* host_count, int reset);

int gpp_x3_range_snapshot(uint64_t* device_count, void* stream);

int gpp_x3_range_snapshot_of(const uint64_t* counter, uint64_t* device_count, void* stream);

int gpp_conv2d_flops(const gpp_conv_desc* host_desc, double* flops);

int gpp_conv2d_preact(const gpp_conv_desc* host_desc, const float* in_scale, const float* in_shift, void* stream);
int gpp_conv2d_preact_tile_candidates(const gpp_conv_desc* host_desc, int* tiles, int capacity, int* count);
int gpp_conv2d_preact_autotune(gpp_conv_desc* desc, const float* in_scale, const float* in_shift, int iters, void* stream, float* best_us);
int gpp_maxpool3x3s2_pad_f32(const float* in, float* out, int B, int H, int W, int C, int pad, int out_pitch, void* stream);
int gpp_avgpool2x2_f32(const float* in, float* out, int B, int H, int W, int C, int out_pitch, void* stream);

typedef struct gpp_mobilenet_block_desc {
    const float* in; const float* dw_weight; const float* dw_bias; const void* pw_weight; const float* pw_bias; const float* out_scale;
    float* out;
    int32_t dtype, B, H, W, C_in, C_out, stride, in_pitch, out_pitch, weight_rows, tile_hint, reserved;
} gpp_mobilenet_block_desc;
typedef struct gpp_mobilenet_stem_desc { const float* in; const float* weight; const float* bias; float* out; int32_t B, H, W, C_out, out_pitch, reserved; } gpp_mobilenet_stem_desc;
int gpp_mobilenet_block(const gpp_mobilenet_block_desc* host_desc, void* stream);
int gpp_mobilenet_block_tile_candidates(const gpp_mobilenet_block_desc* host_desc, int* tiles, int capacity, int* count);
int gpp_mobilenet_block_autotune(gpp_mobilenet_block_desc* desc, int iters, void* stream, float* best_us);
int gpp_mobilenet_stem(const float* in, const float* weight, const float* bias, float* out, int B, int H, int W, int C_out, int out_pitch,
                       void* stream);
int gpp_mobilenet_depthwise(const float* in, const float* weight, const float* bias, float* out, int B, int H, int W, int C, int stride,
                            int in_pitch, int out_pitch, void* stream);

int gpp_stem_conv7x7_bn_relu(const float* in, const float* weight, const float* bias, void* out, int dtype,
                             int B, int H, int W, void* stream);
int gpp_stem_pack_weights_f16(const float* host_weight_147x64, void* host_packed, size_t packed_bytes);
int gpp_stem_conv7x7_bn_relu_mfma(const float* in, const void* packed_weight_f16, const float* bias, void* out,
                                  int dtype, int B, int H, int W, void* stream);
int gpp_maxpool3x3s2_same(const void* in, void* out, int dtype, int B, int H, int W, int C, void* stream);
int gpp_stem_pool_fused_mfma(const float* in, const void* packed_weight_f16, const float* bias, void* out,
                             int dtype, int B, int H, int W, void* stream);
int gpp_stem_pack_weights_f16x3(const float* host_weight_147x64, void* host_packed, size_t packed_bytes);
int gpp_stem_conv7x7_bn_relu_x3(const float* in, const void* packed_weight_x3, const float* bias, float* out,
                                int B, int H, int W, void* stream);
int gpp_stem_conv7x7_bn_relu_x3_rc(const float* in, const void* packed_weight_x3, const float* bias, float* out,
                                   int B, int H, int W, uint64_t* range_counter, void* stream);
int gpp_stem_pool_fused_x3(const float* in, const void* packed_weight_x3, const float* bias, float* out,
                           int B, int H, int W, uint64_t* range_counter, void* stream);
int gpp_stem_conv7x7_bn_relu_ragged(const float* in, const float* weight, const float* bias, void* out, int dtype,
                                    int B, int H, int W, int Hp, const int32_t* heights, void* stream);
int gpp_stem_conv7x7_bn_relu_mfma_ragged(const float* in, const void* packed_weight_f16, const float* bias, void* out,
                                         int dtype, int B, int H, int W, int Hp, const int32_t* heights, void* stream);
int gpp_stem_conv7x7_bn_relu_x3_rc_ragged(const float* in, const void* packed_weight_x3, const float* bias, float* out,
                                          int B, int H, int W, int Hp, const int32_t* heights, uint64_t* range_counter, void* stream);
int gpp_maxpool3x3s2_same_ragged(const void* in, void* out, int dtype, int B, int H, int W, int C, int Hp,
                                 const int32_t* heights, void* stream);
int gpp_stem_pool_fused_mfma_ragged(const float* in, const void* packed_weight_f16, const float* bias, void* out,
                                    int dtype, int B, int H, int W, int Hp, const int32_t* heights, void* stream);
int gpp_stem_pool_fused_x3_ragged(const float* in, const void* packed_weight_x3, const float* bias, float* out,
                                  int B, int H, int W, int Hp, const int32_t* heights, uint64_t* range_counter, void* stream);
int gpp_relu(const void* in, void* out, int dtype, int64_t count, void* stream);
int gpp_relu_strided(const void* in, int64_t in_bstride, void* out, int64_t out_bstride, int dtype, int B,
                     int64_t count, void* stream);

int gpp_preprocess_u8_bgr(const uint8_t* frames, float* out, const int32_t* y0, const int32_t* y1, const float* wy,
                          const int32_t* x0, const int32_t* x1, const float* wx, int B, int H, int W, int Ho, int Wo,
                          float mean_b, float mean_g, float mean_r, void* stream);
int gpp_preprocess_u8_bgr_ragged(const uint8_t* frames, float* out, const int32_t* raw_hw, const int32_t* heights,
                                 const int32_t* y0, const int32_t* y1, const float* wy, const int32_t* x0, const int32_t* x1, const float* wx,
                                 int B, int H, int W, int Hp, int Ho, int Wo, float mean_b, float mean_g, float mean_r, void* stream);

int gpp_detect_workspace_bytes(int B, int64_t n_anchors, size_t* bytes);

int gpp_detect_f32(const float* cls_logits, const float* regression, const float* regression_dim,
                   const float* anchors, int B, int64_t n_anchors, int num_base_anchors, int fused_layout,
                   float score_thr, float iou_thr, int max_det,
                   float* boxes, float* dims, float* scores, int32_t* labels, int32_t* orientations,
                   int32_t* anchor_index, int32_t* counts,
                   void* workspace, size_t workspace_bytes, void* stream);

#define GPP_DETECT_CANDIDATES 1
#define GPP_DETECT_SELECT 2
#define GPP_DETECT_EMIT 4
int gpp_detect_stages_f32(int stages, const float* cls_logits, const float* regression, const float* regression_dim,
                          const float* anchors, int B, int64_t n_anchors, int num_base_anchors, int fused_layout,
                          float score_thr, float iou_thr, int max_det,
                          float* boxes, float* dims, float* scores, int32_t* labels, int32_t* orientations,
                          int32_t* anchor_index, int32_t* counts,
                          void* workspace, size_t workspace_bytes, void* stream);

typedef struct gpp_pixel_list_desc {
    const void* workspace; uint32_t* bitmap; int32_t* rows; int32_t* counts; int32_t* flag;
    int64_t n_anchors;
    int32_t B, num_base_anchors, lists_per_image, n_levels, max_rows, reserved;
    int32_t level_pixels[GPP_MAX_GROUPS]; int32_t reserved2;
} gpp_pixel_list_desc;
int gpp_detect_pixel_lists(const gpp_pixel_list_desc* host_desc, void* stream);

int gpp_detect_osf_workspace_bytes(int B, int64_t n_anchors, size_t* bytes);
int gpp_detect_osf_f32(const float* cls_logits, const float* regression, const float* regression_dim,
                       const float* anchors, int B, int64_t n_anchors, int num_base_anchors, int fused_layout,
                       float score_thr, float iou_thr, int max_det,
                       float* boxes, float* dims, float* scores, int32_t* labels, int32_t* orientations,
                       int32_t* anchor_index, int32_t* counts,
                       void* workspace, size_t workspace_bytes, void* stream);

int gpp_pack_detections(const float* boxes, const float* dims, const float* scores, const int32_t* labels,
                        const int32_t* orientations, const float* keypoints, const float* keyplanes,
                        const float* residuals, int B, int D, float* packed, void* stream);

#define GPP_POSE_COLS 36
int gpp_pose_f32(const float* boxes, const float* dims, const float* scores, const int32_t* labels,
                 const int32_t* orientations, const float* keypoints, const float* residuals,
                 const float* frame_info, int B, int D, float score_thr,
                 float* rows, int32_t* counts, void* stream);

#define GPP_EVAL_MAX_DETECTIONS 1024
#define GPP_EVAL_MAX_ANNOTATIONS 1024
#define GPP_EVAL_ANN_COLS 17
#define GPP_EVAL_ERR_COLS 11
int gpp_eval_match_f32(const float* boxes, const float* dims, const float* scores, const int32_t* labels,
                       const int32_t* orientations, const float* scales, const double* annotations,
                       const int32_t* ann_counts, int B, int D, int A, int num_classes, float score_thr,
                       int max_detections, double iou_thr, int32_t* table, double* errors, int32_t* counts, void* stream);

#define GPP_KITTI_MAX_DETECTIONS 128
#define GPP_KITTI_MAX_LABELS 128
#define GPP_KITTI_MAX_THRESHOLDS 41
#define GPP_KITTI_LABEL_COLS 16
int gpp_kitti_overlaps_f64(const float* rows, const double* labels, const int32_t* label_counts, int B, int D, int A,
                           double* overlaps, void* stream);
int gpp_kitti_stats_f64(const float* rows, const double* labels, const int32_t* label_counts, const double* overlaps,
                        const double* min_overlap, const float* thresholds, const int32_t* n_thresholds, int B, int D, int A, int T,
                        float* tp_scores, int32_t* n_gt, int32_t* stats, double* similarity, void* stream);

#define GPP_LABEL_MOD_COLS 20
int gpp_label_prep_f64(const double* labels, const int32_t* label_counts, const double* P, const double* trig, int B, int A,
                       unsigned det_types, int own_box, double* mod,
                       float* boxes, float* dims, float* scores, int32_t* det_labels, int32_t* orientations, void* stream);

#define GPP_DRAW_PRIM_WORDS 16
#define GPP_DRAW_PRIMS_PER_DET 26
#define GPP_DRAW_COUNT_WORDS 4
#define GPP_DRAW_CAPTION_MAX 20
#define GPP_DRAW_NONE 0
#define GPP_DRAW_LINE 1
#define GPP_DRAW_DASHED 2
#define GPP_DRAW_RECT 3
#define GPP_DRAW_CIRCLE 4
#define GPP_DRAW_CAPTION 5
int gpp_draw_workspace_bytes(int B, int D, size_t* prims_bytes, size_t* workspace_bytes);
int gpp_draw_build(const float* rows, const double* P, int B, int D, float score_thr, void* prims, int32_t* counts, void* stream);
int gpp_draw_raster(const uint8_t* frames_u8, const int32_t* raw_hw, int Hr, int Wr, const void* prims, const int32_t* counts,
                    int B, uint8_t* out_u8, void* workspace, void* stream);

#define GPP_ABSMAX_F32 1
#define GPP_ABSMAX_SPLIT_F16 2
#define GPP_ABSMAX_SPLIT_BF16 3
typedef struct gpp_absmax_desc {
    const void* in; uint32_t* out;
    int64_t M, pitch;
    int32_t C, c_off, layout, reserved;
} gpp_absmax_desc;
typedef struct gpp_absmax_clear_desc { uint32_t* table; int64_t n; } gpp_absmax_clear_desc;
int gpp_channel_absmax(const gpp_absmax_desc* desc, void* stream);
int gpp_absmax_clear(uint32_t* table, int64_t n, void* stream);

#define GPP_OP_STEM 1
#define GPP_OP_MAXPOOL 2
#define GPP_OP_CONV 3
#define GPP_OP_RELU 4
#define GPP_OP_DETECT 5
#define GPP_OP_POLL 6
#define GPP_OP_BOTTLENECK_TAIL 7
#define GPP_OP_DETECT_CANDIDATES 8
#define GPP_OP_DETECT_SELECT 9
#define GPP_OP_DETECT_EMIT 10
#define GPP_OP_DETECT_OSF 12
// ... 80 lines not shown
```

Baseline: 825.7.

## Run last regression tower conv sparsely over dilated candidate pixel rows

Adds a sparse tower path. The last 3x3 conv of the regression tower is computed only on a dilated set of candidate pixels taken from the class head, with a guarded fallback to the dense conv when the list is too large. It also adds a pipelined gathered-row x3 conv kernel that picks its row tile size on device from the live counts, plus autotuning of the row tile. This is meant to skip most of the regression tower work when detections are sparse, at the cost of extra list-building, an extra launch and more code paths that have to stay correct.

After: 857.9 (median of 6 runs). +3.9%, better.

```diff
diff --git a/ground-plane-polling_amd/csrc/conv_igemm.hip b/ground-plane-polling_amd/csrc/conv_igemm.hip
--- a/ground-plane-polling_amd/csrc/conv_igemm.hip
+++ b/ground-plane-polling_amd/csrc/conv_igemm.hip
@@ -32,9 +32,15 @@
     if (d.reserved != 0) return GPP_ERR_BAD_ARG;
 #endif
     if (d.reserved2 != 0 || (d.x3_split & ~(GPP_X3_IN | GPP_X3_OUT | GPP_X3_RES))) return GPP_ERR_BAD_ARG;
-    if (d.reserved3 != 0 || (d.gather_rows != nullptr) != (d.gather_counts != nullptr)) return GPP_ERR_BAD_ARG;
-    if (((uintptr_t)d.gather_rows | (uintptr_t)d.gather_counts | (uintptr_t)d.guard) & 3) return GPP_ERR_ALIGN;
-    if (d.gather_rows && (d.stride != 1 || d.residual || !d.out_f32 || d.split_k > 1)) return GPP_ERR_UNSUPPORTED;
+    if (d.reserved3 != 0 || d.reserved4 != 0 || (d.gather_rows != nullptr) != (d.gather_counts != nullptr)) return GPP_ERR_BAD_ARG;
+    const bool tower = d.tower_rows || d.tower_counts || d.tower_flag;
+    if (tower && (!d.tower_rows || !d.tower_counts || !d.tower_flag || d.gather_rows || d.guard)) return GPP_ERR_BAD_ARG;
+    if (!tower && d.tower_tile != 0) return GPP_ERR_BAD_ARG;
+    if (((uintptr_t)d.gather_rows | (uintptr_t)d.gather_counts | (uintptr_t)d.guard | (uintptr_t)d.tower_rows | (uintptr_t)d.tower_counts |
+         (uintptr_t)d.tower_flag) & 3)
+        return GPP_ERR_ALIGN;
+    if (d.gather_rows && (d.stride != 1 || d.residual || d.split_k > 1)) return GPP_ERR_UNSUPPORTED;
+    if (((d.gather_rows && !d.out_f32) || tower) && !gpp_tiles::gather_pipe_can_run(d)) return GPP_ERR_UNSUPPORTED;
     if (d.x3_split && !is_x3(d.dtype)) return GPP_ERR_BAD_ARG;
     if (d.out_scale && d.dtype != GPP_F16X3) return GPP_ERR_BAD_ARG;
     if ((d.x3_split & GPP_X3_OUT) && (d.out_f32 || d.C_out % 32 != 0 || d.out_pitch % 32 != 0)) return GPP_ERR_UNSUPPORTED;
@@ -95,6 +101,18 @@
         if (d.split_k > 1) return GPP_ERR_UNSUPPORTED;
         return gpp_conv_gather_dispatch(d, st);
     }
+    if (d.tower_rows) {
+        if (d.split_k > 1) return GPP_ERR_UNSUPPORTED;
+        gpp_conv_desc rows = d, dense = d;
+        rows.gather_rows = d.tower_rows; rows.gather_counts = d.tower_counts; rows.tile_hint = d.tower_tile;
+        rows.guard = d.tower_flag; rows.guard_value = 0;
+        dense.guard = d.tower_flag; dense.guard_value = 1;
+        rows.tower_rows = rows.tower_counts = rows.tower_flag = dense.tower_rows = dense.tower_counts = dense.tower_flag = nullptr;
+        rows.tower_tile = dense.tower_tile = 0;
+        const int rc_rows = gpp_conv_gather_dispatch(rows, st);
+        if (rc_rows != GPP_OK) return rc_rows;
+        return dispatch_any(dense, st);
+    }
     switch (d.dtype) {
         case GPP_BF16: return gpp_conv_dispatch_bf16(d, st);
         case GPP_F16: return gpp_conv_dispatch_f16(d, st);
@@ -111,7 +129,7 @@
     int rc = validate(d1);
     if (rc == GPP_OK) rc = validate(d2);
     if (rc != GPP_OK) return rc;
-    if (d1.gather_rows || d2.gather_rows || d1.guard || d2.guard) return GPP_ERR_UNSUPPORTED;
+    if (d1.gather_rows || d2.gather_rows || d1.guard || d2.guard || d1.tower_rows || d2.tower_rows) return GPP_ERR_UNSUPPORTED;
     const gpp_conv_group &G1 = d1.groups[0], &G2 = d2.groups[0];
     if (d1.dtype == GPP_F32) return GPP_ERR_UNSUPPORTED;
     if (is_x3(d1.dtype) && (!(d1.x3_split & GPP_X3_IN) || (d2.x3_split & (GPP_X3_OUT | GPP_X3_RES)) != (GPP_X3_OUT | GPP_X3_RES) || !d2.residual))
@@ -143,7 +161,7 @@
     if (rc == GPP_OK) rc = validate(d2);
     if (rc == GPP_OK) rc = validate(d3);
     if (rc != GPP_OK) return rc;
-    if (d1.gather_rows || d2.gather_rows || d3.gather_rows || d1.guard || d2.guard || d3.guard) return GPP_ERR_UNSUPPORTED;
+    if (d1.gather_rows || d2.gather_rows || d3.gather_rows || d1.guard || d2.guard || d3.guard || d1.tower_rows || d2.tower_rows || d3.tower_rows) return GPP_ERR_UNSUPPORTED;
     const gpp_conv_group &G1 = d1.groups[0], &G2 = d2.groups[0], &G3 = d3.groups[0];
     if (!is_x3(d1.dtype) || d1.dtype != d2.dtype || d1.dtype != d3.dtype) return GPP_ERR_UNSUPPORTED;
     if (d1.n_groups != 1 || d2.n_groups != 1 || d3.n_groups != 1 || d1.batch != d2.batch || d1.batch != d3.batch) return GPP_ERR_UNSUPPORTED;
@@ -258,7 +276,8 @@
 {
     using namespace gpp_tiles;
     const gpp_conv_desc& d = *desc;
-    if ((d.gather_rows != nullptr) != (t.form == GATHER)) return t.code == 0;
+    const int gform = !d.gather_rows ? -1 : (d.out_f32 ? (int)GATHER : (int)GATHER_PIPE);
+    if ((gform >= 0 || t.form == GATHER || t.form == GATHER_PIPE) && t.form != gform) return t.code == 0 && gform >= 0;
     const bool x3_in = is_x3(d.dtype) && (d.x3_split & GPP_X3_IN);
     if (!owner_has(t.owner, f32_storage(d.dtype), is_x3(d.dtype))) return false;
     if (is_x3(d.dtype) && x3_wants_split_input(t.form, t.owner) && !x3_in && t.owner != ALL_X3IN) return false;
@@ -273,6 +292,7 @@
     const auto pads_less_than = [&](int other) { return (d.C_out + bn - 1) / bn * bn < (d.C_out + other - 1) / other * other; };
     switch (t.form) {
         case GATHER: return bn != 160 || pads_less_than(64);
+        case GATHER_PIPE: return gather_pipe_can_run(d);
         case DEEP: {
             int64_t tiles_m = 0;
             for (int g = 0; g < d.n_groups; ++g) tiles_m += ((int64_t)d.batch * d.groups[g].H_out * d.groups[g].W_out + t.bm - 1) / t.bm;
@@ -392,7 +412,7 @@
     if (((uintptr_t)in_scale | (uintptr_t)in_shift) & 15) return GPP_ERR_ALIGN;
     if (d.KH != 1 || d.KW != 1 || d.stride != 1 || d.pad_top != 0 || d.pad_left != 0) return GPP_ERR_UNSUPPORTED;
     if (d.x3_split & GPP_X3_IN) return GPP_ERR_UNSUPPORTED;
-    if (d.gather_rows || d.guard) return GPP_ERR_UNSUPPORTED;
+    if (d.gather_rows || d.guard || d.tower_rows) return GPP_ERR_UNSUPPORTED;
     if (d.C_in > 4096) return GPP_ERR_UNSUPPORTED;
     return GPP_OK;
 }
diff --git a/ground-plane-polling_amd/csrc/conv_igemm_impl.h b/ground-plane-polling_amd/csrc/conv_igemm_impl.h
--- a/ground-plane-polling_amd/csrc/conv_igemm_impl.h
+++ b/ground-plane-polling_amd/csrc/conv_igemm_impl.h
@@ -375,13 +375,15 @@
 
 constexpr int stage_rows(int BM, int NW) { return (BM + 8 * NW - 1) / (8 * NW) * (8 * NW); }
 
-template <int DT, int BM, int BN, int WM, int WN, int STAGES, bool PIPE, bool XIN = false, bool PRE = false, bool GATHER = false>
+template <int DT, int BM, int BN, int WM, int WN, int STAGES, bool PIPE, bool XIN = false, bool PRE = false, bool GATHER = false, bool GLIVE = false>
 __device__ __forceinline__ void conv_igemm_body(const gpp_conv_desc& d, const int block_x, const int grid_x, const float* pre_s = nullptr,
                                                 const float* pre_t = nullptr)
 {
     static_assert(!XIN || kX3<DT>, "pre-split input maps: GPP_BF16X3 / GPP_F16X3");
     static_assert(!PRE || (!PIPE && !XIN && kF32Storage<DT>), "pre-activation: float32-sized input maps, plain loop");
-    static_assert(!GATHER || (!PIPE && !PRE), "gathered rows: plain loop");
+    static_assert(!GATHER || !PRE, "gathered rows: no pre-activation");
+    static_assert(!(GATHER && PIPE) || (kX3<DT> && XIN && GLIVE), "gathered rows on the pipelined loop: x3 types, pre-split maps, tiles over the listed rows");
+    static_assert(!GLIVE || GATHER, "tiles over the listed rows: the gathered form");
     if (d.guard != nullptr && *(const volatile int32_t*)d.guard != d.guard_value) return;
     using E = Elem<DT>;
     using vec8 = typename E::vec8;
@@ -411,14 +413,19 @@
     int tile_start = 0, row_begin = 0, H_in = 0, W_in = 0, H_out = 0, W_out = 0, H_res = 0, W_res = 0;
     int64_t in_off = 0, in_bs = 0, out_off = 0, out_bs = 0, res_off = 0, res_bs = 0;
     int list_begin = 0, list_next = 0, group = 0;
+    int live_start = 0;
 #pragma unroll
     for (int q = 0; q < GPP_MAX_GROUPS; ++q) {
+        const int first_tile = GLIVE ? live_start : d.groups[q].tile_start;
         if constexpr (GATHER) {
-            if (q < d.n_groups && mt >= d.groups[q].tile_start) { list_begin = list_next; group = q; }
+            if (q < d.n_groups && mt >= first_tile) { list_begin = list_next; group = q; }
             if (q < d.n_groups) list_next += d.batch * d.groups[q].H_out * d.groups[q].W_out;
         }
-        if (q < d.n_groups && mt >= d.groups[q].tile_start) {
-            tile_start = d.groups[q].tile_start;
+        if constexpr (GLIVE) {
+            if (q < d.n_groups) live_start += (min(max(d.gather_counts[q], 0), d.batch * d.groups[q].H_out * d.groups[q].W_out) + BM - 1) / BM;
+        }
+        if (q < d.n_groups && mt >= first_tile) {
+            tile_start = first_tile;
             row_begin = d.groups[q].row_begin;
             H_in = d.groups[q].H_in; W_in = d.groups[q].W_in;
             H_out = d.groups[q].H_out; W_out = d.groups[q].W_out;
@@ -1041,6 +1048,35 @@
     conv_igemm_body<DT, BM, BN, WM, WN, STAGES, false, XIN, false, true>(d, blockIdx.x, gridDim.x);
 }
 
+template <int DT, int BM>
+__device__ __forceinline__ void conv_gather_pipe_tiles(const gpp_conv_desc& d, const int live)
+{
+    for (int t = blockIdx.x; t < live; t += gridDim.x) {
+        conv_igemm_body<DT, BM, 256, 2, 4, 2, true, true, false, true, true>(d, t, live);
+        __syncthreads();
+    }
+}
+
+template <int DT>
+__global__ __launch_bounds__(512, 2) void conv_gather_pipe_kernel(const gpp_conv_desc d, const int rows)
+{
+    if (d.guard != nullptr && *(const volatile int32_t*)d.guard != d.guard_value) return;
+    int counts[GPP_MAX_GROUPS];
+#pragma unroll
+    for (int q = 0; q < GPP_MAX_GROUPS; ++q)
+        counts[q] = q < d.n_groups ? min(max(d.gather_counts[q], 0), d.batch * d.groups[q].H_out * d.groups[q].W_out) : 0;
+    const int bm = __builtin_amdgcn_readfirstlane(rows ? rows : gpp_tiles::gather_pipe_rows(counts, d.n_groups, d.C_out / 256));
+    const int live = __builtin_amdgcn_readfirstlane((int)gpp_tiles::gather_pipe_tiles(counts, d.n_groups, d.C_out / 256, bm));
+    switch (bm) {
+        case 128: conv_gather_pipe_tiles<DT, 128>(d, live); break;
+        case 160: conv_gather_pipe_tiles<DT, 160>(d, live); break;
+        case 192: conv_gather_pipe_tiles<DT, 192>(d, live); break;
+        case 224: conv_gather_pipe_tiles<DT, 224>(d, live); break;
+        case 256: conv_gather_pipe_tiles<DT, 256>(d, live); break;
+        default: break;
+    }
+}
+
 template <int DT, int BM, int BN, int WM, int WN>
 __global__ __launch_bounds__(64 * WM * WN, 2) void conv_preact_kernel(const gpp_conv_desc d, const float* in_scale, const float* in_shift)
 {
@@ -2118,10 +2154,33 @@
     return last_launch_rc();
 }
 
+template <int DT>
+int launch_gather_pipe(gpp_conv_desc& d, int rows, hipStream_t st)
+{
+    if constexpr (!kX3<DT>) {
+        return kF32Storage<DT> ? GPP_ERR_UNSUPPORTED : GPP_ERR_BAD_ARG;
+    } else {
+        constexpr int BN = 256;
+        if (!gpp_tiles::gather_pipe_can_run(d)) return GPP_ERR_UNSUPPORTED;
+        constexpr int lds = 2 * (gpp_tiles::kGatherPipeMaxRows + BN) * kRowBytes;
+        constexpr auto kernel = conv_gather_pipe_kernel<DT>;
+        const int rc = allow_lds<kernel>(lds);
+        if (rc != GPP_OK) return rc;
+        const int ok = prepare<gpp_tiles::kGatherPipeMinRows, BN>(d);
+        if (ok < 0) return ok;
+        const int bm = rows ? rows : gpp_tiles::kGatherPipeMinRows;
+        int64_t tiles = 0;
+        for (int g = 0; g < d.n_groups; ++g) tiles += ((int64_t)d.batch * d.groups[g].H_out * d.groups[g].W_out + bm - 1) / bm;
+        tiles *= d.C_out / BN;
+        kernel<<<dim3((unsigned)(tiles < gpp_tiles::kGatherPipeCus ? tiles : gpp_tiles::kGatherPipeCus)), dim3(512), lds, st>>>(d, rows);
+        return last_launch_rc();
+    }
+}
+
 template <int DT, int FORM, int OWNER, int BM, int BN, int WM, int WN, int STAGES>
 int run_tile(gpp_conv_desc& d, hipStream_t st)
 {
-    if constexpr (FORM == gpp_tiles::GATHER) {
+    if constexpr (FORM == gpp_tiles::GATHER || FORM == gpp_tiles::GATHER_PIPE) {
         return GPP_ERR_BAD_ARG;
     } else if constexpr (!gpp_tiles::owner_has(OWNER, kF32Storage<DT>, kX3<DT>)) {
         return kF32Storage<DT> ? GPP_ERR_UNSUPPORTED : GPP_ERR_BAD_ARG;
@@ -2138,7 +2197,8 @@
 #define GPP_RUN_TILE(code, form, owner, bm, bn, wm, wn, stages) \
     case code: return run_tile<DT, gpp_tiles::form, gpp_tiles::owner, bm, bn, wm, wn, stages>(d, st);
 #define GPP_RUN_GATHER(code, form, owner, bm, bn, wm, wn, stages) \
-    case code: if constexpr (gpp_tiles::form == gpp_tiles::GATHER) return launch_gather<DT, bm, bn, wm, wn, stages>(d, st); else break;
+    case code: if constexpr (gpp_tiles::form == gpp_tiles::GATHER) return d.out_f32 ? launch_gather<DT, bm, bn, wm, wn, stages>(d, st) : GPP_ERR_UNSUPPORTED; \
+               else if constexpr (gpp_tiles::form == gpp_tiles::GATHER_PIPE) return launch_gather_pipe<DT>(d, bm, st); else break;
 #define GPP_RUN_PREACT(code, form, owner, bm, bn, wm, wn, stages) \
     case code: return launch_preact<DT, bm, bn, wm, wn>(d, in_scale, in_shift, st);
 
@@ -2157,7 +2217,7 @@
 int dispatch_gather(gpp_conv_desc& d, hipStream_t st)
 {
     switch (d.tile_hint) {
-        case 0: return launch_gather<DT, 64, 64, 2, 2, 2>(d, st);
+        case 0: return d.out_f32 ? launch_gather<DT, 64, 64, 2, 2, 2>(d, st) : launch_gather_pipe<DT>(d, 0, st);
         GPP_CONV_TILES(GPP_RUN_GATHER, GPP_RUN_GATHER, GPP_TILE_NONE)
         default: break;
     }
diff --git a/ground-plane-polling_amd/csrc/conv_tiles.h b/ground-plane-polling_amd/csrc/conv_tiles.h
--- a/ground-plane-polling_amd/csrc/conv_tiles.h
+++ b/ground-plane-polling_amd/csrc/conv_tiles.h
@@ -16,6 +16,7 @@
     DEEP,
     GATHER,
     PREACT,
+    GATHER_PIPE,
 };
 
 enum Owner {
@@ -83,6 +84,13 @@
     T(7064064, GATHER, ALL, 64, 64, 2, 2, 4)                                                                                             \
     T(7032064, GATHER, ALL, 32, 64, 2, 2, 4)                                                                                             \
     T(7064160, GATHER, ALL, 64, 160, 4, 1, 4)                                                                                            \
+                                                       \
+    T(8000256, GATHER_PIPE, X3IN, 0, 256, 2, 4, 2)                                                                                       \
+    X(8128256, GATHER_PIPE, X3IN, 128, 256, 2, 4, 2)                                                                                     \
+    X(8160256, GATHER_PIPE, X3IN, 160, 256, 2, 4, 2)                                                                                     \
+    X(8192256, GATHER_PIPE, X3IN, 192, 256, 2, 4, 2)                                                                                     \
+    X(8224256, GATHER_PIPE, X3IN, 224, 256, 2, 4, 2)                                                                                     \
+    X(8256256, GATHER_PIPE, X3IN, 256, 256, 2, 4, 2)                                                                                     \
     X(64, PLAIN, ALL, 128, 64, 2, 2, 2)                                                                                                  \
     X(128, PLAIN, ALL, 128, 128, 2, 2, 2)                                                                                                \
     X(256, PLAIN, B16, 256, 128, 4, 2, 3)                                                             \
@@ -107,6 +115,37 @@
     return owner == X3IN || owner == ALL_X3IN || (form != PLAIN && form != GATHER && form != PREACT);
 }
 
+inline bool gather_pipe_can_run(const gpp_conv_desc& d)
+{
+    return (d.dtype == GPP_BF16X3 || d.dtype == GPP_F16X3) && (d.x3_split & (GPP_X3_IN | GPP_X3_OUT)) == (GPP_X3_IN | GPP_X3_OUT) && !d.out_f32 &&
+           d.stride == 1 && !d.residual && d.split_k <= 1 && d.C_out > 0 && d.C_out % 256 == 0;
+}
+
+constexpr int kGatherPipeMinRows = 128, kGatherPipeMaxRows = 256, kGatherPipeCus = 256;
+#if defined(__HIPCC__)
+__host__ __device__
+#endif
+inline long long gather_pipe_tiles(const int (&counts)[GPP_MAX_GROUPS], int n_groups, int n_tiles, int bm)
+{
+    long long tiles = 0;
+    for (int g = 0; g < GPP_MAX_GROUPS; ++g) tiles += g < n_groups ? (counts[g] + bm - 1) / bm : 0;
+    return tiles * n_tiles;
+}
+#if defined(__HIPCC__)
+__host__ __device__
+#endif
+inline int gather_pipe_rows(const int (&counts)[GPP_MAX_GROUPS], int n_groups, int n_tiles)
+{
+    int best = 0;
+    long long best_cost = 0;
+    for (int bm = kGatherPipeMinRows; bm <= kGatherPipeMaxRows; bm += 32) {
+        const long long rounds = (gather_pipe_tiles(counts, n_groups, n_tiles, bm) + kGatherPipeCus - 1) / kGatherPipeCus;
+        const long long cost = rounds * bm * (12416 - 17 * bm);
+        if (best == 0 || cost < best_cost) { best = bm; best_cost = cost; }
+    }
+    return best;
+}
+
 constexpr bool tile_pipelined(int form, int bm, int bn, bool f32_storage) { return form == PIPE || (!f32_storage && form == PLAIN && bm == 256 && bn == 256); }
 
 
diff --git a/ground-plane-polling_amd/csrc/decode.hip b/ground-plane-polling_amd/csrc/decode.hip
--- a/ground-plane-polling_amd/csrc/decode.hip
+++ b/ground-plane-polling_amd/csrc/decode.hip
@@ -673,6 +673,7 @@
     int pix_begin[GPP_MAX_GROUPS];
     int word_begin[GPP_MAX_GROUPS];
     int list_begin[GPP_MAX_GROUPS];
+    int width[GPP_MAX_GROUPS];
 };
 
 __global__ __launch_bounds__(256) void mark_pixels_kernel(const unsigned long long* __restrict__ keys, const int32_t* __restrict__ cnt,
@@ -692,10 +693,42 @@
     }
 }
 
+__global__ __launch_bounds__(256) void dilate_pixels_kernel(const uint32_t* __restrict__ bitmap, const LevelTable T, int B, int total_words,
+                                                            uint32_t* __restrict__ dilated)
+{
+    const int64_t gbit = (int64_t)blockIdx.x * 256 + threadIdx.x;
+    const int word = (int)(gbit >> 5);
+    if (word >= total_words) return;
+    int l = 0;
+    for (int q = 1; q < T.n_levels; ++q) l = word >= T.word_begin[q] ? q : l;
+    const int bit = (int)(gbit - ((int64_t)T.word_begin[l] << 5));
+    const int pix = T.pix[l], W = T.width[l], H = pix / W;
+    bool on = false;
+    if (bit < B * pix) {
+        const int b = bit / pix, p = bit - b * pix;
+        const int y = p / W, x = p - y * W;
+        const uint32_t* words = bitmap + T.word_begin[l];
+        for (int dy = -1; dy <= 1; ++dy) {
+            const int yy = y + dy;
+            if (yy < 0 || yy >= H) continue;
+            for (int dx = -1; dx <= 1; ++dx) {
+                const int xx = x + dx;
+                if (xx < 0 || xx >= W) continue;
+                const int nb = b * pix + yy * W + xx;
+                on |= (words[nb >> 5] >> (nb & 31)) & 1u;
+            }
+        }
+    }
+    const unsigned long long mask = __ballot(on);
+    const int lane = threadIdx.x & 63;
+    if (lane == 0) dilated[word] = (uint32_t)mask;
+    if (lane == 32) dilated[word] = (uint32_t)(mask >> 32);
+}
+
 constexpr int kCompactThreads = 1024;
 __global__ __launch_bounds__(kCompactThreads) void compact_pixels_kernel(uint32_t* __restrict__ bitmap, const LevelTable T, int B, int max_rows,
                                                                          int32_t* __restrict__ rows, int32_t* __restrict__ counts,
-                                                                         int32_t* __restrict__ flag)
+                                                                         int32_t* __restrict__ flag, const int32_t* __restrict__ or_flag)
 {
     __shared__ int wave_sum[kCompactThreads / 64];
     const int tid = threadIdx.x, lane = tid & 63, wave = tid >> 6;
@@ -742,7 +775,7 @@
     }
     if (tid == 0) {
         counts[GPP_MAX_GROUPS] = total;
-        flag[0] = total > max_rows ? 1 : 0;
+        flag[0] = (total > max_rows || (or_flag != nullptr && or_flag[0] != 0)) ? 1 : 0;
     }
 }
 
@@ -758,6 +791,9 @@
     if (d.B == 0) return GPP_OK;
     if (!d.workspace || !d.bitmap || !d.rows || !d.counts || !d.flag) return GPP_ERR_BAD_ARG;
     if (((uintptr_t)d.workspace & 15) || (((uintptr_t)d.bitmap | (uintptr_t)d.rows | (uintptr_t)d.counts | (uintptr_t)d.flag) & 3)) return GPP_ERR_ALIGN;
+    const bool dilate = d.dilated_bitmap || d.dilated_rows || d.dilated_counts || d.dilated_flag;
+    if (dilate && (!d.dilated_bitmap || !d.dilated_rows || !d.dilated_counts || !d.dilated_flag || d.dilated_max_rows < 0)) return GPP_ERR_BAD_ARG;
+    if (((uintptr_t)d.dilated_bitmap | (uintptr_t)d.dilated_rows | (uintptr_t)d.dilated_counts | (uintptr_t)d.dilated_flag) & 3) return GPP_ERR_ALIGN;
     const int lists = d.B * d.lists_per_image;
     if (lists > 64) return GPP_ERR_UNSUPPORTED;
     LevelTable T;
@@ -771,6 +807,8 @@
         T.pix_begin[l] = (int)pixels;
         T.word_begin[l] = (int)words;
         T.list_begin[l] = (int)((int64_t)d.B * pixels);
+        T.width[l] = (dilate && l < d.n_levels) ? d.level_width[l] : 0;
+        if (dilate && l < d.n_levels && (T.width[l] <= 0 || pix % T.width[l] != 0)) return GPP_ERR_BAD_ARG;
         pixels += pix;
         words += ((int64_t)d.B * pix + 31) / 32;
     }
@@ -781,7 +819,14 @@
     const unsigned long long* keys = (const unsigned long long*)(ws + kHeaderBytes);
     mark_pixels_kernel<<<dim3(16, (unsigned)lists), 256, 0, st>>>(keys, cnt, pow2_ceil(d.n_anchors), d.n_anchors, d.num_base_anchors,
                                                                    d.lists_per_image, T, d.bitmap);
-    compact_pixels_kernel<<<1, kCompactThreads, 0, st>>>(d.bitmap, T, d.B, d.max_rows, d.rows, d.counts, d.flag);
+    if (dilate) {
+        const int64_t pairs = (words + 1) / 2;
+        dilate_pixels_kernel<<<dim3((unsigned)((pairs * 64 + 255) / 256)), 256, 0, st>>>(d.bitmap, T, d.B, (int)words, d.dilated_bitmap);
+    }
+    compact_pixels_kernel<<<1, kCompactThreads, 0, st>>>(d.bitmap, T, d.B, d.max_rows, d.rows, d.counts, d.flag, nullptr);
+    if (dilate)
+        compact_pixels_kernel<<<1, kCompactThreads, 0, st>>>(d.dilated_bitmap, T, d.B, d.dilated_max_rows, d.dilated_rows, d.dilated_counts,
+                                                             d.dilated_flag, d.flag);
     const hipError_t e = hipGetLastError();
     return e == hipSuccess ? GPP_OK : (int)e;
 }
diff --git a/ground-plane-polling_amd/keras_retinanet_3D/backend/hip.py b/ground-plane-polling_amd/keras_retinanet_3D/backend/hip.py
--- a/ground-plane-polling_amd/keras_retinanet_3D/backend/hip.py
+++ b/ground-plane-polling_amd/keras_retinanet_3D/backend/hip.py
@@ -67,14 +67,18 @@
                 ('groups', ConvGroup * GPP_MAX_GROUPS),
                 ('x3_split', ctypes.c_int32), ('reserved2', ctypes.c_int32), ('out_scale', c_void_p), ('range_counter', c_void_p),
                 ('gather_rows', c_void_p), ('gather_counts', c_void_p), ('guard', c_void_p),
-                ('guard_value', ctypes.c_int32), ('reserved3', ctypes.c_int32)]
+                ('guard_value', ctypes.c_int32), ('reserved3', ctypes.c_int32),
+                ('tower_rows', c_void_p), ('tower_counts', c_void_p), ('tower_flag', c_void_p),
+                ('tower_tile', ctypes.c_int32), ('reserved4', ctypes.c_int32)]
 
 
 class PixelListDesc(ctypes.Structure):
     _fields_ = [('workspace', c_void_p), ('bitmap', c_void_p), ('rows', c_void_p), ('counts', c_void_p), ('flag', c_void_p),
                 ('n_anchors', c_int64)] + \
                [(n, ctypes.c_int32) for n in ('B', 'num_base_anchors', 'lists_per_image', 'n_levels', 'max_rows', 'reserved')] + \
-               [('level_pixels', ctypes.c_int32 * GPP_MAX_GROUPS), ('reserved2', ctypes.c_int32)]
+               [('level_pixels', ctypes.c_int32 * GPP_MAX_GROUPS), ('reserved2', ctypes.c_int32)] + \
+               [('dilated_bitmap', c_void_p), ('dilated_rows', c_void_p), ('dilated_counts', c_void_p), ('dilated_flag', c_void_p),
+                ('level_width', ctypes.c_int32 * GPP_MAX_GROUPS), ('dilated_max_rows', ctypes.c_int32)]
 
 
 class MobileNetBlockDesc(ctypes.Structure):
diff --git a/ground-plane-polling_amd/keras_retinanet_3D/models/plan.py b/ground-plane-polling_amd/keras_retinanet_3D/models/plan.py
--- a/ground-plane-polling_amd/keras_retinanet_3D/models/plan.py
+++ b/ground-plane-polling_amd/keras_retinanet_3D/models/plan.py
@@ -93,7 +93,8 @@
 
 
 PlanOptions = collections.namedtuple('PlanOptions', 'x3_level fuse_stem_pool stage_chunks half_stages fuse_tail fuse_block fuse_block_proj '
-                                                    'br1_lane fpn_lanes p4_lane head_lanes decode_overlap cls_lane autotune tune_key sparse_heads')
+                                                    'br1_lane fpn_lanes p4_lane head_lanes decode_overlap cls_lane autotune tune_key sparse_heads '
+                                                    'sparse_tower sparse_tower_rounds')
 
 
 def block_form(opts, width, projection, split_input, halves, join):
@@ -115,6 +116,9 @@
 RANGE_AUDIT_THRESHOLD = 2.0 ** -9
 X3_QUANTUM = 2.0 ** -24
 SPARSE_HEADS_MAX_SHARE = '0.5'
+SPARSE_TOWER_MAX_SHARE = '0.75'
+SPARSE_TOWER_MIN_ROUNDS = '1'
+COMPUTE_UNITS = 256
 
 
 def audit_report(maps, table, threshold=RANGE_AUDIT_THRESHOLD):
@@ -140,9 +144,10 @@
 
 class SparseHeads(object):
 
-    def __init__(self, torch, device, B, level_pixels, max_share):
+    def __init__(self, torch, device, B, level_pixels, max_share, level_widths=None, tower_share=0.0):
         i32 = torch.int32
         self.B, self.level_pixels = B, [int(p) for p in level_pixels]
+        self.level_widths = [int(w) for w in level_widths] if level_widths else []
         total = B * sum(self.level_pixels)
         self.max_rows = max(0, min(total, int(max_share * total)))
         self.bitmap = torch.zeros((sum((B * p + 31) // 32 for p in self.level_pixels),), dtype=i32, device=device)
@@ -151,23 +156,37 @@
         self.flag = torch.ones((1,), dtype=i32, device=device)
         self.dense, self.gathered = [], []
         self.lists_joined = False
+        self.tower, self.tower_max_rows = [], 0
+        self.tower_bitmap = self.tower_rows = self.tower_counts = self.tower_flag = self.range_scratch = None
+        if tower_share > 0.0:
+            self.tower_max_rows = max(0, min(total, int(tower_share * total)))
+            self.tower_bitmap = torch.zeros_like(self.bitmap)
+            self.tower_rows = torch.zeros_like(self.rows)
+            self.tower_counts = torch.zeros_like(self.counts)
+            self.tower_flag = torch.ones_like(self.flag)
+            self.range_scratch = torch.zeros((1,), dtype=torch.int64, device=device)
 
     def tensors(self):
-        return [self.bitmap, self.rows, self.counts, self.flag]
-
-    def put_every_nth(self, torch, n=8):
+        own = [self.bitmap, self.rows, self.counts, self.flag]
+        return own + ([self.tower_bitmap, self.tower_rows, self.tower_counts, self.tower_flag] if self.tower_rows is not None else [])
+
+    def put_every_nth(self, torch, n=8, tower=False):
+        rows, cnt = (self.tower_rows, self.tower_counts) if tower else (self.rows, self.counts)
         begin, counts = 0, []
         for p in self.level_pixels:
-            idx = torch.arange(0, self.B * p, n, dtype=torch.int32, device=self.rows.device)
-            self.rows[begin:begin + idx.numel()] = idx
+            idx = torch.arange(0, self.B * p, n, dtype=torch.int32, device=rows.device)
+            rows[begin:begin + idx.numel()] = idx
             counts.append(int(idx.numel()))
             begin += self.B * p
         counts += [0] * (hip.GPP_MAX_GROUPS - len(counts)) + [sum(counts)]
-        self.counts.copy_(torch.as_tensor(counts, dtype=torch.int32))
+        cnt.copy_(torch.as_tensor(counts, dtype=torch.int32))
 
     def reset(self, torch):
         self.counts.zero_()
         self.flag.fill_(1)
+        if self.tower_rows is not None:
+            self.tower_counts.zero_()
+            self.tower_flag.fill_(1)
 
 
 class Plan(object):
@@ -220,6 +239,13 @@
         if self.sparse is None or not self.heads_stale:
             return
         self.heads_stale = False
+        for both in self.sparse.tower:
+            d = type(both).from_buffer_copy(both)
+            d.tower_rows = d.tower_counts = d.tower_flag = None
+            d.tower_tile = 0
+            if d.range_counter:
+                d.range_counter = self.sparse.range_scratch.data_ptr()
+            hip.check(hip.lib().gpp_conv2d_igemm(ctypes.byref(d), hip.stream_ptr()), 'gpp_conv2d_igemm (tower layer completed)')
         for guarded in self.sparse.dense:
             d = type(guarded).from_buffer_copy(guarded)
             d.guard, d.guard_value = None, 0
diff --git a/ground-plane-polling_amd/keras_retinanet_3D/models/retinanet.py b/ground-plane-polling_amd/keras_retinanet_3D/models/retinanet.py
--- a/ground-plane-polling_amd/keras_retinanet_3D/models/retinanet.py
+++ b/ground-plane-polling_amd/keras_retinanet_3D/models/retinanet.py
@@ -20,7 +20,7 @@
                    OP_ABSMAX, OP_ABSMAX_CLEAR, OP_STEM_RAGGED, OP_STEM_POOL_RAGGED, OP_MAXPOOL_RAGGED,
                    OP_DETECT_CANDIDATE_PIXELS, DETECT_OPS, OP_JOIN, OP_SYNC,
                    PlanOptions, block_form, part_of, TOWER_SLICES, RANGE_AUDIT_THRESHOLD, X3_QUANTUM,
-                   SPARSE_HEADS_MAX_SHARE, audit_report, SparseHeads, Plan)
+                   SPARSE_HEADS_MAX_SHARE, SPARSE_TOWER_MAX_SHARE, SPARSE_TOWER_MIN_ROUNDS, COMPUTE_UNITS, audit_report, SparseHeads, Plan)
 
 
 class RetinaNet3D(object):
@@ -414,6 +414,11 @@
                 lists = hip.PixelListDesc(ws.data_ptr(), sp.bitmap.data_ptr(), sp.rows.data_ptr(), sp.counts.data_ptr(), sp.flag.data_ptr(),
                                           plan.n_anchors, B, anchor_utils.NUM_BASE_ANCHORS, 4 if self.osf else 1, len(sp.level_pixels),
                                           sp.max_rows, 0, (ctypes.c_int32 * hip.GPP_MAX_GROUPS)(*sp.level_pixels), 0)
+                if sp.tower_rows is not None:
+                    lists.dilated_bitmap, lists.dilated_rows = sp.tower_bitmap.data_ptr(), sp.tower_rows.data_ptr()
+                    lists.dilated_counts, lists.dilated_flag = sp.tower_counts.data_ptr(), sp.tower_flag.data_ptr()
+                    lists.level_width = (ctypes.c_int32 * hip.GPP_MAX_GROUPS)(*sp.level_widths)
+                    lists.dilated_max_rows = sp.tower_max_rows
                 reads, writes = access[OP_DETECT_CANDIDATES]
                 plan.emit(kind, CandidatePixelsDesc(ctypes.addressof(dd), lists), name, reads, writes + sp.tensors(), inner=(dd,), **flags)
                 return
@@ -430,9 +435,33 @@
                    for m in wide]
             for i in range(1, 4):
                 _, dst = pyramid(width)
-                self._conv(plan, '{}_{}'.format(prefix, i), src, dst, 3, pad=(1, 1), relu=True, tag=tag, lane=lane)
+                if i == 3 and out_name == 'pyramid_regression_ops' and plan.sparse is not None and plan.sparse.tower_rows is not None:
+                    tower_last('{}_{}'.format(prefix, i), src, dst, tag, lane)
+                else:
+                    self._conv(plan, '{}_{}'.format(prefix, i), src, dst, 3, pad=(1, 1), relu=True, tag=tag, lane=lane)
                 src = dst
             out_layer(out_name, src, out, lane, join)
+
+        def tower_last(name, src, dst, tag, lane):
+            sp = plan.sparse
+            d = self._desc(plan, name, src, dst, 3, pad=(1, 1), relu=True, lane=lane)
+            d.tower_rows, d.tower_counts, d.tower_flag = sp.tower_rows.data_ptr(), sp.tower_counts.data_ptr(), sp.tower_flag.data_ptr()
+            plan.emit(OP_CONV, d, name, list(src) + [sp.tower_rows, sp.tower_counts, sp.tower_flag], dst, tag=tag, flops=C.conv_flops(d), lane=lane,
+                      join=not sp.lists_joined, io=(src, dst, None))
+            sp.lists_joined = True
+            sp.tower.append(d)
+
+        def sparse_tower_form():
+            if not opts.sparse_heads or not opts.sparse_tower or not opts.decode_overlap or opts.x3_level < 1 or self.dtype not in C.X3_TYPES:
+                return False
+            kh, kw, cin, cout = self.conv_w['pyramid_regression_ops'][2]
+            split = (C.latency_split if self.plan_mode == 'latency' else C.default_split)(kh, kw, cin, cout, sum(f.H * f.W for f in reg_o))
+            kh, kw, cin, cout = self.conv_w['pyramid_regression_3'][2]
+            split3 = (C.latency_split if self.plan_mode == 'latency' else C.default_split)(kh, kw, cin, cout, sum(f.H * f.W for f in reg_o))
+            if split > 1 or split3 > 1 or cout % 256:
+                return False
+            workgroups = sum((P[0].B * m.H * m.W + 255) // 256 for m in P) * (cout // 256)
+            return workgroups > opts.sparse_tower_rounds * COMPUTE_UNITS
 
         def out_layer(name, src, out, lane, join):
             sp = plan.sparse
@@ -461,7 +490,8 @@
                   'reg': ('pyramid_regression', 512, 0, 'pyramid_regression_ops', reg_o, 1, 0, bool(opts.cls_lane)),
                   'dim': ('pyramid_regression_dim', 128, 768, 'pyramid_regression_dim', dim_o, 0, l_dim)}
         if opts.sparse_heads:
-            plan.sparse = SparseHeads(self.torch, self.device, P[0].B, [m.H * m.W for m in P], opts.sparse_heads)
+            plan.sparse = SparseHeads(self.torch, self.device, P[0].B, [m.H * m.W for m in P], opts.sparse_heads, [m.W for m in P],
+                                      opts.sparse_tower if sparse_tower_form() else 0.0)
             plan.keep += plan.sparse.tensors()
         if opts.decode_overlap:
             tower(*towers['cls'])
@@ -621,6 +651,9 @@
             autotune=env('GPP_AUTOTUNE', '1') != '0',
             sparse_heads=(max(1e-9, float(env('GPP_SPARSE_HEADS_MAX_SHARE', SPARSE_HEADS_MAX_SHARE)))
                           if (overlap and not self.audit and env('GPP_SPARSE_HEADS', '1') != '0') else 0.0),
+            sparse_tower=(max(1e-9, float(env('GPP_SPARSE_TOWER_MAX_SHARE', SPARSE_TOWER_MAX_SHARE)))
+                          if (overlap and not self.audit and env('GPP_SPARSE_HEADS', '1') != '0' and env('GPP_SPARSE_TOWER', '1') != '0') else 0.0),
+            sparse_tower_rounds=float(env('GPP_SPARSE_TOWER_MIN_ROUNDS', SPARSE_TOWER_MIN_ROUNDS)),
             tune_key='x3split={};fuse={}/{};plan={}{}'.format(env('GPP_X3_SPLIT', '2'), env('GPP_FUSE_TAIL', '64,128'), env('GPP_FUSE_BLOCK', '64,128'),
                                                               self.plan_mode, C.latency_split_config() if self.plan_mode == 'latency' else '') +
                      (';audit' if self.audit else ''))
@@ -752,6 +785,15 @@
             setattr(target, field, self._tuned[key][0])
             plan.tuning[name] = self._tuned[key]
             plan.tuning_parts.setdefault(name, []).append(self._tuned[key])
+            if kind == OP_CONV and desc.tower_rows:
+                rows_key = (name + '@rows',) + key[1:]
+                if rows_key in self._tuned and self._tuned[rows_key][0] not in self._tower_tiles(desc):
+                    del self._tuned[rows_key]
+                if rows_key not in self._tuned:
+                    self._tuned[rows_key] = self._time_tower_tiles(plan, index, desc)
+                    fresh = True
+                desc.tower_tile = self._tuned[rows_key][0]
+                plan.tuning[name + '@rows'] = self._tuned[rows_key]
         if plan.sparse is not None:
             plan.sparse.reset(self.torch)
         self.torch.cuda.synchronize()
@@ -807,6 +849,36 @@
         else:
             hip.check(hip.lib().gpp_conv2d_autotune(ctypes.byref(target), iters, hip.stream_ptr(), ctypes.byref(best)), 'gpp_conv2d_autotune')
         return int(target.tile_hint), round(float(best.value), 2)
+
+    @staticmethod
+    def _tower_tiles(desc):
+        rows = type(desc).from_buffer_copy(desc)
+        rows.gather_rows, rows.gather_counts = desc.tower_rows, desc.tower_counts
+        rows.tower_rows = rows.tower_counts = rows.tower_flag = None
+        rows.tower_tile, rows.split_k = 0, 1
+        tiles, count = (ctypes.c_int * 32)(), ctypes.c_int(0)
+        hip.check(hip.lib().gpp_conv2d_tile_candidates(ctypes.byref(rows), tiles, 32, ctypes.byref(count)), 'gpp_conv2d_tile_candidates')
+        return [t for t in tiles[:min(count.value, 32)] if t]
+
+    def _time_tower_tiles(self, plan, index, desc, iters=8):
+        sp, torch = plan.sparse, self.torch
+        sp.put_every_nth(torch, 3, tower=True)
+        sp.tower_flag.fill_(0)
+        times = {}
+        for tile in self._tower_tiles(desc):
+            desc.tower_tile = tile
+            e0, e1 = torch.cuda.Event(enable_timing=True), torch.cuda.Event(enable_timing=True)
+            self.run_op(plan, index)
+            e0.record()
+            for _ in range(iters):
+                self.run_op(plan, index)
+            e1.record()
+            e1.synchronize()
+            times[tile] = e0.elapsed_time(e1) * 1000.0 / iters
+        sp.tower_flag.fill_(1)
+        sp.tower_counts.zero_()
+        tile = min(times, key=times.get)
+        return tile, round(times[tile], 2)
 
     @staticmethod
     def _tile_is_listed(desc, tile):
diff --git a/include/gpp.h b/include/gpp.h
--- a/include/gpp.h
+++ b/include/gpp.h
@@ -73,6 +73,11 @@
     const int32_t* guard;
     int32_t guard_value;
     int32_t reserved3;
+    const int32_t* tower_rows;
+    const int32_t* tower_counts;
+    const int32_t* tower_flag;
+    int32_t tower_tile;
+    int32_t reserved4;
 } gpp_conv_desc;
 #define GPP_X3_IN 1
 #define GPP_X3_OUT 2
@@ -181,6 +186,8 @@
     int64_t n_anchors;
     int32_t B, num_base_anchors, lists_per_image, n_levels, max_rows, reserved;
     int32_t level_pixels[GPP_MAX_GROUPS]; int32_t reserved2;
+    uint32_t* dilated_bitmap; int32_t* dilated_rows; int32_t* dilated_counts; int32_t* dilated_flag;
+    int32_t level_width[GPP_MAX_GROUPS]; int32_t dilated_max_rows;
 } gpp_pixel_list_desc;
 int gpp_detect_pixel_lists(const gpp_pixel_list_desc* host_desc, void* stream);
 
```
